# lmb-freiburg/neural-point-cloud-diffusion

Measured on AMD Instinct MI355X. Metric: denoiser train steps/sec (+ rendered rays/sec under 'render'), SRN-Cars 512pt x 128d, higher is better.
Workload: dtype bf16; 1 GPU; BASELINE configs[1]: denoiser fwd/bwd + AdamW + EMA, 512 points x 128-d latents, width 1024 / 24 layers / 16 heads (seq 513), bf16 autocast; global_batch=64, per_gpu_batch=64, parallelism=dp1, rng=weights seed 1234 on every rank; timestep / noise draws seed 42 + rank

## Files before the change

include/npcd_hip.h:

```cpp
#ifndef NPCD_HIP_H
#define NPCD_HIP_H

#include <stdint.h>

#ifdef __cplusplus
extern "C" {
#endif

#define NPCD_OK 0
#define NPCD_ERR_ARG (-1)
#define NPCD_ERR_UNSUPPORTED (-2)
#define NPCD_ERR_HIP (-3)

#define NPCD_BF16 0
#define NPCD_F16 1
#define NPCD_F32 2

int npcd_abi_version(void);
const char* npcd_error_string(int code);
const char* npcd_last_hip_error(void);

int npcd_attn_fwd(const void* q, const void* k, const void* v, void* out, float* lse,
                  int B, int n, int H, int d,
                  int64_t qkv_sb, int64_t qkv_sn, int64_t qkv_sh,
                  int64_t out_sb, int64_t out_sn, int64_t out_sh,
                  float scale, int dtype, void* stream);

int64_t npcd_attn_fwd_workspace_floats(int B, int n, int H);
int npcd_attn_fwd_ws(const void* q, const void* k, const void* v, void* out, float* lse, float* workspace,
                     int B, int n, int H, int d,
                     int64_t qkv_sb, int64_t qkv_sn, int64_t qkv_sh,
                     int64_t out_sb, int64_t out_sn, int64_t out_sh,
                     float scale, int dtype, void* stream);

int64_t npcd_attn_fwd_fp8_workspace_bytes(int B, int n, int H);
int npcd_attn_fwd_fp8(const void* q, const void* k, const void* v, void* out, float* lse, void* workspace,
                      int B, int n, int H, int d,
                      int64_t qkv_sb, int64_t qkv_sn, int64_t qkv_sh,
                      int64_t out_sb, int64_t out_sn, int64_t out_sh,
                      float scale, int dtype, void* stream);

int64_t npcd_attn_bwd_workspace_floats(int B, int n, int H);
int npcd_attn_bwd(const void* q, const void* k, const void* v, const void* out, const void* dout,
                  const float* lse, void* dq, void* dk, void* dv, float* delta,
                  int B, int n, int H, int d,
                  int64_t qkv_sb, int64_t qkv_sn, int64_t qkv_sh,
                  int64_t out_sb, int64_t out_sn, int64_t out_sh,
                  int64_t g_sb, int64_t g_sn, int64_t g_sh,
                  float scale, int dtype, void* stream);

int npcd_attn_bwd_colsum_rows(int B, int n, int H);
int npcd_attn_bwd_colsum(int passes, const void* q, const void* k, const void* v, const void* out, const void* dout,
                         const float* lse, void* dq, void* dk, void* dv, float* delta, float* colsum_part,
                         int B, int n, int H, int d,
                         int64_t qkv_sb, int64_t qkv_sn, int64_t qkv_sh,
                         int64_t out_sb, int64_t out_sn, int64_t out_sh,
                         int64_t g_sb, int64_t g_sn, int64_t g_sh,
                         float scale, int dtype, void* stream);

int npcd_attn_bwd_pass(int pass, const void* q, const void* k, const void* v, const void* out, const void* dout,
                       const float* lse, void* dq, void* dk, void* dv, float* delta,
                       int B, int n, int H, int d,
                       int64_t qkv_sb, int64_t qkv_sn, int64_t qkv_sh,
                       int64_t out_sb, int64_t out_sn, int64_t out_sh,
                       int64_t g_sb, int64_t g_sn, int64_t g_sh,
                       float scale, int dtype, void* stream);

int64_t npcd_attn_bwd_fused_slab_floats(int B, int n, int H);
int npcd_attn_bwd_fused(const void* q, const void* k, const void* v, const void* out, const void* dout,
                        const float* lse, void* dq, void* dk, void* dv, float* delta, float* dq_slab,
                        int B, int n, int H, int d,
                        int64_t qkv_sb, int64_t qkv_sn, int64_t qkv_sh,
                        int64_t out_sb, int64_t out_sn, int64_t out_sh,
                        int64_t g_sb, int64_t g_sn, int64_t g_sh,
                        float scale, int dtype, void* stream);

typedef struct npcd_grid_params {
    float voxel_size[3];
    int32_t voxel_scale[3];
    int32_t kernel_size[3];
    int32_t max_points_per_voxel;
    int32_t max_occ_voxels_per_example;
    float range_min[3];
    float range_max[3];
    int32_t dims[3];
    int32_t cdims[3];
    int32_t grid_level;
} npcd_grid_params;
#define NPCD_GRID_FINE 0
#define NPCD_GRID_SCALED 1

int64_t npcd_grid_workspace_bytes(const npcd_grid_params* g, int B, int N);

int npcd_grid_build(const npcd_grid_params* g, const float* points, const int32_t* counts,
                    int B, int N, void* workspace, void* stream);

int npcd_grid_query(const npcd_grid_params* g, const void* workspace, const float* points,
                    int B, int N, int R, int S, int M, int k, float r, int mode,
                    const float* x, const float* rays_o, const float* rays_d,
                    const float* t0, const float* t1,
                    int32_t* sample_idx, float* sample_loc, int32_t* slot_sample, int32_t* nsel,
                    void* stream);

int npcd_grid_query_compact(const npcd_grid_params* g, const void* workspace, const float* points,
                            int B, int N, int R, int S, int M, int k, float r,
                            const float* rays_o, const float* rays_d, const float* t0, const float* t1,
                            int32_t* counter, int32_t capacity, int32_t* ray_base, int32_t* ray_nsel,
                            uint64_t* ray_bits, int32_t* nb_idx, float* pts, void* stream);

int64_t npcd_grid_query_order_ws_bytes(int B, int R, int M, int k);
int npcd_grid_query_compact_ordered(const npcd_grid_params* g, const void* workspace, const float* points,
                                    int B, int N, int R, int S, int M, int k, float r,
                                    const float* rays_o, const float* rays_d, const float* t0, const float* t1,
                                    int32_t* counter, int32_t capacity, int32_t* ray_base, int32_t* ray_nsel,
                                    uint64_t* ray_bits, int32_t* nb_idx, float* pts, void* order_ws, void* stream);

int64_t npcd_ray_gen_ws_floats(int V, int res, int n_ids);
int npcd_ray_gen(const float* extr, const float* intr, int V, int res, float box,
                 float* rays_o, float* rays_d, float* t0, float* t1, float* limits_ws, void* stream);
int npcd_ray_gen_subset(const float* extr, const float* intr, int V, int res, float box, const int32_t* pixel_ids, int n_ids,
                        float* rays_o, float* rays_d, float* t0, float* t1, float* limits_ws, void* stream);

#define NPCD_SHADE_NONFINITE_PAIRS 1
#define NPCD_SHADE_NONFINITE_HEADS 2
int64_t npcd_shade_wpack_bytes(int feat_dim, int n_freqs, int hidden);
int64_t npcd_shade_workspace_bytes(int max_points, int hidden);
int npcd_shade_pack_weights(const float* const* weights_host, const float* const* biases_host,
                            int feat_dim, int n_freqs, int hidden, void* wpack_host);
int npcd_shade_points(const void* wpack, int feat_dim, int n_freqs, int hidden,
                      const int32_t* nb_idx, const float* pts, const float* kp_pos, const float* kp_feat,
                      const int32_t* n_points_dev, int max_points, int k,
                      float* sigma, float* rgb, void* workspace, int32_t* status, void* stream);

int npcd_shade_points_dir(const void* wpack, int feat_dim, int n_freqs, int hidden,
                          const int32_t* nb_idx, const float* pts, const float* kp_pos, const float* kp_feat,
                          const int32_t* n_points_dev, int max_points, int k,
                          float* sigma, float* rgb, void* workspace, const float* dir_bias, const int32_t* point_ray,
                          int32_t* status, void* stream);

int64_t npcd_pairs_x2_wpack_bytes(int feat_dim);
int npcd_pairs_x2_pack(const float* const* weights_host, const float* const* biases_host, int feat_dim, void* wpack_host);
int npcd_pairs_x2(const void* wpack, int feat_dim, const int32_t* nb_idx, const float* pts, const float* kp_pos, const float* kp_feat,
                  const int32_t* n_points_dev, int max_points, int k, float* G, void* stream);
int64_t npcd_points_x2_wpack_bytes(void);
int npcd_points_x2_pack(const float* const* weights_host, const float* const* biases_host, int c0_in_dim, void* wpack_host);
int npcd_points_x2(const void* wpack, const float* feat, const int32_t* n_points_dev, int max_points, float* sigma, float* rgb,
                   const float* dir_bias, const int32_t* point_ray, void* stream);
int npcd_points_x2_train(const void* wpack, const float* feat, int max_points, float* save, float* pre, void* stream);
int npcd_points_x2_pack_dev(const float* const* weights_dev, const float* const* biases_dev, int c0_in_dim, void* wpack_dev, void* stream);

int64_t npcd_ray_march_ws_floats(int Nr);
int npcd_ray_march(const float* sigma, const float* rgb, const uint8_t* slot_valid, const float* slot_loc,
                   const int32_t* point_base, const float* rays_o, const float* rays_d, const float* t1,
                   int Nr, int M, int white_back, float* mask, float* depth, float* channels,
                   float* depth_ws, void* stream);

int npcd_ray_march_bwd(const float* sigma, const float* rgb, const uint8_t* slot_valid, const float* slot_loc,
                       const int32_t* point_base, const float* rays_o, const float* rays_d, const float* t1,
                       int Nr, int M, int white_back, const float* depth_ws, const float* g_mask, const float* g_depth,
                       const float* g_chan, float* dsigma, float* drgb, void* stream);

int npcd_add_ln_fwd(const float* x_in, const void* delta, const float* gamma, const float* beta,
                    float* x_out, void* y, float* mean, float* rstd, int T, int W, float eps, void* stream);
int npcd_ln_bwd_blocks(int T);
int npcd_ln_bwd(const void* dy, const float* x, const float* mean, const float* rstd, const float* gamma,
                const float* dres, float* dx, void* dxb, float* part_gamma, float* part_beta,
                float* part_col, int T, int W, void* stream);
int npcd_colsum_scratch_rows(void);
int npcd_colsum_finalize(const float* part, int nblk, int N, float* out, int accumulate, void* stream);
#define NPCD_COLSUM_MAX_JOBS 8
typedef struct NpcdColsumJob {
    const float* part;
    float* out;
    int nblk, N, accumulate, reserved;
} NpcdColsumJob;
int npcd_colsum_finalize_batch(const NpcdColsumJob* jobs, int njobs, void* stream);
int npcd_gelu_fwd(const void* h, void* g, int64_t numel, void* stream);
int npcd_colsum_blocks(int T);
int npcd_gelu_bwd(const void* dg, const void* h, void* dh, float* part, int T, int N, void* stream);
int npcd_colsum_bf16(const void* a, float* part, int T, int N, void* stream);
int npcd_small_wgrad_blocks(int T);
int npcd_small_wgrad(const void* dy, const void* x, float* part, int T, int J, int K, void* stream);
int npcd_adamw_ema(float* p, float* g, float* m, float* v, float* ema, void* shadow_bf16, int64_t numel,
                   float lr, float beta1, float beta2, float eps, float weight_decay, int step,
                   float ema_decay, int zero_grad, void* stream);
int npcd_cast_f32_bf16(const float* src, void* dst, int64_t numel, void* stream);
int npcd_add_ln_fwd_dt(const float* x_in, const void* delta, const float* gamma, const float* beta,
                       float* x_out, void* y, float* mean, float* rstd, int T, int W, float eps, int dtype, void* stream);
int npcd_ln_bwd_dt(const void* dy, const float* x, const float* mean, const float* rstd, const float* gamma,
                   const float* dres, float* dx, void* dxb, float* part_gamma, float* part_beta,
                   float* part_col, int T, int W, int dtype, void* stream);
int npcd_gelu_fwd_dt(const void* h, void* g, int64_t numel, int dtype, void* stream);
int npcd_gelu_bwd_dt(const void* dg, const void* h, void* dh, float* part, int T, int N, int dtype, void* stream);
int npcd_colsum_dt(const void* a, float* part, int T, int N, int dtype, void* stream);
int npcd_adamw_ema_dt(float* p, float* g, float* m, float* v, float* ema, void* shadow, int shadow_dtype, int64_t numel,
                      float lr, float beta1, float beta2, float eps, float weight_decay, int step,
                      float ema_decay, int zero_grad, void* stream);
int npcd_cast_f32_dt(const float* src, void* dst, int64_t numel, int dtype, void* stream);

typedef struct NpcdScalerCtl {
    int32_t found_inf, step, growth_tracker, skipped;
    float loss_scale, inv_scale, grad_norm, clip_coef, bc1, bc2_sqrt;
    int32_t reserved[6];
} NpcdScalerCtl;
int npcd_grad_stats_blocks(void);
int npcd_grad_stats(const float* g, int64_t n, double* work, double* out, void* stream);
int npcd_scaler_finalize(const double* stats, int nslots, NpcdScalerCtl* ctl, int scaling, int clip, float max_norm,
                         float beta1, float beta2, float growth_factor, float backoff_factor, int growth_interval, void* stream);
int npcd_adamw_ema_gated(float* p, float* g, float* m, float* v, float* ema, void* shadow, int shadow_dtype, int64_t numel,
                         float lr, float beta1, float beta2, float eps, float weight_decay, double ema_decay, int zero_grad,
                         const NpcdScalerCtl* ctl, void* stream);

int npcd_wgrad_slices(int T, int N, int K);
int npcd_wgrad(const void* dy, const void* x, float* out, float* workspace, int T, int N, int K, int dtype, void* stream);
int npcd_wgrad_group(int count, const void* const* dy, const void* const* x, float* const* out, const int* N, const int* K, int T,
                     int dtype, void* stream);
int npcd_wgrad_group_blocks(int tiles_per_block, int max_products, int products_per_block);

int npcd_linear_fwd(const void* x, const void* w, const void* bias, void* y, int M, int N, int K, int dtype, void* stream);
int npcd_linear_gelu_fwd(const void* x, const void* w, const void* bias, void* h, void* g, int M, int N, int K, int dtype, void* stream);
int npcd_linear_dgelu_rows(int M);
int npcd_linear_dgelu_bwd(const void* dy, const void* wt, const void* h, void* dh, float* part, int M, int N, int K, int dtype, void* stream);
int npcd_linear128_fwd(const void* x, const void* w, const void* bias, void* y, int M, int N, int K, int dtype, void* stream);
int npcd_transpose_16(const void* in, void* out, int R, int C, void* stream);
int npcd_transpose16_group(int count, const void* const* in, void* const* out, const int* R, const int* C, void* stream);

int npcd_sum_slices(const float* part, float* out, int S, int64_t numel, void* stream);

int npcd_ddpm_reverse_step(const float* x_t, const void* eps, int eps_dtype, const float* noise, float* x_prev, float* x0_out,
                           const int64_t* t, int B, int64_t per_sample, const float* tab_recip, const float* tab_recipm1,
                           const float* tab_coef1, const float* tab_coef2, const float* tab_logvar, float clip_lo, float clip_hi,
                           int has_clip, void* stream);

#define NPCD_SAMPLER_REVERSE 0
#define NPCD_SAMPLER_HOLD 1
typedef struct NpcdSamplerTensor {
    const float* x_t;
    const void* eps;
    const float* noise;
    const float* known;
    float* out;
    float* x0_out;
    int64_t per_sample;
    float clip_lo, clip_hi;
    int32_t has_clip, mode, eps_dtype, reserved;
} NpcdSamplerTensor;
int npcd_sampler_step(const NpcdSamplerTensor* coords, const NpcdSamplerTensor* feats, const int64_t* t, const float* table, int T,
                      int B, int deterministic, void* stream);

int npcd_q_sample(const float* x0, const float* noise, const int64_t* t, const float* tab_sqrt_acp, const float* tab_sqrt_1macp,
                  float* x_t, int B, int64_t per_sample, void* stream);
int npcd_eps_mse_blocks(void);
int npcd_eps_mse_fwd(const float* noise, const void* eps, int eps_dtype, int64_t numel, float* pointwise, float* part, float* loss,
                     void* stream);
int npcd_eps_mse_bwd(const float* noise, const void* eps, int eps_dtype, int64_t numel, const float* upstream_dev, void* grad,
                     void* stream);

int npcd_ray_march_compact(const float* sigma, const float* rgb, const uint64_t* ray_bits, const float* pts,
                           const int32_t* ray_base, const float* rays_o, const float* rays_d, const float* t1,
                           int Nr, int M, int capacity, int white_back, float* mask, float* depth, float* channels,
                           float* depth_ws, void* stream);

int64_t npcd_render_lim_words(int B, int R);
int npcd_render_rays_query(const npcd_grid_params* grid, const void* workspace, const float* points, int B, int N, const float* extr,
                           const float* intr, int views, int res, float box, int S, int M, int k, float r, float* rays_o, float* rays_d,
                           float* t0, float* t1, int32_t* counter, int32_t capacity, int32_t* ray_base, int32_t* ray_nsel,
                           uint64_t* ray_bits, int32_t* nb_idx, float* pts, void* order_ws, uint32_t* lim_part, void* stream);
int npcd_ray_march_compact_fused(const float* sigma, const float* rgb, const uint64_t* ray_bits, const float* pts, const int32_t* ray_base,
                                 const float* rays_o, const float* rays_d, const float* t0, const float* t1, const uint32_t* lim_part,
                                 int lim_pairs, int Nr, int M, int capacity, int white_back, float* mask, float* depth,
                                 float* channels, float* depth_ws, void* stream);

int npcd_pair_input_fwd(const int64_t* flat, const int64_t* owner, const float* pts, const float* kp_pos, const float* kp_feat,
                        int feat_dim, int n_freqs, int64_t n_pairs, float* x0, float* w, void* stream);
int npcd_pair_input_bwd(const int64_t* flat, const float* dx0, int feat_dim, int n_cols, int64_t n_pairs, float* dfeat, void* stream);
int npcd_leaky_bwd_blocks(int64_t rows);
int npcd_leaky_bwd_colsum(const void* dz, const void* z, void* dy, float* part, int64_t rows, int N, float slope, int dtype,
                          void* stream);
int npcd_pair_aggregate(int backward, const float* src, const float* w, const int64_t* off, const int64_t* cnt, int channels,
                        int64_t n_points, float* dst, void* stream);

#define NPCD_PAIR_MLP_BF16 0
#define NPCD_PAIR_MLP_X2 1
int64_t npcd_pair_mlp_wpack_bytes(int feat_dim, int precision);
int npcd_pair_mlp_pack(const float* const* weights_dev, const float* const* biases_dev, int feat_dim, int precision, void* wpack_dev,
                       void* stream);
int npcd_pair_mlp_fwd(const void* wpack, int feat_dim, int precision, const int64_t* nb_idx, const float* pts, const float* kp_pos,
                      const float* kp_feat, const int64_t* off, int64_t n_points, int k, int64_t n_pairs, void* x0, void* acts,
                      float* wn, float* G, void* stream);
int npcd_pair_mlp_bwd_slabs(int64_t n_pairs, int precision);
int64_t npcd_pair_mlp_bwd_workspace_floats(int feat_dim, int64_t n_pairs, int precision);
int npcd_pair_mlp_bwd(const void* wpack, int feat_dim, int precision, const float* dG, const int64_t* owner, const float* wn,
                      const void* x0, const void* acts, int64_t n_pairs, void* dact, float* dfeat, float* part, float* const* dW,
                      float* const* db, void* stream);

int npcd_split3_bf16(const float* x, const float* bias, void* out, int64_t rows, int K, int gelu, void* stream);
int npcd_add_ln_split3_bf16(const float* x, const float* o, const float* bias, const float* gamma, const float* beta, float* xnew,
                            void* out, int64_t rows, int W, float eps, void* stream);

#define NPCD_SPLIT_WEIGHTS_MAX 8
typedef struct NpcdSplitWeight {
    const float* w;
    void* fwd;
    void* dgrad;
    int N, K;
} NpcdSplitWeight;
int npcd_add_ln_split3_stats_bf16(const float* x, const float* o, const float* bias, const float* gamma, const float* beta, float* xnew,
                                  void* out, float* mean, float* rstd, int64_t rows, int W, float eps, void* stream);
int npcd_split_weights_bf16(const NpcdSplitWeight* desc, int count, void* stream);
int npcd_ln_bwd_split3_bf16(const float* dy, const float* x, const float* mean, const float* rstd, const float* gamma,
                            const float* dres, float* dx, void* dx3, float* part_gamma, float* part_beta, float* part_col, int T, int W,
                            void* stream);
int npcd_split3_colsum_bf16(const float* a, const float* h, const float* bias, void* out, float* part, int T, int N, int gelu,
                            void* stream);

int64_t npcd_stage1_reg_workspace_floats(int B);
int npcd_stage1_reg_fwd(const float* coords, const int32_t* nb, int64_t nb_ld, const float* feats, int64_t feats_ld, const float* mean,
                        const float* log_var, int64_t kl_ld, int B, int N, int k, int F, float weight_tv, float weight_kl, int dtype,
                        float* tv_pointwise, float* tv_total, float* kl_pointwise, float* kl_total, float* workspace, void* stream);
int npcd_stage1_reg_bwd(const float* coords, const int32_t* nb, int64_t nb_ld, const float* feats, int64_t feats_ld, const float* mean,
                        const float* log_var, int64_t kl_ld, int B, int N, int k, int F, float weight_tv, float weight_kl, int dtype,
                        const float* g_tv_total, const float* g_tv_pointwise, const float* g_kl_total, const float* g_kl_pointwise,
                        float* dfeats, float* dmean, float* dlog_var, void* stream);

int npcd_fps_resident_points(void);
int npcd_fps_max_points(void);
int npcd_fps(const float* points, const int32_t* lengths, const int32_t* ks, const int32_t* start, int64_t* idx_out, float* pts_out,
             int N, int P, int Kmax, void* stream);

int npcd_chamfer_max_points(void);
int npcd_chamfer_directed(const float* x, const int32_t* x_len, const float* y, const int32_t* y_len, float* out, int M, int P, int N,
                          int Q, void* stream);

int npcd_emd_max_points(void);
int npcd_emd_directed(const float* x, const int32_t* x_len, const float* y, const int32_t* y_len, float* out, int M, int P, int N, int Q,
                      void* stream);

int npcd_occupancy_max_resolution(void);
int npcd_occupancy_clouds_per_workgroup(int n, int P, int R);
int npcd_occupancy_grid(const float* points, const int32_t* lengths, const float* lattice, const uint8_t* k_lo, const uint8_t* k_hi,
                        int32_t* counts, int32_t* clouds, int32_t* cells, int n, int P, int R, void* stream);

int npcd_image_metrics_tile(int* rows_host, int* cols_host);
int64_t npcd_image_metrics_workspace_bytes(int V, int C, int H, int W, int w);
int npcd_image_metrics(const float* pred, const float* target, int V, int C, int H, int W, int64_t pred_sv, int64_t pred_sc,
                       int64_t pred_sh, int64_t pred_sw, int64_t target_sv, int64_t target_sc, int64_t target_sh, int64_t target_sw,
                       const double* taps, int w, double n, double data_range, double* workspace, double* mse, double* ssim, double* map,
                       void* stream);

#ifdef __cplusplus
}
#endif
#endif
```

neural-point-cloud-diffusion_amd/csrc/elementwise.hip:

```cpp
#include <math.h>

#include <stdlib.h>

#include "common.h"

namespace npcd {

constexpr int kMaxChunks = 8;

template <class E>
struct V {
    typedef E x4 __attribute__((ext_vector_type(4)));
    typedef E x8 __attribute__((ext_vector_type(8)));
};
template <class X4>
__device__ __forceinline__ f32x4 to_f32(X4 v) { return f32x4{(float)v[0], (float)v[1], (float)v[2], (float)v[3]}; }
template <class E>
__device__ __forceinline__ typename V<E>::x4 from_f32(f32x4 v) { return typename V<E>::x4{(E)v[0], (E)v[1], (E)v[2], (E)v[3]}; }
__device__ __forceinline__ f32x4 bf16x4_to_f32(bf16x4 v) { return to_f32(v); }
__device__ __forceinline__ bf16x4 f32_to_bf16x4(f32x4 v) { return from_f32<__bf16>(v); }

template <class E, int NCH>
__global__ __launch_bounds__(256) void add_ln_fwd_kernel(const float* __restrict__ x_in, const E* __restrict__ delta,
                                                         const float* __restrict__ gamma, const float* __restrict__ beta,
                                                         float* __restrict__ x_out, E* __restrict__ y, float* __restrict__ mean,
                                                         float* __restrict__ rstd, int T, int W, float eps) {
    using e4 = typename V<E>::x4;
    const int lane = threadIdx.x & 63, wave = threadIdx.x >> 6;
    const int NW = gridDim.x * 4;
    int row = blockIdx.x * 4 + wave;
    if (row >= T) return;
    f32x4 gm[NCH], bt[NCH], v[NCH], nx[NCH];
    e4 nd[NCH];
#pragma unroll
    for (int ch = 0; ch < NCH; ++ch) {
        const int c = ch * 256 + lane * 4;
        gm[ch] = bt[ch] = nx[ch] = f32x4{0.f, 0.f, 0.f, 0.f};
        nd[ch] = e4{0, 0, 0, 0};
        if (c < W) {
            gm[ch] = *reinterpret_cast<const f32x4*>(gamma + c);
            bt[ch] = *reinterpret_cast<const f32x4*>(beta + c);
        }
    }
    auto load_row = [&](int r) {
        const int64_t base = (int64_t)r * W;
#pragma unroll
        for (int ch = 0; ch < NCH; ++ch) {
            const int c = ch * 256 + lane * 4;
            if (c < W) {
                nx[ch] = *reinterpret_cast<const f32x4*>(x_in + base + c);
                if (delta) nd[ch] = *reinterpret_cast<const e4*>(delta + base + c);
            }
        }
    };
    load_row(row);
    for (; row < T; row += NW) {
        const int64_t base = (int64_t)row * W;
        float s = 0.f;
#pragma unroll
        for (int ch = 0; ch < NCH; ++ch) {
            v[ch] = nx[ch];
            if (delta) v[ch] += to_f32(nd[ch]);
        }
        if (row + NW < T) load_row(row + NW);
#pragma unroll
        for (int ch = 0; ch < NCH; ++ch) {
            const int c = ch * 256 + lane * 4;
            if (c < W) {
                if (x_out) *reinterpret_cast<f32x4*>(x_out + base + c) = v[ch];
                s += (v[ch][0] + v[ch][1]) + (v[ch][2] + v[ch][3]);
            }
        }
        const float mu = wave_sum64(s) / (float)W;
        float q = 0.f;
#pragma unroll
        for (int ch = 0; ch < NCH; ++ch) {
            const int c = ch * 256 + lane * 4;
            if (c < W) {
                const f32x4 d = v[ch] - mu;
                q += (d[0] * d[0] + d[1] * d[1]) + (d[2] * d[2] + d[3] * d[3]);
            }
        }
        const float rs = rsqrtf(wave_sum64(q) / (float)W + eps);
#pragma unroll
        for (int ch = 0; ch < NCH; ++ch) {
            const int c = ch * 256 + lane * 4;
            if (c < W) *reinterpret_cast<e4*>(y + base + c) = from_f32<E>((v[ch] - mu) * rs * gm[ch] + bt[ch]);
        }
        if (lane == 0) {
            mean[row] = mu;
            rstd[row] = rs;
        }
    }
}

static inline int ln_rows_per_wave(int T) {
    const int one_round = (T + 4 * 512 - 1) / (4 * 512);
    if (one_round <= 32) return one_round < 1 ? 1 : one_round;
    return 16;
}

template <class E, int NCH, class D = E, bool SPLIT = false>
__global__ __launch_bounds__(256, 2) void ln_bwd_kernel(const D* __restrict__ dy, const float* __restrict__ x, const float* __restrict__ mean,
                                                     const float* __restrict__ rstd, const float* __restrict__ gamma,
                                                     const float* __restrict__ dres, float* __restrict__ dx, E* __restrict__ dxb,
                                                     float* __restrict__ part_gamma, float* __restrict__ part_beta,
                                                     float* __restrict__ part_col, int T, int W, int rows_per_wave) {
    using e4 = typename V<D>::x4;
    extern __shared__ __attribute__((aligned(16))) unsigned char dsmem[];
    float* red = reinterpret_cast<float*>(dsmem);
    const int lane = threadIdx.x & 63, wave = threadIdx.x >> 6;
    f32x4 ag[NCH], ab[NCH], ac[NCH];
#pragma unroll
    for (int ch = 0; ch < NCH; ++ch) ag[ch] = ab[ch] = ac[ch] = f32x4{0.f, 0.f, 0.f, 0.f};
    const int row0 = blockIdx.x * 4 + wave, NW = gridDim.x * 4;
    const int nrows = row0 < T ? min(rows_per_wave, (T - row0 + NW - 1) / NW) : 0;
    e4 dyA[NCH], dyB[NCH];
    f32x4 xA[NCH], xB[NCH], rA[NCH], rB[NCH];
    float muA = 0.f, rsA = 0.f, muB = 0.f, rsB = 0.f;
    auto load_row = [&](int row, e4 (&dyr)[NCH], f32x4 (&xr)[NCH], f32x4 (&rr2)[NCH], float& mu, float& rs) {
        const int64_t base = (int64_t)row * W;
        mu = mean[row];
        rs = rstd[row];
#pragma unroll
        for (int ch = 0; ch < NCH; ++ch) {
            const int c = ch * 256 + lane * 4;
            if (c < W) {
                dyr[ch] = *reinterpret_cast<const e4*>(dy + base + c);
                xr[ch] = *reinterpret_cast<const f32x4*>(x + base + c);
                if (dres) rr2[ch] = *reinterpret_cast<const f32x4*>(dres + base + c);
            }
        }
    };
    if (nrows > 0) load_row(row0, dyA, xA, rA, muA, rsA);
    for (int rr = 0; rr < nrows; ++rr) {
        const int row = row0 + rr * NW;
        const int64_t base = (int64_t)row * W;
        if (rr + 1 < nrows) load_row(row + NW, dyB, xB, rB, muB, rsB);
        const float mu = muA, rs = rsA;
        f32x4 gy[NCH], xh[NCH];
        float s1 = 0.f, s2 = 0.f;
#pragma unroll
        for (int ch = 0; ch < NCH; ++ch) {
            const int c = ch * 256 + lane * 4;
            gy[ch] = xh[ch] = f32x4{0.f, 0.f, 0.f, 0.f};
            if (c < W) {
                const f32x4 d = to_f32(dyA[ch]);
                xh[ch] = (xA[ch] - mu) * rs;
                ag[ch] += d * xh[ch];
                ab[ch] += d;
                gy[ch] = d * *reinterpret_cast<const f32x4*>(gamma + c);
                const f32x4 t = gy[ch] * xh[ch];
                s1 += (gy[ch][0] + gy[ch][1]) + (gy[ch][2] + gy[ch][3]);
                s2 += (t[0] + t[1]) + (t[2] + t[3]);
            }
        }
        const float c1 = wave_sum64(s1) / (float)W, c2 = wave_sum64(s2) / (float)W;
#pragma unroll
        for (int ch = 0; ch < NCH; ++ch) {
            const int c = ch * 256 + lane * 4;
            if (c < W) {
                f32x4 o = (gy[ch] - c1 - xh[ch] * c2) * rs;
                if (dres) o += rA[ch];
                *reinterpret_cast<f32x4*>(dx + base + c) = o;
                if (SPLIT && dxb) {
                    bf16x4 hi, lo;
#pragma unroll
                    for (int j = 0; j < 4; ++j) {
                        hi[j] = (__bf16)o[j];
                        lo[j] = (__bf16)(o[j] - (float)hi[j]);
                    }
                    __bf16* o3 = reinterpret_cast<__bf16*>(dxb) + 3 * base + c;
                    *reinterpret_cast<bf16x4*>(o3) = hi;
                    *reinterpret_cast<bf16x4*>(o3 + W) = lo;
                    *reinterpret_cast<bf16x4*>(o3 + 2 * W) = hi;
                } else if (dxb) {
                    *reinterpret_cast<typename V<E>::x4*>(dxb + base + c) = from_f32<E>(o);
                }
                ac[ch] += o;
            }
        }
#pragma unroll
        for (int ch = 0; ch < NCH; ++ch) {
            dyA[ch] = dyB[ch];
            xA[ch] = xB[ch];
            rA[ch] = rB[ch];
        }
        muA = muB;
        rsA = rsB;
    }
#pragma unroll
    for (int ch = 0; ch < NCH; ++ch) {
        const int c = ch * 256 + lane * 4;
        if (c < W) {
            *reinterpret_cast<f32x4*>(red + (0 * 4 + wave) * W + c) = ag[ch];
            *reinterpret_cast<f32x4*>(red + (1 * 4 + wave) * W + c) = ab[ch];
            *reinterpret_cast<f32x4*>(red + (2 * 4 + wave) * W + c) = ac[ch];
        }
    }
    __syncthreads();
    float* outs[3] = {part_gamma, part_beta, part_col};
    for (int q = 0; q < 3; ++q) {
        if (!outs[q]) continue;
        for (int c = threadIdx.x; c < W; c += 256) {
            const float* p = red + q * 4 * W + c;
            outs[q][(int64_t)blockIdx.x * W + c] = (p[0] + p[W]) + (p[2 * W] + p[3 * W]);
        }
    }
}

constexpr int kFinSlices = 16;

struct FinBatch {
    NpcdColsumJob job[NPCD_COLSUM_MAX_JOBS];
    int first1[NPCD_COLSUM_MAX_JOBS + 1];
    int first2[NPCD_COLSUM_MAX_JOBS + 1];
    int njobs;
};
__device__ __forceinline__ int fin_job(const int* first, int njobs, int bx) {
    int j = 0;
    while (j + 1 < njobs && bx >= first[j + 1]) ++j;
    return j;
}
__device__ __forceinline__ bool fin_two_stage(int nblk) { return nblk > 2 * kFinSlices; }

__global__ __launch_bounds__(256) void colsum_stage1_kernel(FinBatch fb) {
    __shared__ float red[4][64];
    const int j = fin_job(fb.first1, fb.njobs, blockIdx.x);
    const float* __restrict__ part = fb.job[j].part;
    const int nblk = fb.job[j].nblk, N = fb.job[j].N;
    if (!fin_two_stage(nblk)) return;
    float* __restrict__ stage = const_cast<float*>(part) + (int64_t)nblk * N;
    const int tx = threadIdx.x & 63, ty = threadIdx.x >> 6;
    const int c = (blockIdx.x - fb.first1[j]) * 64 + tx;
    const int per = (nblk + kFinSlices - 1) / kFinSlices;
    const int b0 = blockIdx.y * per, b1 = min(nblk, b0 + per);
    float s0 = 0.f, s1 = 0.f;
    if (c < N) {
        int b = b0 + ty;
        for (; b + 4 < b1; b += 8) {
            s0 += part[(int64_t)b * N + c];
            s1 += part[(int64_t)(b + 4) * N + c];
        }
        if (b < b1) s0 += part[(int64_t)b * N + c];
    }
    red[ty][tx] = s0 + s1;
    __syncthreads();
    if (ty == 0 && c < N) stage[(int64_t)blockIdx.y * N + c] = (red[0][tx] + red[1][tx]) + (red[2][tx] + red[3][tx]);
}

__global__ __launch_bounds__(256) void colsum_stage2_kernel(FinBatch fb) {
    const int j = fin_job(fb.first2, fb.njobs, blockIdx.x);
    const int nblk = fb.job[j].nblk, N = fb.job[j].N;
    const int c = (blockIdx.x - fb.first2[j]) * 256 + threadIdx.x;
    if (c >= N) return;
    const bool two = fin_two_stage(nblk);
    const float* __restrict__ src = two ? fb.job[j].part + (int64_t)nblk * N : fb.job[j].part;
    const int nrows = two ? kFinSlices : nblk;
    float s = 0.f;
    for (int k = 0; k < nrows; ++k) s += src[(int64_t)k * N + c];
    float* __restrict__ out = fb.job[j].out;
    out[c] = fb.job[j].accumulate ? out[c] + s : s;
}

__device__ __forceinline__ float gelu_f(float x) { return 0.5f * x * (1.f + erff(x * 0.70710678118654752f)); }
__device__ __forceinline__ float gelu_grad_f(float x) {
    return 0.5f * (1.f + erff(x * 0.70710678118654752f)) + x * 0.3989422804014327f * __expf(-0.5f * x * x);
}

__device__ __forceinline__ float gelu_fast(float x) {
    const float u = fabsf(x) * 0.70710678118654752f;
    const float t = __builtin_amdgcn_rcpf(__builtin_fmaf(0.3275911f, u, 1.f));
    const float e = __builtin_amdgcn_exp2f(x * x * -0.72134752044448170f);
    float poly = __builtin_fmaf(t, 1.061405429f, -1.453152027f);
    poly = __builtin_fmaf(poly, t, 1.421413741f);
    poly = __builtin_fmaf(poly, t, -0.284496736f);
    poly = __builtin_fmaf(poly, t, 0.254829592f);
    const float erf_abs = __builtin_fmaf(-poly * t, e, 1.f);
    return x * __builtin_fmaf(0.5f, copysignf(erf_abs, x), 0.5f);
}

template <class E, int VARIANT>
__global__ __launch_bounds__(256) void gelu_fwd_kernel(const typename V<E>::x8* __restrict__ h, typename V<E>::x8* __restrict__ g, int64_t n8) {
    using e8 = typename V<E>::x8;
    for (int64_t i = (int64_t)blockIdx.x * 256 + threadIdx.x; i < n8; i += (int64_t)gridDim.x * 256) {
        const e8 v = h[i];
        e8 o;
#pragma unroll
        for (int j = 0; j < 8; ++j) o[j] = (E)(VARIANT == 0 ? gelu_f((float)v[j]) : gelu_fast((float)v[j]));
        g[i] = o;
    }
}

static inline int col_rows(int T) {
    static const int forced = [] { const char* e = getenv("NPCD_COL_ROWS"); return e ? atoi(e) : 0; }();
    if (forced > 0) return forced;
    int r = T / 512;
    return r < 8 ? 8 : (r > 64 ? 64 : r);
}

__device__ __forceinline__ float gelu_grad_fast(float x) {
    const float u = fabsf(x) * 0.70710678118654752f;
    const float t = __builtin_amdgcn_rcpf(__builtin_fmaf(0.3275911f, u, 1.f));
    const float e = __builtin_amdgcn_exp2f(x * x * -0.72134752044448170f);
    float poly = __builtin_fmaf(t, 1.061405429f, -1.453152027f);
    poly = __builtin_fmaf(poly, t, 1.421413741f);
    poly = __builtin_fmaf(poly, t, -0.284496736f);
    poly = __builtin_fmaf(poly, t, 0.254829592f);
    const float erf_abs = __builtin_fmaf(-poly * t, e, 1.f);
    const float phi_cdf = __builtin_fmaf(0.5f, copysignf(erf_abs, x), 0.5f);
    return __builtin_fmaf(x * 0.3989422804014327f, e, phi_cdf);
}

template <class E, bool GELU, int VARIANT = 1>
__global__ __launch_bounds__(256) void colsum_kernel(const E* __restrict__ a, const E* __restrict__ hpre, E* __restrict__ out,
                                                     float* __restrict__ part, int T, int N, int rows) {
    using e8 = typename V<E>::x8;
    const int col = (blockIdx.x * 256 + threadIdx.x) * 8;
    if (col >= N) return;
    float acc[8];
#pragma unroll
    for (int j = 0; j < 8; ++j) acc[j] = 0.f;
    auto one = [&](const e8 v, const e8 hp, int64_t off) {
        e8 o;
#pragma unroll
        for (int j = 0; j < 8; ++j) {
            const float gp = VARIANT == 0 ? gelu_grad_f((float)hp[j]) : gelu_grad_fast((float)hp[j]);
            o[j] = (E)((float)v[j] * gp);
            acc[j] += (float)o[j];
        }
        *reinterpret_cast<e8*>(out + off) = o;
    };
    if (GELU && VARIANT == 2) {
        int rr = 0;
        for (; rr + 1 < rows; rr += 2) {
            const int r0 = rr * gridDim.y + blockIdx.y, r1 = r0 + gridDim.y;
            if (r1 >= T) break;
            const int64_t o0 = (int64_t)r0 * N + col, o1 = (int64_t)r1 * N + col;
            const e8 v0 = *reinterpret_cast<const e8*>(a + o0), h0 = *reinterpret_cast<const e8*>(hpre + o0);
            const e8 v1 = *reinterpret_cast<const e8*>(a + o1), h1 = *reinterpret_cast<const e8*>(hpre + o1);
            one(v0, h0, o0);
            one(v1, h1, o1);
        }
        for (; rr < rows; ++rr) {
            const int row = rr * gridDim.y + blockIdx.y;
            if (row >= T) break;
            const int64_t off = (int64_t)row * N + col;
            one(*reinterpret_cast<const e8*>(a + off), *reinterpret_cast<const e8*>(hpre + off), off);
        }
    } else {
        for (int rr = 0; rr < rows; ++rr) {
            const int row = rr * gridDim.y + blockIdx.y;
            if (row >= T) break;
            const int64_t off = (int64_t)row * N + col;
            const e8 v = (GELU && VARIANT == 3) ? __builtin_nontemporal_load(reinterpret_cast<const e8*>(a + off))
                                                    : *reinterpret_cast<const e8*>(a + off);
            if (GELU) {
                one(v, VARIANT == 3 ? __builtin_nontemporal_load(reinterpret_cast<const e8*>(hpre + off))
                                    : *reinterpret_cast<const e8*>(hpre + off), off);
            } else {
#pragma unroll
                for (int j = 0; j < 8; ++j) acc[j] += (float)v[j];
            }
        }
    }
    float* p = part + (int64_t)blockIdx.y * N + col;
    *reinterpret_cast<f32x4*>(p) = f32x4{acc[0], acc[1], acc[2], acc[3]};
    *reinterpret_cast<f32x4*>(p + 4) = f32x4{acc[4], acc[5], acc[6], acc[7]};
}

template <int J>
__global__ __launch_bounds__(256) void small_wgrad_kernel(const __bf16* __restrict__ dy, const __bf16* __restrict__ x, float* __restrict__ part,
                                                          int T, int K, int rows_per_block) {
    extern __shared__ float swg_red[];
    const int chunks = K >> 3, lanes = 256 / chunks;
    const int cc = threadIdx.x % chunks, rl = threadIdx.x / chunks;
    const int row0 = blockIdx.x * rows_per_block, row1 = min(T, row0 + rows_per_block);
    float acc[J][8];
#pragma unroll
    for (int j = 0; j < J; ++j)
#pragma unroll
        for (int i = 0; i < 8; ++i) acc[j][i] = 0.f;
    for (int row = row0 + rl; row < row1; row += lanes) {
        const bf16x8 v = *reinterpret_cast<const bf16x8*>(x + (int64_t)row * K + 8 * cc);
        float w[J];
#pragma unroll
        for (int j = 0; j < J; ++j) w[j] = (float)dy[(int64_t)row * J + j];
#pragma unroll
        for (int j = 0; j < J; ++j)
#pragma unroll
            for (int i = 0; i < 8; ++i) acc[j][i] = __builtin_fmaf(w[j], (float)v[i], acc[j][i]);
    }
#pragma unroll
    for (int j = 0; j < J; ++j)
#pragma unroll
        for (int i = 0; i < 8; ++i) swg_red[(rl * J + j) * K + 8 * cc + i] = acc[j][i];
    __syncthreads();
    for (int e = threadIdx.x; e < J * K; e += 256) {
        float sum = 0.f;
        for (int r2 = 0; r2 < lanes; ++r2) sum += swg_red[r2 * J * K + e];
        part[(int64_t)blockIdx.x * J * K + e] = sum;
    }
}

struct AdamArgs {
    float lr, beta1, beta2, eps, wd, bc1, bc2_sqrt, ema_w;
};

__device__ __forceinline__ void adamw_one(f32x4& pp, const f32x4 gg, f32x4& mm, f32x4& vv, const AdamArgs& a) {
    pp *= (1.f - a.lr * a.wd);
    mm = mm * a.beta1 + gg * (1.f - a.beta1);
    vv = vv * a.beta2 + gg * gg * (1.f - a.beta2);
    const float step = a.lr / a.bc1;
#pragma unroll
    for (int j = 0; j < 4; ++j) pp[j] -= step * (mm[j] / (sqrtf(vv[j]) / a.bc2_sqrt + a.eps));
}

template <class E, bool GATED>
__device__ __forceinline__ void adamw_ema_body(f32x4* __restrict__ p, f32x4* __restrict__ g, f32x4* __restrict__ m, f32x4* __restrict__ v,
                                               f32x4* __restrict__ ema, typename V<E>::x4* __restrict__ shadow, int64_t n4, AdamArgs a,
                                               int zero_grad, const NpcdScalerCtl* __restrict__ ctl, float skip_ema_w) {
    const int64_t stride = (int64_t)gridDim.x * 256;
    int64_t i = (int64_t)blockIdx.x * 256 + threadIdx.x;
    float gs = 1.f, gc = 1.f;
    if constexpr (GATED) {
        if (ctl->found_inf) {
            for (; i < n4; i += stride) {
                if (ema) {
                    const f32x4 e = ema[i], pp = p[i];
                    ema[i] = e + (pp - e) * skip_ema_w;
                }
                if (zero_grad) g[i] = f32x4{0.f, 0.f, 0.f, 0.f};
            }
            return;
        }
        gs = ctl->inv_scale;
        gc = ctl->clip_coef;
        a.bc1 = ctl->bc1;
        a.bc2_sqrt = ctl->bc2_sqrt;
    }
    auto grad = [&](f32x4 x) -> f32x4 {
        if constexpr (GATED) {
            x = (x * gs) * gc;
            asm volatile("" : "+v"(x));
        }
        return x;
    };
    for (; i + stride < n4; i += 2 * stride) {
        const int64_t k = i + stride;
        f32x4 p0 = p[i], p1 = p[k];
        const f32x4 g0 = grad(g[i]), g1 = grad(g[k]);
        f32x4 m0 = m[i], m1 = m[k], v0 = v[i], v1 = v[k];
        f32x4 e0 = {0.f, 0.f, 0.f, 0.f}, e1 = e0;
        if (ema) { e0 = ema[i]; e1 = ema[k]; }
        adamw_one(p0, g0, m0, v0, a);
        adamw_one(p1, g1, m1, v1, a);
        p[i] = p0; p[k] = p1;
        m[i] = m0; m[k] = m1;
        v[i] = v0; v[k] = v1;
        if (ema) { ema[i] = e0 + (p0 - e0) * a.ema_w; ema[k] = e1 + (p1 - e1) * a.ema_w; }
        if (shadow) { shadow[i] = from_f32<E>(p0); shadow[k] = from_f32<E>(p1); }
        if (zero_grad) { g[i] = f32x4{0.f, 0.f, 0.f, 0.f}; g[k] = f32x4{0.f, 0.f, 0.f, 0.f}; }
    }
    if (i < n4) {
        f32x4 pp = p[i];
        const f32x4 gg = grad(g[i]);
        f32x4 mm = m[i], vv = v[i];
        adamw_one(pp, gg, mm, vv, a);
        p[i] = pp;
        m[i] = mm;
        v[i] = vv;
        if (ema) {
            const f32x4 e = ema[i];
            ema[i] = e + (pp - e) * a.ema_w;
        }
        if (shadow) shadow[i] = from_f32<E>(pp);
        if (zero_grad) g[i] = f32x4{0.f, 0.f, 0.f, 0.f};
    }
}

template <class E>
__global__ __launch_bounds__(256) void adamw_ema_kernel(f32x4* __restrict__ p, f32x4* __restrict__ g, f32x4* __restrict__ m, f32x4* __restrict__ v,
                                                        f32x4* __restrict__ ema, typename V<E>::x4* __restrict__ shadow, int64_t n4, AdamArgs a, int zero_grad) {
    adamw_ema_body<E, false>(p, g, m, v, ema, shadow, n4, a, zero_grad, nullptr, 0.f);
}
template <class E>
__global__ __launch_bounds__(256) void adamw_ema_gated_kernel(f32x4* __restrict__ p, f32x4* __restrict__ g, f32x4* __restrict__ m,
                                                              f32x4* __restrict__ v, f32x4* __restrict__ ema, typename V<E>::x4* __restrict__ shadow,
                                                              int64_t n4, AdamArgs a, int zero_grad, const NpcdScalerCtl* __restrict__ ctl,
                                                              float skip_ema_w) {
    adamw_ema_body<E, true>(p, g, m, v, ema, shadow, n4, a, zero_grad, ctl, skip_ema_w);
}

constexpr int kStatBlocks = 512;

__device__ __forceinline__ void stat_one(float x, double& s, uint32_t& bad) {
    const bool ok = fabsf(x) <= 3.402823466e38f;
    const double d = ok ? (double)x : 0.0;
    s = fma(d, d, s);
    bad += ok ? 0u : 1u;
}
__device__ __forceinline__ void stat_four(f32x4 x, double& s, uint32_t& bad) {
#pragma unroll
    for (int j = 0; j < 4; ++j) stat_one(x[j], s, bad);
}
__device__ __forceinline__ double wave_sum_f64(double x) {
#pragma unroll
    for (int off = 32; off > 0; off >>= 1) x += __shfl_xor(x, off, 64);
    return x;
}
__device__ __forceinline__ void block_sum2(double& s, double& c) {
    __shared__ double red[2][4];
    s = wave_sum_f64(s);
    c = wave_sum_f64(c);
    if ((threadIdx.x & 63) == 0) { red[0][threadIdx.x >> 6] = s; red[1][threadIdx.x >> 6] = c; }
    __syncthreads();
    s = (red[0][0] + red[0][1]) + (red[0][2] + red[0][3]);
    c = (red[1][0] + red[1][1]) + (red[1][2] + red[1][3]);
}

__global__ __launch_bounds__(256) void grad_stats_kernel(const float* __restrict__ g, int64_t n, double* __restrict__ part) {
    const f32x4* g4 = reinterpret_cast<const f32x4*>(g);
    const int64_t n4 = n / 4, stride = (int64_t)gridDim.x * 256, gid = (int64_t)blockIdx.x * 256 + threadIdx.x;
    double s = 0.0;
    uint32_t bad = 0;
    int64_t i = gid;
    for (; i + stride < n4; i += 2 * stride) {
        const f32x4 x0 = g4[i], x1 = g4[i + stride];
        stat_four(x0, s, bad);
        stat_four(x1, s, bad);
    }
    if (i < n4) stat_four(g4[i], s, bad);
    if (gid < n - 4 * n4) stat_one(g[4 * n4 + gid], s, bad);
    double c = (double)bad;
    block_sum2(s, c);
    if (threadIdx.x == 0) { part[2 * blockIdx.x] = s; part[2 * blockIdx.x + 1] = c; }
}
__global__ __launch_bounds__(256) void grad_stats_sum_kernel(const double* __restrict__ part, int nblk, double* __restrict__ out) {
    double s = 0.0, c = 0.0;
    for (int b = threadIdx.x; b < nblk; b += 256) { s += part[2 * b]; c += part[2 * b + 1]; }
    block_sum2(s, c);
    if (threadIdx.x == 0) { out[0] = s; out[1] = c; }
}

__global__ __launch_bounds__(64) void scaler_finalize_kernel(const double* __restrict__ stats, int nslots, NpcdScalerCtl* __restrict__ ctl,
                                                             int scaling, int clip, float max_norm, float beta1, float beta2, float growth,
                                                             float backoff, int interval) {
    if (threadIdx.x != 0) return;
    double sumsq = 0.0, bad = 0.0;
    for (int k = 0; k < nslots; ++k) { sumsq += stats[2 * k]; bad += stats[2 * k + 1]; }
    NpcdScalerCtl c = *ctl;
    const float inv = scaling ? 1.f / c.loss_scale : 1.f;
    c.inv_scale = inv;
    c.found_inf = (scaling && bad > 0.0) ? 1 : 0;
    const float norm = bad > 0.0 ? INFINITY : (float)(sqrt(sumsq) * (double)inv);
    c.grad_norm = norm;
    c.clip_coef = clip ? fminf((1.f / (norm + 1e-6f)) * max_norm, 1.f) : 1.f;
    if (c.found_inf) {
        c.loss_scale *= backoff;
        c.growth_tracker = 0;
        c.skipped += 1;
    } else {
        c.step += 1;
        c.bc1 = (float)(1.0 - pow((double)beta1, (double)c.step));
        c.bc2_sqrt = (float)sqrt(1.0 - pow((double)beta2, (double)c.step));
        if (scaling && ++c.growth_tracker == interval) {
            c.loss_scale *= growth;
            c.growth_tracker = 0;
        }
    }
    *ctl = c;
}

template <class E>
__global__ __launch_bounds__(256) void cast_kernel(const f32x4* __restrict__ src, typename V<E>::x4* __restrict__ dst, int64_t n4) {
    for (int64_t i = (int64_t)blockIdx.x * 256 + threadIdx.x; i < n4; i += (int64_t)gridDim.x * 256) dst[i] = from_f32<E>(src[i]);
}

template <int S>
__global__ __launch_bounds__(256) void sum_slices_kernel(const f32x4* __restrict__ part, f32x4* __restrict__ out, int64_t n4) {
    for (int64_t i = (int64_t)blockIdx.x * 256 + threadIdx.x; i < n4; i += (int64_t)gridDim.x * 256) {
        f32x4 v[S];
#pragma unroll
        for (int s2 = 0; s2 < S; ++s2) v[s2] = __builtin_nontemporal_load(part + s2 * n4 + i);
        f32x4 acc = v[0];
#pragma unroll
        for (int s2 = 1; s2 < S; ++s2) acc += v[s2];
        out[i] = acc;
    }
}

struct DdpmTables {
    const float *recip, *recipm1, *c1, *c2, *logvar;
};
template <class EPS>
__global__ __launch_bounds__(256) void ddpm_reverse_kernel(const float* __restrict__ x_t, const EPS* __restrict__ eps, const float* __restrict__ noise,
                                                           float* __restrict__ x_prev, float* __restrict__ x0_out, const int64_t* __restrict__ t,
                                                           int64_t per_sample, DdpmTables tab, float lo, float hi, int has_clip) {
    const int b = blockIdx.y;
    const int64_t ts = t[b];
    const float a = tab.recip[ts], bb = tab.recipm1[ts], c1 = tab.c1[ts], c2 = tab.c2[ts];
    const float sd = ts != 0 ? expf(0.5f * tab.logvar[ts]) : 0.f;
    for (int64_t i = (int64_t)blockIdx.x * 256 + threadIdx.x; i < per_sample; i += (int64_t)gridDim.x * 256) {
        const int64_t j = (int64_t)b * per_sample + i;
        const float x = x_t[j];
        float x0 = a * x - bb * (float)eps[j];
        if (has_clip) x0 = fminf(fmaxf(x0, lo), hi);
        if (x0_out) x0_out[j] = x0;
        x_prev[j] = (c1 * x0 + c2 * x) + sd * noise[j];
    }
}

struct SamplerCoef {
    float r, m, c1, c2, s, h1, h2;
};
struct SamplerArgs {
    NpcdSamplerTensor tz[2];
    int vec[2];
};

__device__ __forceinline__ float sampler_x0(const SamplerCoef& k, float x, float e, int has_clip, float lo, float hi) {
    float x0 = __builtin_fmaf(k.r, x, -(k.m * e));
    if (has_clip) x0 = fminf(fmaxf(x0, lo), hi);
    return x0;
}

template <class EPS, bool VEC>
__device__ __forceinline__ void sampler_reverse(const NpcdSamplerTensor& a, const SamplerCoef& k, int64_t base) {
    const float* __restrict__ x_t = a.x_t + base;
    const EPS* __restrict__ eps = static_cast<const EPS*>(a.eps) + base;
    const float* __restrict__ noise = a.noise ? a.noise + base : nullptr;
    float* __restrict__ out = a.out + base;
    float* __restrict__ x0_out = a.x0_out ? a.x0_out + base : nullptr;
    if constexpr (VEC) {
        const int64_t n4 = a.per_sample / 4;
        for (int64_t i = (int64_t)blockIdx.x * 256 + threadIdx.x; i < n4; i += (int64_t)gridDim.x * 256) {
            const f32x4 x = reinterpret_cast<const f32x4*>(x_t)[i];
            const f32x4 e = to_f32(reinterpret_cast<const typename V<EPS>::x4*>(eps)[i]);
            f32x4 z = f32x4{0.f, 0.f, 0.f, 0.f};
            if (noise) z = reinterpret_cast<const f32x4*>(noise)[i];
            f32x4 x0, o;
#pragma unroll
            for (int q = 0; q < 4; ++q) {
                x0[q] = sampler_x0(k, x[q], e[q], a.has_clip, a.clip_lo, a.clip_hi);
                o[q] = __builtin_fmaf(k.c1, x0[q], k.c2 * x[q]);
                if (noise) o[q] = __builtin_fmaf(k.s, z[q], o[q]);
            }
            if (x0_out) reinterpret_cast<f32x4*>(x0_out)[i] = x0;
            reinterpret_cast<f32x4*>(out)[i] = o;
        }
    } else {
        for (int64_t i = (int64_t)blockIdx.x * 256 + threadIdx.x; i < a.per_sample; i += (int64_t)gridDim.x * 256) {
            const float x = x_t[i];
            const float x0 = sampler_x0(k, x, (float)eps[i], a.has_clip, a.clip_lo, a.clip_hi);
            float o = __builtin_fmaf(k.c1, x0, k.c2 * x);
            if (noise) o = __builtin_fmaf(k.s, noise[i], o);
            if (x0_out) x0_out[i] = x0;
            out[i] = o;
        }
    }
}

template <bool VEC>
__device__ __forceinline__ void sampler_hold(const NpcdSamplerTensor& a, const SamplerCoef& k, int64_t base) {
    const float* __restrict__ known = a.known + base;
    const float* __restrict__ noise = a.noise + base;
    float* __restrict__ out = a.out + base;
    if constexpr (VEC) {
        const int64_t n4 = a.per_sample / 4;
        for (int64_t i = (int64_t)blockIdx.x * 256 + threadIdx.x; i < n4; i += (int64_t)gridDim.x * 256) {
            const f32x4 kn = reinterpret_cast<const f32x4*>(known)[i], z = reinterpret_cast<const f32x4*>(noise)[i];
            f32x4 o;
#pragma unroll
            for (int q = 0; q < 4; ++q) o[q] = __builtin_fmaf(k.h1, kn[q], k.h2 * z[q]);
            reinterpret_cast<f32x4*>(out)[i] = o;
        }
    } else {
        for (int64_t i = (int64_t)blockIdx.x * 256 + threadIdx.x; i < a.per_sample; i += (int64_t)gridDim.x * 256)
            out[i] = __builtin_fmaf(k.h1, known[i], k.h2 * noise[i]);
    }
}

__global__ __launch_bounds__(256) void sampler_step_kernel(SamplerArgs args, const int64_t* __restrict__ t, const float* __restrict__ table, int T) {
    const int z = blockIdx.z, b = blockIdx.y;
    const NpcdSamplerTensor& a = args.tz[z];
    const int vec = args.vec[z];
    const int64_t ts = t[b];
    const float nan = __builtin_nanf("");
    SamplerCoef k{nan, nan, nan, nan, nan, nan, nan};
    if (ts >= 0 && ts < T) {
        const f32x4 lo = reinterpret_cast<const f32x4*>(table)[2 * ts], hi = reinterpret_cast<const f32x4*>(table)[2 * ts + 1];
        k = SamplerCoef{lo[0], lo[1], lo[2], lo[3], hi[0], hi[1], hi[2]};
    }
    const int64_t base = (int64_t)b * a.per_sample;
    if (a.mode == NPCD_SAMPLER_HOLD) {
        if (vec) sampler_hold<true>(a, k, base);
        else sampler_hold<false>(a, k, base);
    } else if (a.eps_dtype == NPCD_F32) {
        if (vec) sampler_reverse<float, true>(a, k, base);
        else sampler_reverse<float, false>(a, k, base);
    } else {
        if (vec) sampler_reverse<__bf16, true>(a, k, base);
        else sampler_reverse<__bf16, false>(a, k, base);
    }
}

static bool al16(const void* p) { return (reinterpret_cast<uintptr_t>(p) & 15) == 0; }

}

using namespace npcd;

static inline int ln_fwd_blocks(int T) { const int b = (T + 3) / 4; return b < 2048 ? b : 2048; }

static inline bool dt16(int dtype) { return dtype == NPCD_BF16 || dtype == NPCD_F16; }

extern "C" int npcd_add_ln_fwd_dt(const float* x_in, const void* delta, const float* gamma, const float* beta, float* x_out, void* y,
                                  float* mean, float* rstd, int T, int W, float eps, int dtype, void* stream) {
    if (!x_in || !gamma || !beta || !y || !mean || !rstd || T <= 0 || W <= 0) return NPCD_ERR_ARG;
    if (W % 4 != 0 || W > 256 * kMaxChunks || !dt16(dtype)) return NPCD_ERR_UNSUPPORTED;
    if (!al16(x_in) || !al16(gamma) || !al16(beta) || (x_out && !al16(x_out)) || (reinterpret_cast<uintptr_t>(y) & 7) ||
        (delta && (reinterpret_cast<uintptr_t>(delta) & 7)))
        return NPCD_ERR_ARG;
#define NPCD_LAUNCH_LN_FWD(E, NCH)                                                                                            \
    hipLaunchKernelGGL((add_ln_fwd_kernel<E, NCH>), dim3(ln_fwd_blocks(T)), dim3(256), 0, static_cast<hipStream_t>(stream), x_in, \
                       static_cast<const E*>(delta), gamma, beta, x_out, static_cast<E*>(y), mean, rstd, T, W, eps)
#define NPCD_LN_FWD_W(E)                     \
    do {                                     \
        if (W <= 256) NPCD_LAUNCH_LN_FWD(E, 1);      \
        else if (W <= 512) NPCD_LAUNCH_LN_FWD(E, 2); \
        else if (W <= 1024) NPCD_LAUNCH_LN_FWD(E, 4);\
        else NPCD_LAUNCH_LN_FWD(E, 8);               \
    } while (0)
    if (dtype == NPCD_BF16) NPCD_LN_FWD_W(__bf16);
    else NPCD_LN_FWD_W(_Float16);
#undef NPCD_LN_FWD_W
#undef NPCD_LAUNCH_LN_FWD
    NPCD_HIP_CHECK(hipGetLastError());
    return NPCD_OK;
}
extern "C" int npcd_add_ln_fwd(const float* x_in, const void* delta, const float* gamma, const float* beta, float* x_out, void* y,
                               float* mean, float* rstd, int T, int W, float eps, void* stream) {
    return npcd_add_ln_fwd_dt(x_in, delta, gamma, beta, x_out, y, mean, rstd, T, W, eps, NPCD_BF16, stream);
}

extern "C" int npcd_ln_bwd_blocks(int T) { const int r = ln_rows_per_wave(T); return (T + 4 * r - 1) / (4 * r); }

extern "C" int npcd_ln_bwd_dt(const void* dy, const float* x, const float* mean, const float* rstd, const float* gamma, const float* dres,
                              float* dx, void* dxb, float* part_gamma, float* part_beta, float* part_col, int T, int W, int dtype, void* stream) {
    if (!dy || !x || !mean || !rstd || !gamma || !dx || T <= 0 || W <= 0) return NPCD_ERR_ARG;
    if (W % 4 != 0 || W > 256 * kMaxChunks || !dt16(dtype)) return NPCD_ERR_UNSUPPORTED;
    if (!al16(x) || !al16(gamma) || !al16(dx) || (dres && !al16(dres))) return NPCD_ERR_ARG;
    const int nblk = npcd_ln_bwd_blocks(T);
    const size_t lds = (size_t)3 * 4 * W * sizeof(float);
    hipStream_t st = static_cast<hipStream_t>(stream);
    static DynLds lds_attr_b, lds_attr_h;
    if (dtype == NPCD_BF16) NPCD_HIP_CHECK(lds_attr_b.ensure(reinterpret_cast<const void*>(ln_bwd_kernel<__bf16, 8>), 3 * 4 * 2048 * 4));
    else NPCD_HIP_CHECK(lds_attr_h.ensure(reinterpret_cast<const void*>(ln_bwd_kernel<_Float16, 8>), 3 * 4 * 2048 * 4));
#define NPCD_LAUNCH_LN_BWD(E, NCH)                                                                                             \
    hipLaunchKernelGGL((ln_bwd_kernel<E, NCH>), dim3(nblk), dim3(256), lds, st, static_cast<const E*>(dy), x, mean, rstd, gamma, \
                       dres, dx, static_cast<E*>(dxb), part_gamma, part_beta, part_col, T, W, ln_rows_per_wave(T))
#define NPCD_LN_BWD_W(E)                     \
    do {                                     \
        if (W <= 256) NPCD_LAUNCH_LN_BWD(E, 1);      \
        else if (W <= 512) NPCD_LAUNCH_LN_BWD(E, 2); \
        else if (W <= 1024) NPCD_LAUNCH_LN_BWD(E, 4);\
        else NPCD_LAUNCH_LN_BWD(E, 8);               \
    } while (0)
    if (dtype == NPCD_BF16) NPCD_LN_BWD_W(__bf16);
    else NPCD_LN_BWD_W(_Float16);
#undef NPCD_LN_BWD_W
#undef NPCD_LAUNCH_LN_BWD
    NPCD_HIP_CHECK(hipGetLastError());
    return NPCD_OK;
}
extern "C" int npcd_ln_bwd_split3_bf16(const float* dy, const float* x, const float* mean, const float* rstd, const float* gamma,
                                       const float* dres, float* dx, void* dx3, float* part_gamma, float* part_beta, float* part_col, int T,
                                       int W, void* stream) {
    if (!dy || !x || !mean || !rstd || !gamma || !dx || T <= 0 || W <= 0) return NPCD_ERR_ARG;
    if (W % 4 != 0 || W > 256 * kMaxChunks) return NPCD_ERR_UNSUPPORTED;
    if (!al16(dy) || !al16(x) || !al16(gamma) || !al16(dx) || (dres && !al16(dres)) || (dx3 && !al16(dx3))) return NPCD_ERR_ARG;
    const int nblk = npcd_ln_bwd_blocks(T);
    const size_t lds = (size_t)3 * 4 * W * sizeof(float);
    hipStream_t st = static_cast<hipStream_t>(stream);
    static DynLds lds_attr;
    NPCD_HIP_CHECK(lds_attr.ensure(reinterpret_cast<const void*>(ln_bwd_kernel<__bf16, 8, float, true>), 3 * 4 * 2048 * 4));
#define NPCD_LAUNCH_LN_BWD3(NCH)                                                                                                        \
    hipLaunchKernelGGL((ln_bwd_kernel<__bf16, NCH, float, true>), dim3(nblk), dim3(256), lds, st, dy, x, mean, rstd, gamma, dres, dx, \
                       static_cast<__bf16*>(dx3), part_gamma, part_beta, part_col, T, W, ln_rows_per_wave(T))
    if (W <= 256) NPCD_LAUNCH_LN_BWD3(1);
    else if (W <= 512) NPCD_LAUNCH_LN_BWD3(2);
    else if (W <= 1024) NPCD_LAUNCH_LN_BWD3(4);
    else NPCD_LAUNCH_LN_BWD3(8);
#undef NPCD_LAUNCH_LN_BWD3
    NPCD_HIP_CHECK(hipGetLastError());
    return NPCD_OK;
}

extern "C" int npcd_ln_bwd(const void* dy, const float* x, const float* mean, const float* rstd, const float* gamma, const float* dres,
                           float* dx, void* dxb, float* part_gamma, float* part_beta, float* part_col, int T, int W, void* stream) {
    return npcd_ln_bwd_dt(dy, x, mean, rstd, gamma, dres, dx, dxb, part_gamma, part_beta, part_col, T, W, NPCD_BF16, stream);
}

__global__ __launch_bounds__(1024) void colsum_onepass_kernel(FinBatch fb) {
    __shared__ float red[16][64];
    const int j = fin_job(fb.first1, fb.njobs, blockIdx.x);
    const float* __restrict__ part = fb.job[j].part;
    const int nblk = fb.job[j].nblk, N = fb.job[j].N;
    const int tx = threadIdx.x & 63, ty = threadIdx.x >> 6;
    const int c = (blockIdx.x - fb.first1[j]) * 64 + tx;
    float s0 = 0.f, s1 = 0.f;
    if (c < N) {
        int b = ty;
        for (; b + 16 < nblk; b += 32) {
            s0 += part[(int64_t)b * N + c];
            s1 += part[(int64_t)(b + 16) * N + c];
        }
        if (b < nblk) s0 += part[(int64_t)b * N + c];
    }
    red[ty][tx] = s0 + s1;
    __syncthreads();
    if (ty == 0 && c < N) {
        float q[4];
#pragma unroll
        for (int g = 0; g < 4; ++g) q[g] = (red[4 * g][tx] + red[4 * g + 1][tx]) + (red[4 * g + 2][tx] + red[4 * g + 3][tx]);
        const float s = (q[0] + q[1]) + (q[2] + q[3]);
        float* __restrict__ out = fb.job[j].out;
        out[c] = fb.job[j].accumulate ? out[c] + s : s;
    }
}

extern "C" int npcd_colsum_scratch_rows(void) { return kFinSlices; }

extern "C" int npcd_colsum_finalize_batch(const NpcdColsumJob* jobs, int njobs, void* stream) {
    if (!jobs || njobs <= 0 || njobs > NPCD_COLSUM_MAX_JOBS) return NPCD_ERR_ARG;
    FinBatch fb;
    fb.njobs = njobs;
    bool any_two_stage = false;
    int n1 = 0, n2 = 0;
    for (int j = 0; j < njobs; ++j) {
        if (!jobs[j].part || !jobs[j].out || jobs[j].nblk <= 0 || jobs[j].N <= 0) return NPCD_ERR_ARG;
        fb.job[j] = jobs[j];
        fb.first1[j] = n1;
        fb.first2[j] = n2;
        n1 += (jobs[j].N + 63) / 64;
        n2 += (jobs[j].N + 255) / 256;
        any_two_stage |= jobs[j].nblk > 2 * kFinSlices;
    }
    for (int j = njobs; j <= NPCD_COLSUM_MAX_JOBS; ++j) { fb.first1[j] = n1; fb.first2[j] = n2; }
    hipStream_t st = static_cast<hipStream_t>(stream);
    static const bool onepass = [] { const char* e = getenv("NPCD_COLSUM_ONEPASS"); return e && atoi(e) > 0; }();
    if (onepass) {
        hipLaunchKernelGGL(colsum_onepass_kernel, dim3(n1), dim3(1024), 0, st, fb);
        NPCD_HIP_CHECK(hipGetLastError());
        return NPCD_OK;
    }
    if (any_two_stage) hipLaunchKernelGGL(colsum_stage1_kernel, dim3(n1, kFinSlices), dim3(256), 0, st, fb);
    hipLaunchKernelGGL(colsum_stage2_kernel, dim3(n2), dim3(256), 0, st, fb);
    NPCD_HIP_CHECK(hipGetLastError());
    return NPCD_OK;
}

extern "C" int npcd_colsum_finalize(const float* part, int nblk, int N, float* out, int accumulate, void* stream) {
    NpcdColsumJob job;
    job.part = part; job.out = out; job.nblk = nblk; job.N = N; job.accumulate = accumulate; job.reserved = 0;
    return npcd_colsum_finalize_batch(&job, 1, stream);
}

extern "C" int npcd_gelu_fwd_dt(const void* h, void* g, int64_t numel, int dtype, void* stream) {
    if (!h || !g || numel <= 0) return NPCD_ERR_ARG;
    if (numel % 8 != 0 || !al16(h) || !al16(g) || !dt16(dtype)) return NPCD_ERR_UNSUPPORTED;
    const int64_t n8 = numel / 8;
    const int grid = (int)((n8 + 255) / 256 < 16384 ? (n8 + 255) / 256 : 16384);
    static const int variant = [] { const char* e = getenv("NPCD_GELU_FWD_VARIANT"); return e ? atoi(e) : 1; }();
    hipStream_t st = static_cast<hipStream_t>(stream);
#define NPCD_LAUNCH_GELU_FWD(E, VV)                                                                                                 \
    hipLaunchKernelGGL((gelu_fwd_kernel<E, VV>), dim3(grid), dim3(256), 0, st, static_cast<const typename V<E>::x8*>(h), \
                       static_cast<typename V<E>::x8*>(g), n8)
    if (dtype == NPCD_BF16) {
        if (variant == 0) NPCD_LAUNCH_GELU_FWD(__bf16, 0);
        else NPCD_LAUNCH_GELU_FWD(__bf16, 1);
    } else {
        NPCD_LAUNCH_GELU_FWD(_Float16, 1);
    }
#undef NPCD_LAUNCH_GELU_FWD
    NPCD_HIP_CHECK(hipGetLastError());
    return NPCD_OK;
}
extern "C" int npcd_gelu_fwd(const void* h, void* g, int64_t numel, void* stream) { return npcd_gelu_fwd_dt(h, g, numel, NPCD_BF16, stream); }

extern "C" int npcd_colsum_blocks(int T) { const int r = col_rows(T); return (T + r - 1) / r; }

extern "C" int npcd_gelu_bwd_dt(const void* dg, const void* h, void* dh, float* part, int T, int N, int dtype, void* stream) {
    if (!dg || !h || !dh || !part || T <= 0 || N <= 0) return NPCD_ERR_ARG;
    if (N % 8 != 0 || !al16(dg) || !al16(h) || !al16(dh) || !al16(part) || !dt16(dtype)) return NPCD_ERR_UNSUPPORTED;
    dim3 grid((N / 8 + 255) / 256, npcd_colsum_blocks(T));
    static const int variant = [] { const char* e = getenv("NPCD_GELU_BWD_VARIANT"); return e ? atoi(e) : 1; }();
#define NPCD_LAUNCH_GELU_BWD(E, VV)                                                                                                    \
    hipLaunchKernelGGL((colsum_kernel<E, true, VV>), grid, dim3(256), 0, static_cast<hipStream_t>(stream), static_cast<const E*>(dg), \
                       static_cast<const E*>(h), static_cast<E*>(dh), part, T, N, col_rows(T))
    if (dtype == NPCD_F16) NPCD_LAUNCH_GELU_BWD(_Float16, 1);
    else if (variant == 0) NPCD_LAUNCH_GELU_BWD(__bf16, 0);
    else if (variant == 2) NPCD_LAUNCH_GELU_BWD(__bf16, 2);
    else if (variant == 3) NPCD_LAUNCH_GELU_BWD(__bf16, 3);
    else NPCD_LAUNCH_GELU_BWD(__bf16, 1);
#undef NPCD_LAUNCH_GELU_BWD
    NPCD_HIP_CHECK(hipGetLastError());
    return NPCD_OK;
}
extern "C" int npcd_gelu_bwd(const void* dg, const void* h, void* dh, float* part, int T, int N, void* stream) {
    return npcd_gelu_bwd_dt(dg, h, dh, part, T, N, NPCD_BF16, stream);
}

extern "C" int npcd_colsum_dt(const void* a, float* part, int T, int N, int dtype, void* stream) {
    if (!a || !part || T <= 0 || N <= 0) return NPCD_ERR_ARG;
    if (N % 8 != 0 || !al16(a) || !al16(part) || !dt16(dtype)) return NPCD_ERR_UNSUPPORTED;
    dim3 grid((N / 8 + 255) / 256, npcd_colsum_blocks(T));
    if (dtype == NPCD_BF16)
        hipLaunchKernelGGL((colsum_kernel<__bf16, false>), grid, dim3(256), 0, static_cast<hipStream_t>(stream), static_cast<const __bf16*>(a),
                           static_cast<const __bf16*>(nullptr), static_cast<__bf16*>(nullptr), part, T, N, col_rows(T));
    else
        hipLaunchKernelGGL((colsum_kernel<_Float16, false>), grid, dim3(256), 0, static_cast<hipStream_t>(stream), static_cast<const _Float16*>(a),
                           static_cast<const _Float16*>(nullptr), static_cast<_Float16*>(nullptr), part, T, N, col_rows(T));
    NPCD_HIP_CHECK(hipGetLastError());
    return NPCD_OK;
}
extern "C" int npcd_colsum_bf16(const void* a, float* part, int T, int N, void* stream) { return npcd_colsum_dt(a, part, T, N, NPCD_BF16, stream); }

extern "C" int npcd_small_wgrad_blocks(int T) { return T <= 0 ? -1 : (T + 255) / 256 < 1024 ? (T + 255) / 256 : 1024; }

extern "C" int npcd_small_wgrad(const void* dy, const void* x, float* part, int T, int J, int K, void* stream) {
    if (!dy || !x || !part || T <= 0) return NPCD_ERR_ARG;
    if (J < 1 || J > 4 || K < 64 || K > 2048 || (K & (K - 1)) || !al16(x) || !al16(part)) return NPCD_ERR_UNSUPPORTED;
    const int nblk = npcd_small_wgrad_blocks(T), rpb = (T + nblk - 1) / nblk;
    const size_t lds = (size_t)(256 / (K / 8)) * J * K * sizeof(float);
    hipStream_t st = static_cast<hipStream_t>(stream);
    const __bf16* d = static_cast<const __bf16*>(dy);
    const __bf16* xx = static_cast<const __bf16*>(x);
    switch (J) {
        case 1: hipLaunchKernelGGL(small_wgrad_kernel<1>, dim3(nblk), dim3(256), lds, st, d, xx, part, T, K, rpb); break;
        case 2: hipLaunchKernelGGL(small_wgrad_kernel<2>, dim3(nblk), dim3(256), lds, st, d, xx, part, T, K, rpb); break;
        case 3: hipLaunchKernelGGL(small_wgrad_kernel<3>, dim3(nblk), dim3(256), lds, st, d, xx, part, T, K, rpb); break;
        default: hipLaunchKernelGGL(small_wgrad_kernel<4>, dim3(nblk), dim3(256), lds, st, d, xx, part, T, K, rpb); break;
    }
    NPCD_HIP_CHECK(hipGetLastError());
    return NPCD_OK;
}

extern "C" int npcd_adamw_ema_dt(float* p, float* g, float* m, float* v, float* ema, void* shadow, int shadow_dtype, int64_t numel, float lr,
                                 float beta1, float beta2, float eps, float weight_decay, int step, float ema_decay, int zero_grad, void* stream) {
    if (!p || !g || !m || !v || numel <= 0 || step <= 0) return NPCD_ERR_ARG;
    if (numel % 4 != 0 || !al16(p) || !al16(g) || !al16(m) || !al16(v) || (ema && !al16(ema)) ||
        (shadow && ((reinterpret_cast<uintptr_t>(shadow) & 7) || !dt16(shadow_dtype))))
        return NPCD_ERR_UNSUPPORTED;
    AdamArgs a;
    a.lr = lr; a.beta1 = beta1; a.beta2 = beta2; a.eps = eps; a.wd = weight_decay;
    a.bc1 = (float)(1.0 - pow((double)beta1, (double)step));
    a.bc2_sqrt = (float)sqrt(1.0 - pow((double)beta2, (double)step));
    a.ema_w = 1.f - ema_decay;
    const int64_t n4 = numel / 4;
    const int grid = (int)((n4 + 255) / 256 < 8192 ? (n4 + 255) / 256 : 8192);
    hipStream_t st = static_cast<hipStream_t>(stream);
    if (shadow && shadow_dtype == NPCD_F16)
        hipLaunchKernelGGL(adamw_ema_kernel<_Float16>, dim3(grid), dim3(256), 0, st, reinterpret_cast<f32x4*>(p), reinterpret_cast<f32x4*>(g),
                           reinterpret_cast<f32x4*>(m), reinterpret_cast<f32x4*>(v), reinterpret_cast<f32x4*>(ema),
                           static_cast<V<_Float16>::x4*>(shadow), n4, a, zero_grad);
    else
        hipLaunchKernelGGL(adamw_ema_kernel<__bf16>, dim3(grid), dim3(256), 0, st, reinterpret_cast<f32x4*>(p), reinterpret_cast<f32x4*>(g),
                           reinterpret_cast<f32x4*>(m), reinterpret_cast<f32x4*>(v), reinterpret_cast<f32x4*>(ema),
                           static_cast<V<__bf16>::x4*>(shadow), n4, a, zero_grad);
    NPCD_HIP_CHECK(hipGetLastError());
    return NPCD_OK;
}
extern "C" int npcd_adamw_ema(float* p, float* g, float* m, float* v, float* ema, void* shadow_bf16, int64_t numel, float lr, float beta1,
                              float beta2, float eps, float weight_decay, int step, float ema_decay, int zero_grad, void* stream) {
    return npcd_adamw_ema_dt(p, g, m, v, ema, shadow_bf16, NPCD_BF16, numel, lr, beta1, beta2, eps, weight_decay, step, ema_decay, zero_grad, stream);
}

extern "C" int npcd_adamw_ema_gated(float* p, float* g, float* m, float* v, float* ema, void* shadow, int shadow_dtype, int64_t numel, float lr,
                                    float beta1, float beta2, float eps, float weight_decay, double ema_decay, int zero_grad,
                                    const NpcdScalerCtl* ctl, void* stream) {
    if (!p || !g || !m || !v || !ctl || numel <= 0) return NPCD_ERR_ARG;
    if (numel % 4 != 0 || !al16(p) || !al16(g) || !al16(m) || !al16(v) || (ema && !al16(ema)) || (reinterpret_cast<uintptr_t>(ctl) & 15) ||
        (shadow && ((reinterpret_cast<uintptr_t>(shadow) & 7) || !dt16(shadow_dtype))))
        return NPCD_ERR_UNSUPPORTED;
    AdamArgs a;
    a.lr = lr; a.beta1 = beta1; a.beta2 = beta2; a.eps = eps; a.wd = weight_decay;
    a.bc1 = 1.f; a.bc2_sqrt = 1.f;
    a.ema_w = 1.f - (float)ema_decay;
    const float skip_w = (float)(1.0 - ema_decay);
    const int64_t n4 = numel / 4;
    const int grid = (int)((n4 + 255) / 256 < 8192 ? (n4 + 255) / 256 : 8192);
    hipStream_t st = static_cast<hipStream_t>(stream);
    if (shadow && shadow_dtype == NPCD_F16)
        hipLaunchKernelGGL(adamw_ema_gated_kernel<_Float16>, dim3(grid), dim3(256), 0, st, reinterpret_cast<f32x4*>(p), reinterpret_cast<f32x4*>(g),
                           reinterpret_cast<f32x4*>(m), reinterpret_cast<f32x4*>(v), reinterpret_cast<f32x4*>(ema),
                           static_cast<V<_Float16>::x4*>(shadow), n4, a, zero_grad, ctl, skip_w);
    else
        hipLaunchKernelGGL(adamw_ema_gated_kernel<__bf16>, dim3(grid), dim3(256), 0, st, reinterpret_cast<f32x4*>(p), reinterpret_cast<f32x4*>(g),
                           reinterpret_cast<f32x4*>(m), reinterpret_cast<f32x4*>(v), reinterpret_cast<f32x4*>(ema),
                           static_cast<V<__bf16>::x4*>(shadow), n4, a, zero_grad, ctl, skip_w);
    NPCD_HIP_CHECK(hipGetLastError());
    return NPCD_OK;
}

extern "C" int npcd_grad_stats_blocks(void) { return kStatBlocks; }

extern "C" int npcd_grad_stats(const float* g, int64_t n, double* work, double* out, void* stream) {
    if (!g || !work || !out || n <= 0) return NPCD_ERR_ARG;
    if (!al16(g) || (reinterpret_cast<uintptr_t>(work) & 7) || (reinterpret_cast<uintptr_t>(out) & 7)) return NPCD_ERR_UNSUPPORTED;
    const int64_t n4 = n / 4, want = (n4 + 511) / 512;
    const int grid = (int)(want < 1 ? 1 : want < kStatBlocks ? want : kStatBlocks);
    hipStream_t st = static_cast<hipStream_t>(stream);
    hipLaunchKernelGGL(grad_stats_kernel, dim3(grid), dim3(256), 0, st, g, n, work);
    hipLaunchKernelGGL(grad_stats_sum_kernel, dim3(1), dim3(256), 0, st, work, grid, out);
    NPCD_HIP_CHECK(hipGetLastError());
    return NPCD_OK;
}

extern "C" int npcd_scaler_finalize(const double* stats, int nslots, NpcdScalerCtl* ctl, int scaling, int clip, float max_norm, float beta1,
                                    float beta2, float growth_factor, float backoff_factor, int growth_interval, void* stream) {
    if (!stats || !ctl || nslots <= 0 || growth_interval <= 0) return NPCD_ERR_ARG;
    if ((reinterpret_cast<uintptr_t>(stats) & 7) || (reinterpret_cast<uintptr_t>(ctl) & 15)) return NPCD_ERR_UNSUPPORTED;
    hipLaunchKernelGGL(scaler_finalize_kernel, dim3(1), dim3(64), 0, static_cast<hipStream_t>(stream), stats, nslots, ctl, scaling, clip, max_norm,
                       beta1, beta2, growth_factor, backoff_factor, growth_interval);
    NPCD_HIP_CHECK(hipGetLastError());
    return NPCD_OK;
}

extern "C" int npcd_ddpm_reverse_step(const float* x_t, const void* eps, int eps_dtype, const float* noise, float* x_prev, float* x0_out,
                                      const int64_t* t, int B, int64_t per_sample, const float* tab_recip, const float* tab_recipm1,
                                      const float* tab_coef1, const float* tab_coef2, const float* tab_logvar, float clip_lo, float clip_hi,
                                      int has_clip, void* stream) {
    if (!x_t || !eps || !noise || !x_prev || !t || B <= 0 || per_sample <= 0) return NPCD_ERR_ARG;
    if (!tab_recip || !tab_recipm1 || !tab_coef1 || !tab_coef2 || !tab_logvar) return NPCD_ERR_ARG;
    if (eps_dtype != NPCD_F32 && eps_dtype != NPCD_BF16) return NPCD_ERR_UNSUPPORTED;
    const DdpmTables tab{tab_recip, tab_recipm1, tab_coef1, tab_coef2, tab_logvar};
    const int gx = (int)((per_sample + 255) / 256 < 1024 ? (per_sample + 255) / 256 : 1024);
    hipStream_t st = static_cast<hipStream_t>(stream);
    if (eps_dtype == NPCD_F32)
        hipLaunchKernelGGL(ddpm_reverse_kernel<float>, dim3(gx, B), dim3(256), 0, st, x_t, static_cast<const float*>(eps), noise, x_prev, x0_out, t,
                           per_sample, tab, clip_lo, clip_hi, has_clip);
    else
        hipLaunchKernelGGL(ddpm_reverse_kernel<__bf16>, dim3(gx, B), dim3(256), 0, st, x_t, static_cast<const __bf16*>(eps), noise, x_prev, x0_out, t,
                           per_sample, tab, clip_lo, clip_hi, has_clip);
    NPCD_HIP_CHECK(hipGetLastError());
    return NPCD_OK;
}

extern "C" int npcd_sampler_step(const NpcdSamplerTensor* coords, const NpcdSamplerTensor* feats, const int64_t* t, const float* table, int T,
                                 int B, int deterministic, void* stream) {
    if (!coords || !feats || !t || !table || T <= 0 || B <= 0) return NPCD_ERR_ARG;
    if (B > 65535 || !al16(table)) return NPCD_ERR_UNSUPPORTED;
    SamplerArgs args;
    int gx = 1;
    for (int z = 0; z < 2; ++z) {
        const NpcdSamplerTensor& a = z ? *feats : *coords;
        if (!a.out || a.per_sample <= 0) return NPCD_ERR_ARG;
        bool vec = a.per_sample % 4 == 0 && al16(a.out);
        if (a.mode == NPCD_SAMPLER_HOLD) {
            if (!a.known || !a.noise) return NPCD_ERR_ARG;
            vec = vec && al16(a.known) && al16(a.noise);
        } else if (a.mode == NPCD_SAMPLER_REVERSE) {
            if (!a.x_t || !a.eps || (!a.noise && !deterministic)) return NPCD_ERR_ARG;
            if (a.eps_dtype != NPCD_F32 && a.eps_dtype != NPCD_BF16) return NPCD_ERR_UNSUPPORTED;
            vec = vec && al16(a.x_t) && (!a.noise || al16(a.noise)) && (!a.x0_out || al16(a.x0_out)) &&
                  (reinterpret_cast<uintptr_t>(a.eps) & (a.eps_dtype == NPCD_F32 ? 15 : 7)) == 0;
        } else {
            return NPCD_ERR_ARG;
        }
        args.tz[z] = a;
        args.vec[z] = vec ? 1 : 0;
        const int64_t items = vec ? a.per_sample / 4 : a.per_sample;
        const int g = (int)((items + 255) / 256 < 1024 ? (items + 255) / 256 : 1024);
        gx = g > gx ? g : gx;
    }
    hipLaunchKernelGGL(sampler_step_kernel, dim3(gx, B, 2), dim3(256), 0, static_cast<hipStream_t>(stream), args, t, table, T);
    NPCD_HIP_CHECK(hipGetLastError());
    return NPCD_OK;
}

namespace npcd {
__global__ __launch_bounds__(256) void q_sample_kernel(const float* __restrict__ x0, const float* __restrict__ noise, const int64_t* __restrict__ t,
                                                       const float* __restrict__ tab_a, const float* __restrict__ tab_s, float* __restrict__ xt,
                                                       int64_t per_sample) {
#pragma clang fp contract(off)
    const int b = blockIdx.y;
    const float ca = tab_a[t[b]], cs = tab_s[t[b]];
    const int64_t base = (int64_t)b * per_sample;
    for (int64_t i = (int64_t)blockIdx.x * 256 + threadIdx.x; i < per_sample; i += (int64_t)gridDim.x * 256) {
        const float p0 = ca * x0[base + i], p1 = cs * noise[base + i];
        xt[base + i] = p0 + p1;
    }
}

constexpr int kMseBlocks = 256;
template <class T>
__global__ __launch_bounds__(256) void eps_mse_fwd_kernel(const float* __restrict__ noise, const T* __restrict__ eps, float* __restrict__ pointwise,
                                                          float* __restrict__ part, int64_t numel) {
    __shared__ float red[4];
    float s = 0.f;
    for (int64_t i = (int64_t)blockIdx.x * 256 + threadIdx.x; i < numel; i += (int64_t)gridDim.x * 256) {
        const float d = noise[i] - (float)eps[i];
        const float pw = d * d * 0.5f;
        if (pointwise) pointwise[i] = pw;
        s += pw;
    }
#pragma unroll
    for (int off = 32; off > 0; off >>= 1) s += __shfl_xor(s, off, 64);
    if ((threadIdx.x & 63) == 0) red[threadIdx.x >> 6] = s;
    __syncthreads();
    if (threadIdx.x == 0) part[blockIdx.x] = (red[0] + red[1]) + (red[2] + red[3]);
}
__global__ __launch_bounds__(64) void eps_mse_finalize_kernel(const float* __restrict__ part, int nblocks, float inv_numel, float* __restrict__ out) {
    float s = 0.f;
    for (int i = threadIdx.x; i < nblocks; i += 64) s += part[i];
#pragma unroll
    for (int off = 32; off > 0; off >>= 1) s += __shfl_xor(s, off, 64);
    if (threadIdx.x == 0) out[0] = s * inv_numel;
}
template <class T>
__global__ __launch_bounds__(256) void eps_mse_bwd_kernel(const float* __restrict__ noise, const T* __restrict__ eps, const float* __restrict__ upstream,
                                                          float inv_numel, T* __restrict__ grad, int64_t numel) {
    const float g = upstream[0] * inv_numel;
    for (int64_t i = (int64_t)blockIdx.x * 256 + threadIdx.x; i < numel; i += (int64_t)gridDim.x * 256)
        grad[i] = (T)(-(noise[i] - (float)eps[i]) * g);
}
}

extern "C" int npcd_q_sample(const float* x0, const float* noise, const int64_t* t, const float* tab_sqrt_acp, const float* tab_sqrt_1macp,
                             float* x_t, int B, int64_t per_sample, void* stream) {
    if (!x0 || !noise || !t || !tab_sqrt_acp || !tab_sqrt_1macp || !x_t || B <= 0 || per_sample <= 0) return NPCD_ERR_ARG;
    const int gx = (int)((per_sample + 255) / 256 < 256 ? (per_sample + 255) / 256 : 256);
    hipLaunchKernelGGL(q_sample_kernel, dim3(gx, B), dim3(256), 0, static_cast<hipStream_t>(stream), x0, noise, t, tab_sqrt_acp, tab_sqrt_1macp, x_t,
                       per_sample);
    NPCD_HIP_CHECK(hipGetLastError());
    return NPCD_OK;
}

extern "C" int npcd_eps_mse_blocks(void) { return kMseBlocks; }

extern "C" int npcd_eps_mse_fwd(const float* noise, const void* eps, int eps_dtype, int64_t numel, float* pointwise, float* part, float* loss,
                                void* stream) {
    if (!noise || !eps || !part || !loss || numel <= 0) return NPCD_ERR_ARG;
    if (eps_dtype != NPCD_F32 && eps_dtype != NPCD_BF16) return NPCD_ERR_UNSUPPORTED;
    hipStream_t st = static_cast<hipStream_t>(stream);
    if (eps_dtype == NPCD_F32)
        hipLaunchKernelGGL(eps_mse_fwd_kernel<float>, dim3(kMseBlocks), dim3(256), 0, st, noise, static_cast<const float*>(eps), pointwise, part, numel);
    else
        hipLaunchKernelGGL(eps_mse_fwd_kernel<__bf16>, dim3(kMseBlocks), dim3(256), 0, st, noise, static_cast<const __bf16*>(eps), pointwise, part, numel);
    hipLaunchKernelGGL(eps_mse_finalize_kernel, dim3(1), dim3(64), 0, st, part, kMseBlocks, 1.f / (float)numel, loss);
    NPCD_HIP_CHECK(hipGetLastError());
    return NPCD_OK;
}

extern "C" int npcd_eps_mse_bwd(const float* noise, const void* eps, int eps_dtype, int64_t numel, const float* upstream_dev, void* grad,
                                void* stream) {
    if (!noise || !eps || !upstream_dev || !grad || numel <= 0) return NPCD_ERR_ARG;
    if (eps_dtype != NPCD_F32 && eps_dtype != NPCD_BF16) return NPCD_ERR_UNSUPPORTED;
    hipStream_t st = static_cast<hipStream_t>(stream);
    const int grid = (int)((numel + 255) / 256 < 2048 ? (numel + 255) / 256 : 2048);
    if (eps_dtype == NPCD_F32)
        hipLaunchKernelGGL(eps_mse_bwd_kernel<float>, dim3(grid), dim3(256), 0, st, noise, static_cast<const float*>(eps), upstream_dev,
                           1.f / (float)numel, static_cast<float*>(grad), numel);
    else
        hipLaunchKernelGGL(eps_mse_bwd_kernel<__bf16>, dim3(grid), dim3(256), 0, st, noise, static_cast<const __bf16*>(eps), upstream_dev,
                           1.f / (float)numel, static_cast<__bf16*>(grad), numel);
    NPCD_HIP_CHECK(hipGetLastError());
    return NPCD_OK;
}

extern "C" int npcd_sum_slices(const float* part, float* out, int S, int64_t numel, void* stream) {
    if (!part || !out || numel <= 0) return NPCD_ERR_ARG;
    if ((S != 2 && S != 4 && S != 8) || numel % 4 != 0 || !al16(part) || !al16(out)) return NPCD_ERR_UNSUPPORTED;
    const int64_t n4 = numel / 4;
    const int grid = (int)((n4 + 255) / 256 < 4096 ? (n4 + 255) / 256 : 4096);
    hipStream_t st = static_cast<hipStream_t>(stream);
    const f32x4* p4 = reinterpret_cast<const f32x4*>(part);
    f32x4* o4 = reinterpret_cast<f32x4*>(out);
    if (S == 2) hipLaunchKernelGGL(sum_slices_kernel<2>, dim3(grid), dim3(256), 0, st, p4, o4, n4);
    else if (S == 4) hipLaunchKernelGGL(sum_slices_kernel<4>, dim3(grid), dim3(256), 0, st, p4, o4, n4);
    else hipLaunchKernelGGL(sum_slices_kernel<8>, dim3(grid), dim3(256), 0, st, p4, o4, n4);
    NPCD_HIP_CHECK(hipGetLastError());
    return NPCD_OK;
}

extern "C" int npcd_cast_f32_dt(const float* src, void* dst, int64_t numel, int dtype, void* stream) {
    if (!src || !dst || numel <= 0) return NPCD_ERR_ARG;
    if (numel % 4 != 0 || !al16(src) || (reinterpret_cast<uintptr_t>(dst) & 7) || !dt16(dtype)) return NPCD_ERR_UNSUPPORTED;
    const int64_t n4 = numel / 4;
    const int grid = (int)((n4 + 255) / 256 < 8192 ? (n4 + 255) / 256 : 8192);
    hipStream_t st = static_cast<hipStream_t>(stream);
    if (dtype == NPCD_BF16)
        hipLaunchKernelGGL(cast_kernel<__bf16>, dim3(grid), dim3(256), 0, st, reinterpret_cast<const f32x4*>(src), static_cast<V<__bf16>::x4*>(dst), n4);
    else
        hipLaunchKernelGGL(cast_kernel<_Float16>, dim3(grid), dim3(256), 0, st, reinterpret_cast<const f32x4*>(src), static_cast<V<_Float16>::x4*>(dst), n4);
    NPCD_HIP_CHECK(hipGetLastError());
    return NPCD_OK;
}
extern "C" int npcd_cast_f32_bf16(const float* src, void* dst, int64_t numel, void* stream) { return npcd_cast_f32_dt(src, dst, numel, NPCD_BF16, stream); }
```

neural-point-cloud-diffusion_amd/npcd/hip/__init__.py:

```python
import ctypes
import os
from ctypes import POINTER, c_char_p, c_double, c_float, c_int, c_int32, c_int64, c_void_p

import torch

_PKG_ROOT = os.path.dirname(os.path.dirname(os.path.dirname(os.path.abspath(__file__))))
LIB_PATH = os.environ.get("NPCD_HIP_LIB") or os.path.join(_PKG_ROOT, "lib", "libnpcd_hip.so")

NPCD_BF16, NPCD_F16, NPCD_F32 = 0, 1, 2
NPCD_GRID_FINE, NPCD_GRID_SCALED = 0, 1
_DTYPE_CODE = {torch.bfloat16: NPCD_BF16, torch.float16: NPCD_F16, torch.float32: NPCD_F32}


class GridParams(ctypes.Structure):
    _fields_ = [("voxel_size", c_float * 3), ("voxel_scale", c_int32 * 3), ("kernel_size", c_int32 * 3),
                ("max_points_per_voxel", c_int32), ("max_occ_voxels_per_example", c_int32),
                ("range_min", c_float * 3), ("range_max", c_float * 3), ("dims", c_int32 * 3), ("cdims", c_int32 * 3),
                ("grid_level", c_int32)]


_P = c_void_p
SIGNATURES = {
    "npcd_abi_version": (c_int, []),
    "npcd_error_string": (c_char_p, [c_int]),
    "npcd_last_hip_error": (c_char_p, []),
    "npcd_attn_fwd": (c_int, [_P, _P, _P, _P, _P, c_int, c_int, c_int, c_int] + [c_int64] * 6 + [c_float, c_int, _P]),
    "npcd_attn_fwd_workspace_floats": (c_int64, [c_int, c_int, c_int]),
    "npcd_attn_fwd_ws": (c_int, [_P, _P, _P, _P, _P, _P, c_int, c_int, c_int, c_int] + [c_int64] * 6 + [c_float, c_int, _P]),
    "npcd_ray_march_bwd": (c_int, [_P] * 8 + [c_int, c_int, c_int] + [_P] * 6 + [_P]),
    "npcd_leaky_bwd_blocks": (c_int, [c_int64]),
    "npcd_leaky_bwd_colsum": (c_int, [_P, _P, _P, _P, c_int64, c_int, c_float, c_int, _P]),
    "npcd_pair_input_fwd": (c_int, [_P] * 5 + [c_int, c_int, c_int64, _P, _P, _P]),
    "npcd_pair_input_bwd": (c_int, [_P, _P, c_int, c_int, c_int64, _P, _P]),
    "npcd_pair_aggregate": (c_int, [c_int, _P, _P, _P, _P, c_int, c_int64, _P, _P]),
    "npcd_attn_bwd": (c_int, [_P] * 10 + [c_int] * 4 + [c_int64] * 9 + [c_float, c_int, _P]),
    "npcd_attn_bwd_workspace_floats": (c_int64, [c_int, c_int, c_int]),
    "npcd_attn_bwd_colsum_rows": (c_int, [c_int, c_int, c_int]),
    "npcd_attn_bwd_colsum": (c_int, [c_int] + [_P] * 11 + [c_int] * 4 + [c_int64] * 9 + [c_float, c_int, _P]),
    "npcd_attn_fwd_fp8_workspace_bytes": (c_int64, [c_int, c_int, c_int]),
    "npcd_attn_fwd_fp8": (c_int, [_P] * 6 + [c_int] * 4 + [c_int64] * 6 + [c_float, c_int, _P]),
    "npcd_attn_bwd_fused_slab_floats": (c_int64, [c_int, c_int, c_int]),
    "npcd_attn_bwd_fused": (c_int, [_P] * 11 + [c_int] * 4 + [c_int64] * 9 + [c_float, c_int, _P]),
    "npcd_attn_bwd_pass": (c_int, [c_int] + [_P] * 10 + [c_int] * 4 + [c_int64] * 9 + [c_float, c_int, _P]),
    "npcd_grid_workspace_bytes": (c_int64, [POINTER(GridParams), c_int, c_int]),
    "npcd_grid_build": (c_int, [POINTER(GridParams), _P, _P, c_int, c_int, _P, _P]),
    "npcd_grid_query": (c_int, [POINTER(GridParams), _P, _P] + [c_int] * 6 + [c_float, c_int] + [_P] * 9 + [_P]),
    "npcd_grid_query_compact": (c_int, [POINTER(GridParams), _P, _P] + [c_int] * 6 + [c_float] + [_P] * 5 + [c_int32] + [_P] * 5 + [_P]),
    "npcd_grid_query_compact_ordered": (c_int, [POINTER(GridParams), _P, _P] + [c_int] * 6 + [c_float] + [_P] * 5 + [c_int32] + [_P] * 5
                                        + [_P, _P]),
    "npcd_grid_query_order_ws_bytes": (c_int64, [c_int] * 4),
    "npcd_ray_march_compact": (c_int, [_P] * 8 + [c_int, c_int, c_int, c_int] + [_P] * 4 + [_P]),
    "npcd_render_lim_words": (c_int64, [c_int, c_int]),
    "npcd_render_rays_query": (c_int, [POINTER(GridParams), _P, _P, c_int, c_int, _P, _P, c_int, c_int, c_float, c_int, c_int, c_int, c_float]
                               + [_P] * 5 + [c_int32] + [_P] * 7 + [_P]),
    "npcd_ray_march_compact_fused": (c_int, [_P] * 10 + [c_int, c_int, c_int, c_int, c_int] + [_P] * 4 + [_P]),
    "npcd_ray_gen": (c_int, [_P, _P, c_int, c_int, c_float] + [_P] * 5 + [_P]),
    "npcd_ray_gen_subset": (c_int, [_P, _P, c_int, c_int, c_float, _P, c_int] + [_P] * 5 + [_P]),
    "npcd_shade_wpack_bytes": (c_int64, [c_int, c_int, c_int]),
    "npcd_shade_workspace_bytes": (c_int64, [c_int, c_int]),
    "npcd_shade_pack_weights": (c_int, [POINTER(_P), POINTER(_P), c_int, c_int, c_int, _P]),
    "npcd_pairs_x2_wpack_bytes": (c_int64, [c_int]),
    "npcd_pairs_x2_pack": (c_int, [POINTER(_P), POINTER(_P), c_int, _P]),
    "npcd_pairs_x2": (c_int, [_P, c_int, _P, _P, _P, _P, _P, c_int, c_int, _P, _P]),
    "npcd_points_x2_wpack_bytes": (c_int64, []),
    "npcd_points_x2_pack": (c_int, [POINTER(_P), POINTER(_P), c_int, _P]),
    "npcd_points_x2": (c_int, [_P, _P, _P, c_int, _P, _P, _P, _P, _P]),
    "npcd_points_x2_train": (c_int, [_P, _P, c_int, _P, _P, _P]),
    "npcd_points_x2_pack_dev": (c_int, [POINTER(_P), POINTER(_P), c_int, _P, _P]),
    "npcd_shade_points": (c_int, [_P, c_int, c_int, c_int] + [_P] * 5 + [c_int, c_int] + [_P] * 3 + [_P] + [_P]),
    "npcd_shade_points_dir": (c_int, [_P, c_int, c_int, c_int] + [_P] * 5 + [c_int, c_int] + [_P] * 3 + [_P, _P] + [_P] + [_P]),
    "npcd_ray_march_ws_floats": (c_int64, [c_int]),
    "npcd_ray_gen_ws_floats": (c_int64, [c_int, c_int, c_int]),
    "npcd_ray_march": (c_int, [_P] * 8 + [c_int, c_int, c_int] + [_P] * 4 + [_P]),
    "npcd_add_ln_fwd": (c_int, [_P] * 8 + [c_int, c_int, c_float, _P]),
    "npcd_ln_bwd_blocks": (c_int, [c_int]),
    "npcd_ln_bwd": (c_int, [_P] * 11 + [c_int, c_int, _P]),
    "npcd_colsum_scratch_rows": (c_int, []),
    "npcd_colsum_finalize": (c_int, [_P, c_int, c_int, _P, c_int, _P]),
    "npcd_colsum_finalize_batch": (c_int, [_P, c_int, _P]),
    "npcd_ddpm_reverse_step": (c_int, [_P, _P, c_int, _P, _P, _P, _P, c_int, c_int64, _P, _P, _P, _P, _P, c_float, c_float, c_int, _P]),
    "npcd_sampler_step": (c_int, [_P, _P, _P, _P, c_int, c_int, c_int, _P]),
    "npcd_gelu_fwd": (c_int, [_P, _P, c_int64, _P]),
    "npcd_colsum_blocks": (c_int, [c_int]),
    "npcd_gelu_bwd": (c_int, [_P, _P, _P, _P, c_int, c_int, _P]),
    "npcd_colsum_bf16": (c_int, [_P, _P, c_int, c_int, _P]),
    "npcd_adamw_ema": (c_int, [_P] * 6 + [c_int64] + [c_float] * 5 + [c_int, c_float, c_int, _P]),
    "npcd_cast_f32_bf16": (c_int, [_P, _P, c_int64, _P]),
    "npcd_add_ln_fwd_dt": (c_int, [_P] * 8 + [c_int, c_int, c_float, c_int, _P]),
    "npcd_ln_bwd_dt": (c_int, [_P] * 11 + [c_int, c_int, c_int, _P]),
    "npcd_gelu_fwd_dt": (c_int, [_P, _P, c_int64, c_int, _P]),
    "npcd_gelu_bwd_dt": (c_int, [_P, _P, _P, _P, c_int, c_int, c_int, _P]),
    "npcd_colsum_dt": (c_int, [_P, _P, c_int, c_int, c_int, _P]),
    "npcd_adamw_ema_dt": (c_int, [_P] * 6 + [c_int, c_int64] + [c_float] * 5 + [c_int, c_float, c_int, _P]),
    "npcd_cast_f32_dt": (c_int, [_P, _P, c_int64, c_int, _P]),
    "npcd_grad_stats_blocks": (c_int, []),
    "npcd_grad_stats": (c_int, [_P, c_int64, _P, _P, _P]),
    "npcd_scaler_finalize": (c_int, [_P, c_int, _P, c_int, c_int] + [c_float] * 5 + [c_int, _P]),
    "npcd_adamw_ema_gated": (c_int, [_P] * 6 + [c_int, c_int64] + [c_float] * 5 + [c_double, c_int, _P, _P]),
    "npcd_wgrad_slices": (c_int, [c_int, c_int, c_int]),
    "npcd_wgrad": (c_int, [_P, _P, _P, _P, c_int, c_int, c_int, c_int, _P]),
    "npcd_wgrad_group": (c_int, [c_int, POINTER(_P), POINTER(_P), POINTER(_P), POINTER(c_int), POINTER(c_int), c_int, c_int, _P]),
    "npcd_wgrad_group_blocks": (c_int, [c_int, c_int, c_int]),
    "npcd_sum_slices": (c_int, [_P, _P, c_int, c_int64, _P]),
    "npcd_linear_fwd": (c_int, [_P, _P, _P, _P, c_int, c_int, c_int, c_int, _P]),
    "npcd_linear128_fwd": (c_int, [_P, _P, _P, _P, c_int, c_int, c_int, c_int, _P]),
    "npcd_linear_gelu_fwd": (c_int, [_P, _P, _P, _P, _P, c_int, c_int, c_int, c_int, _P]),
    "npcd_linear_dgelu_rows": (c_int, [c_int]),
    "npcd_linear_dgelu_bwd": (c_int, [_P, _P, _P, _P, _P, c_int, c_int, c_int, c_int, _P]),
    "npcd_transpose_16": (c_int, [_P, _P, c_int, c_int, _P]),
    "npcd_transpose16_group": (c_int, [c_int, POINTER(_P), POINTER(_P), POINTER(c_int), POINTER(c_int), _P]),
    "npcd_small_wgrad_blocks": (c_int, [c_int]),
    "npcd_small_wgrad": (c_int, [_P, _P, _P, c_int, c_int, c_int, _P]),
    "npcd_q_sample": (c_int, [_P] * 6 + [c_int, c_int64, _P]),
    "npcd_eps_mse_blocks": (c_int, []),
    "npcd_eps_mse_fwd": (c_int, [_P, _P, c_int, c_int64, _P, _P, _P, _P]),
    "npcd_eps_mse_bwd": (c_int, [_P, _P, c_int, c_int64, _P, _P, _P]),
    "npcd_split3_bf16": (c_int, [_P, _P, _P, c_int64, c_int, c_int, _P]),
    "npcd_add_ln_split3_bf16": (c_int, [_P] * 7 + [c_int64, c_int, c_float, _P]),
    "npcd_add_ln_split3_stats_bf16": (c_int, [_P] * 9 + [c_int64, c_int, c_float, _P]),
    "npcd_split_weights_bf16": (c_int, [_P, c_int, _P]),
    "npcd_ln_bwd_split3_bf16": (c_int, [_P] * 11 + [c_int, c_int, _P]),
    "npcd_split3_colsum_bf16": (c_int, [_P] * 5 + [c_int, c_int, c_int, _P]),
    "npcd_pair_mlp_wpack_bytes": (c_int64, [c_int, c_int]),
    "npcd_pair_mlp_pack": (c_int, [POINTER(_P), POINTER(_P), c_int, c_int, _P, _P]),
    "npcd_pair_mlp_fwd": (c_int, [_P, c_int, c_int] + [_P] * 5 + [c_int64, c_int, c_int64] + [_P] * 4 + [_P]),
    "npcd_pair_mlp_bwd_slabs": (c_int, [c_int64, c_int]),
    "npcd_pair_mlp_bwd_workspace_floats": (c_int64, [c_int, c_int64, c_int]),
    "npcd_pair_mlp_bwd": (c_int, [_P, c_int, c_int] + [_P] * 5 + [c_int64] + [_P] * 3 + [POINTER(_P), POINTER(_P), _P]),
    "npcd_stage1_reg_workspace_floats": (c_int64, [c_int]),
    "npcd_stage1_reg_fwd": (c_int, [_P, _P, c_int64, _P, c_int64, _P, _P, c_int64] + [c_int] * 4 + [c_float, c_float, c_int] + [_P] * 5 + [_P]),
    "npcd_stage1_reg_bwd": (c_int, [_P, _P, c_int64, _P, c_int64, _P, _P, c_int64] + [c_int] * 4 + [c_float, c_float, c_int] + [_P] * 7 + [_P]),
    "npcd_fps_resident_points": (c_int, []),
    "npcd_fps_max_points": (c_int, []),
    "npcd_fps": (c_int, [_P] * 6 + [c_int, c_int, c_int, _P]),
    "npcd_chamfer_max_points": (c_int, []),
    "npcd_chamfer_directed": (c_int, [_P] * 5 + [c_int] * 4 + [_P]),
    "npcd_emd_max_points": (c_int, []),
    "npcd_emd_directed": (c_int, [_P] * 5 + [c_int] * 4 + [_P]),
    "npcd_occupancy_max_resolution": (c_int, []),
    "npcd_occupancy_clouds_per_workgroup": (c_int, [c_int, c_int, c_int]),
    "npcd_occupancy_grid": (c_int, [_P] * 8 + [c_int] * 3 + [_P]),
    "npcd_image_metrics_tile": (c_int, [POINTER(c_int), POINTER(c_int)]),
    "npcd_image_metrics_workspace_bytes": (c_int64, [c_int] * 5),
    "npcd_image_metrics": (c_int, [_P, _P] + [c_int] * 4 + [c_int64] * 8 + [_P, c_int, c_double, c_double] + [_P] * 4 + [_P]),
}

_lib = None


def lib() -> ctypes.CDLL:
    global _lib
    if _lib is None:
        if not os.path.exists(LIB_PATH):
            raise RuntimeError(
                f"libnpcd_hip.so not found at {LIB_PATH}: build it with "
                f"`python neural-point-cloud-diffusion_amd/csrc/build.py` (or __graft_entry__.build()). "
                f"There is no CPU / PyTorch fallback for the NPCD hot path.")
        handle = ctypes.CDLL(LIB_PATH)
        missing = []
        for name, (res, args) in SIGNATURES.items():
            try:
                fn = getattr(handle, name)
            except AttributeError:
                missing.append(name)
                continue
            fn.restype, fn.argtypes = res, args
        handle.npcd_missing = tuple(missing)
        _lib = handle
    return _lib


def check(rc: int, what: str):
    if rc != 0:
        L = lib()
        msg = L.npcd_error_string(rc).decode()
        if rc == -3:
            msg += ": " + L.npcd_last_hip_error().decode()
        raise RuntimeError(f"{what} failed: {msg} (code {rc})")


def require_gpu(*tensors: torch.Tensor):
    for t in tensors:
        if t is not None and not t.is_cuda:
            raise RuntimeError("npcd.hip operators need GPU tensors (MI355X); got a tensor on "
                               f"{t.device}. There is no CPU fallback in the product path.")


def dtype_code(t: torch.Tensor) -> int:
    try:
        return _DTYPE_CODE[t.dtype]
    except KeyError:
        raise RuntimeError(f"unsupported dtype {t.dtype}") from None


def ptr(t):
    return c_void_p(0 if t is None else t.data_ptr())


_raw_stream = getattr(torch._C, "_cuda_getCurrentRawStream", None)


def stream_ptr():
    if _raw_stream is not None:
        return c_void_p(_raw_stream(torch.cuda.current_device()))
    return c_void_p(torch.cuda.current_stream().cuda_stream)
```

neural-point-cloud-diffusion_amd/npcd/hip/elementwise.py:

```python
import ctypes

import torch

from . import arena, check, dtype_code, lib, ptr, require_gpu, stream_ptr

_f32, _bf16, _f16 = torch.float32, torch.bfloat16, torch.float16
MAX_JOBS = 8

KERNEL_EVENTS = None


def _timed(tag, fn):
    if KERNEL_EVENTS is None or tag not in KERNEL_EVENTS:
        return fn()
    e0, e1 = torch.cuda.Event(enable_timing=True), torch.cuda.Event(enable_timing=True)
    e0.record()
    rc = fn()
    e1.record()
    KERNEL_EVENTS[tag].append((e0, e1))
    return rc


class ColsumJob(ctypes.Structure):
    _fields_ = [("part", ctypes.c_void_p), ("out", ctypes.c_void_p), ("nblk", ctypes.c_int), ("N", ctypes.c_int),
                ("accumulate", ctypes.c_int), ("reserved", ctypes.c_int)]


class ColsumBatch:

    def __init__(self):
        self.jobs = []

    def add(self, part, nblk, N, out, accumulate=False):
        self.jobs.append((part, nblk, N, out, accumulate))

    def flush(self):
        L, s = lib(), stream_ptr()
        for i in range(0, len(self.jobs), MAX_JOBS):
            chunk = self.jobs[i:i + MAX_JOBS]
            arr = (ColsumJob * len(chunk))()
            for a, (part, nblk, N, out, acc) in zip(arr, chunk):
                a.part, a.out, a.nblk, a.N, a.accumulate, a.reserved = part.data_ptr(), out.data_ptr(), nblk, N, int(acc), 0
            check(L.npcd_colsum_finalize_batch(ctypes.cast(arr, ctypes.c_void_p), len(chunk), s), "npcd_colsum_finalize_batch")
        self.jobs = []


def _finish(batch, part, nblk, N, out):
    if batch is not None:
        batch.add(part, nblk, N, out)
    else:
        check(lib().npcd_colsum_finalize(ptr(part), nblk, N, ptr(out), 0, stream_ptr()), "npcd_colsum_finalize")


def add_ln_fwd(x_in, delta, gamma, beta, eps=1e-5, want_sum=True, dtype=_bf16):
    require_gpu(x_in)
    T, W = x_in.shape
    dev = x_in.device
    if delta is not None:
        dtype = delta.dtype
    x_out = arena.empty_like(x_in) if (delta is not None and want_sum) else None
    y = arena.empty((T, W), dtype, dev)
    mean = arena.empty(T, _f32, dev)
    rstd = arena.empty(T, _f32, dev)
    check(_timed("add_ln_fwd" if delta is not None and want_sum else "ln_fwd",
                 lambda: lib().npcd_add_ln_fwd_dt(ptr(x_in), ptr(delta), ptr(gamma), ptr(beta), ptr(x_out), ptr(y), ptr(mean), ptr(rstd), T, W,
                                                  float(eps), dtype_code(y), stream_ptr())), "npcd_add_ln_fwd")
    return x_out, y, mean, rstd


def ln_bwd(dy, x, mean, rstd, gamma, dres, dgamma_out, dbeta_out, dcol_out=None, want_bf16=True, batch=None):
    T, W = x.shape
    dev = x.device
    L = lib()
    nblk = L.npcd_ln_bwd_blocks(T)
    dx = arena.empty((T, W), _f32, dev)
    dxb = arena.empty((T, W), dy.dtype, dev) if want_bf16 else None
    parts = arena.empty((3, nblk + L.npcd_colsum_scratch_rows(), W), _f32, dev)
    full = dres is not None and want_bf16
    check(_timed("ln_bwd" if full else "ln_bwd_partial",
                 lambda: L.npcd_ln_bwd_dt(ptr(dy), ptr(x), ptr(mean), ptr(rstd), ptr(gamma), ptr(dres), ptr(dx), ptr(dxb), ptr(parts[0]),
                                          ptr(parts[1]), ptr(parts[2]) if dcol_out is not None else ptr(None), T, W, dtype_code(dy), stream_ptr())),
          "npcd_ln_bwd")
    _finish(batch, parts[0], nblk, W, dgamma_out)
    _finish(batch, parts[1], nblk, W, dbeta_out)
    if dcol_out is not None:
        _finish(batch, parts[2], nblk, W, dcol_out)
    return dx, dxb


def gelu_fwd(h):
    g = arena.empty_like(h)
    check(_timed("gelu_fwd", lambda: lib().npcd_gelu_fwd_dt(ptr(h), ptr(g), h.numel(), dtype_code(h), stream_ptr())), "npcd_gelu_fwd")
    return g


def gelu_bwd(dg, h, dbias_out, batch=None, out=None, part_rows=None):
    T, N = h.shape
    L = lib()
    nblk = L.npcd_colsum_blocks(T)
    dh = arena.empty_like(h) if out is None else out
    if part_rows is not None:
        check(_timed("gelu_bwd", lambda: L.npcd_gelu_bwd_dt(ptr(dg), ptr(h), ptr(dh), ptr(part_rows), T, N, dtype_code(h), stream_ptr())), "npcd_gelu_bwd")
        return dh, nblk
    part = arena.empty((nblk + L.npcd_colsum_scratch_rows(), N), _f32, h.device)
    check(_timed("gelu_bwd", lambda: L.npcd_gelu_bwd_dt(ptr(dg), ptr(h), ptr(dh), ptr(part), T, N, dtype_code(h), stream_ptr())), "npcd_gelu_bwd")
    _finish(batch, part, nblk, N, dbias_out)
    return dh


def colsum_bf16(a, out, batch=None):
    T, N = a.shape
    L = lib()
    nblk = L.npcd_colsum_blocks(T)
    part = arena.empty((nblk + L.npcd_colsum_scratch_rows(), N), _f32, a.device)
    check(L.npcd_colsum_dt(ptr(a), ptr(part), T, N, dtype_code(a), stream_ptr()), "npcd_colsum")
    _finish(batch, part, nblk, N, out)
    return out


def adamw_ema(p, g, m, v, ema, shadow, lr, beta1, beta2, eps, weight_decay, step, ema_decay, zero_grad=True):
    require_gpu(p)
    check(lib().npcd_adamw_ema_dt(ptr(p), ptr(g), ptr(m), ptr(v), ptr(ema), ptr(shadow), dtype_code(shadow) if shadow is not None else 0,
                                  p.numel(), float(lr), float(beta1), float(beta2), float(eps), float(weight_decay), int(step),
                                  float(ema_decay if ema_decay is not None else 0.0), int(bool(zero_grad)), stream_ptr()), "npcd_adamw_ema")



CTL_FOUND_INF, CTL_STEP, CTL_GROWTH_TRACKER, CTL_SKIPPED = 0, 1, 2, 3
CTL_LOSS_SCALE, CTL_INV_SCALE, CTL_GRAD_NORM, CTL_CLIP_COEF, CTL_BC1, CTL_BC2_SQRT = 4, 5, 6, 7, 8, 9
CTL_WORDS = 16


def scaler_record(device, loss_scale=1.0, step=0):
    ctl = torch.zeros(CTL_WORDS, dtype=torch.int32, device=device)
    ctl[CTL_STEP] = int(step)
    ctl.view(_f32)[CTL_LOSS_SCALE] = float(loss_scale)
    return ctl


def grad_stats_work(device):
    return torch.empty(2 * lib().npcd_grad_stats_blocks(), dtype=torch.float64, device=device)


def grad_stats(g, out, work):
    require_gpu(g)
    check(lib().npcd_grad_stats(ptr(g), g.numel(), ptr(work), ptr(out), stream_ptr()), "npcd_grad_stats")


def scaler_finalize(stats, nslots, ctl, scaling, max_norm, beta1, beta2, growth_factor=2.0, backoff_factor=0.5, growth_interval=2000):
    check(lib().npcd_scaler_finalize(ptr(stats), int(nslots), ptr(ctl), int(bool(scaling)), int(max_norm is not None),
                                     float(max_norm if max_norm is not None else 0.0), float(beta1), float(beta2), float(growth_factor),
                                     float(backoff_factor), int(growth_interval), stream_ptr()), "npcd_scaler_finalize")


def adamw_ema_gated(p, g, m, v, ema, shadow, lr, beta1, beta2, eps, weight_decay, ema_decay, ctl, zero_grad=True):
    require_gpu(p)
    check(lib().npcd_adamw_ema_gated(ptr(p), ptr(g), ptr(m), ptr(v), ptr(ema), ptr(shadow), dtype_code(shadow) if shadow is not None else 0,
                                     p.numel(), float(lr), float(beta1), float(beta2), float(eps), float(weight_decay),
                                     float(ema_decay if ema_decay is not None else 0.0), int(bool(zero_grad)), ptr(ctl), stream_ptr()),
          "npcd_adamw_ema_gated")

def small_wgrad(dy, x):
    T, J = dy.shape
    K = x.shape[1]
    if not (1 <= J <= 4 and 64 <= K <= 2048 and K & (K - 1) == 0 and dy.dtype == _bf16 and x.dtype == _bf16 and dy.is_contiguous()
            and x.is_contiguous() and T > 0):
        return None
    L = lib()
    nblk = L.npcd_small_wgrad_blocks(T)
    part = arena.empty((nblk + L.npcd_colsum_scratch_rows(), J * K), _f32, x.device)
    out = arena.empty((J, K), _f32, x.device)
    check(L.npcd_small_wgrad(ptr(dy), ptr(x), ptr(part), T, J, K, stream_ptr()), "npcd_small_wgrad")
    check(L.npcd_colsum_finalize(ptr(part), nblk, J * K, ptr(out), 0, stream_ptr()), "npcd_colsum_finalize")
    return out


def wgrad(dy, x, out):
    T, N = dy.shape
    K = x.shape[1]
    if (N % 256 or K % 256 or dy.dtype != x.dtype or dy.dtype not in (_bf16, _f16) or not dy.is_contiguous() or not x.is_contiguous()
            or not out.is_contiguous() or out.dtype != _f32):
        return False
    L = lib()
    S = L.npcd_wgrad_slices(T, N, K)
    ws = arena.empty((S, N, K), _f32, dy.device) if S > 1 else None
    check(L.npcd_wgrad(ptr(dy), ptr(x), ptr(out), ptr(ws), T, N, K, dtype_code(dy), stream_ptr()), "npcd_wgrad")
    return True


WGRAD_GROUP_MAX = 16


def wgrad_group(triples):
    import ctypes
    n = len(triples)
    if not 1 <= n <= WGRAD_GROUP_MAX:
        return False
    T, dt = triples[0][0].shape[0], triples[0][0].dtype
    for dy, x, out in triples:
        if (dy.shape[0] != T or x.shape[0] != T or dy.dtype != dt or x.dtype != dt or dt not in (_bf16, _f16) or dy.shape[1] % 256 or x.shape[1] % 256
                or not dy.is_contiguous() or not x.is_contiguous() or not out.is_contiguous() or out.dtype != _f32
                or tuple(out.shape) != (dy.shape[1], x.shape[1])):
            return False
    if len({t[2].data_ptr() for t in triples}) != n:
        return False
    P = ctypes.c_void_p * n
    I = ctypes.c_int * n
    check(lib().npcd_wgrad_group(n, P(*[ptr(t[0]) for t in triples]), P(*[ptr(t[1]) for t in triples]), P(*[ptr(t[2]) for t in triples]),
                                 I(*[t[0].shape[1] for t in triples]), I(*[t[1].shape[1] for t in triples]), T, dtype_code(triples[0][0]), stream_ptr()),
          "npcd_wgrad_group")
    return True


def wgrad_group_blocks_rule(tiles_per_block, max_products, products_per_block, cus):
    if tiles_per_block <= 0 or products_per_block <= 0 or cus <= 0:
        return 0
    G = 1
    while G * products_per_block <= max_products:
        tiles = G * tiles_per_block
        rounds = -(-tiles // cus)
        if tiles * 100 >= rounds * cus * 95:
            return G
        G += 1
    return 0


def wgrad_group_blocks(shapes):
    if not shapes or any(N % 256 or K % 256 for N, K in shapes):
        return 0
    return int(lib().npcd_wgrad_group_blocks(sum((N // 256) * (K // 256) for N, K in shapes), WGRAD_GROUP_MAX, len(shapes)))


def sum_slices(part, out):
    S, n = part.shape[0], out.numel()
    if S not in (2, 4, 8) or n % 4 or not part.is_contiguous() or not out.is_contiguous() or part.dtype != _f32 or out.dtype != _f32:
        return False
    check(lib().npcd_sum_slices(ptr(part), ptr(out), S, n, stream_ptr()), "npcd_sum_slices")
    return True


def cast_f32_bf16(src, dst):
    check(lib().npcd_cast_f32_dt(ptr(src), ptr(dst), src.numel(), dtype_code(dst), stream_ptr()), "npcd_cast_f32")
    return dst


def split3(x, bias=None, gelu=False):
    require_gpu(x)
    x = x.contiguous()
    T, K = x.shape
    out = arena.empty((T, 3 * K), torch.bfloat16, x.device)
    b = None if bias is None else bias.to(torch.float32).contiguous()
    check(lib().npcd_split3_bf16(ptr(x), ptr(b), ptr(out), T, K, 1 if gelu else 0, stream_ptr()), "npcd_split3_bf16")
    return out


def add_ln_split3(x, gamma, beta, o=None, bias=None, eps=1e-5):
    require_gpu(x)
    T, W = x.shape
    if W % 256 or W // 256 not in (1, 2, 3, 4, 8, 16):
        return None
    x = x.contiguous()
    out = arena.empty((T, 3 * W), torch.bfloat16, x.device)
    xnew = None
    if o is not None:
        o = o.contiguous()
        bias = bias.to(torch.float32).contiguous()
        xnew = arena.empty_like(x)
    check(lib().npcd_add_ln_split3_bf16(ptr(x), ptr(o), ptr(bias), ptr(gamma.contiguous()), ptr(beta.contiguous()), ptr(xnew), ptr(out), T, W,
                                        float(eps), stream_ptr()), "npcd_add_ln_split3_bf16")
    return (x if xnew is None else xnew), out


class SplitWeight(ctypes.Structure):
    _fields_ = [("w", ctypes.c_void_p), ("fwd", ctypes.c_void_p), ("dgrad", ctypes.c_void_p), ("N", ctypes.c_int), ("K", ctypes.c_int)]


def split_weights(ws):
    require_gpu(*ws)
    if not all(w.is_contiguous() and w.dtype == _f32 for w in ws):
        raise RuntimeError("split_weights takes contiguous fp32 weights (the views of a trainer's flat parameter buffer)")
    out = []
    arr = (SplitWeight * len(ws))()
    for a, w in zip(arr, ws):
        N, K = w.shape
        f, d = arena.empty((N, 3 * K), _bf16, w.device), arena.empty((3 * N, K), _bf16, w.device)
        a.w, a.fwd, a.dgrad, a.N, a.K = w.data_ptr(), f.data_ptr(), d.data_ptr(), N, K
        out.append((f, d))
    check(lib().npcd_split_weights_bf16(ctypes.cast(arr, ctypes.c_void_p), len(ws), stream_ptr()), "npcd_split_weights_bf16")
    return out


def add_ln_split3_stats(x, gamma, beta, o=None, bias=None, eps=1e-5):
    require_gpu(x)
    T, W = x.shape
    if W % 256 or W // 256 not in (1, 2, 3, 4, 8, 16):
        raise RuntimeError(f"npcd_add_ln_split3_stats_bf16 takes widths 256, 512, 768, 1024, 2048 and 4096 (got {W})")
    x = x.contiguous()
    out = arena.empty((T, 3 * W), _bf16, x.device)
    mean, rstd = arena.empty(T, _f32, x.device), arena.empty(T, _f32, x.device)
    xnew = None
    if o is not None:
        o, bias = o.contiguous(), bias.to(_f32).contiguous()
        xnew = arena.empty_like(x)
    check(lib().npcd_add_ln_split3_stats_bf16(ptr(x), ptr(o), ptr(bias), ptr(gamma.contiguous()), ptr(beta.contiguous()), ptr(xnew), ptr(out),
                                              ptr(mean), ptr(rstd), T, W, float(eps), stream_ptr()), "npcd_add_ln_split3_stats_bf16")
    return (x if xnew is None else xnew), out, mean, rstd


def ln_bwd_split3(dy, x, mean, rstd, gamma, dres, dgamma_out, dbeta_out, dcol_out=None, want_split=True, batch=None):
    T, W = x.shape
    dev = x.device
    L = lib()
    nblk = L.npcd_ln_bwd_blocks(T)
    dx = arena.empty((T, W), _f32, dev)
    dx3 = arena.empty((T, 3 * W), _bf16, dev) if want_split else None
    parts = arena.empty((3, nblk + L.npcd_colsum_scratch_rows(), W), _f32, dev)
    check(L.npcd_ln_bwd_split3_bf16(ptr(dy), ptr(x), ptr(mean), ptr(rstd), ptr(gamma), ptr(dres), ptr(dx), ptr(dx3), ptr(parts[0]), ptr(parts[1]),
                                    ptr(parts[2]) if dcol_out is not None else ptr(None), T, W, stream_ptr()), "npcd_ln_bwd_split3_bf16")
    _finish(batch, parts[0], nblk, W, dgamma_out)
    _finish(batch, parts[1], nblk, W, dbeta_out)
    if dcol_out is not None:
        _finish(batch, parts[2], nblk, W, dcol_out)
    return dx, dx3


def split3_colsum(a, colsum_out, h=None, bias=None, batch=None):
    require_gpu(a)
    T, N = a.shape
    L = lib()
    nblk = L.npcd_colsum_blocks(T)
    out = arena.empty((T, 3 * N), _bf16, a.device)
    part = arena.empty((nblk + L.npcd_colsum_scratch_rows(), N), _f32, a.device)
    b = None if bias is None else bias.to(_f32).contiguous()
    check(L.npcd_split3_colsum_bf16(ptr(a), ptr(h), ptr(b), ptr(out), ptr(part), T, N, int(h is not None), stream_ptr()), "npcd_split3_colsum_bf16")
    _finish(batch, part, nblk, N, colsum_out)
    return out


def ddpm_reverse_step(x_t, eps, noise, t, tables, clip=None, want_x0=False):
    require_gpu(x_t)
    x_t, noise, eps = x_t.contiguous(), noise.contiguous(), eps.contiguous()
    B = x_t.shape[0]
    out = arena.empty_like(x_t)
    x0 = arena.empty_like(x_t) if want_x0 else None
    code = {torch.float32: 2, torch.bfloat16: 0}[eps.dtype]
    lo, hi = (float(clip[0]), float(clip[1])) if clip is not None else (0.0, 0.0)
    check(lib().npcd_ddpm_reverse_step(ptr(x_t), ptr(eps), code, ptr(noise), ptr(out), ptr(x0), ptr(t), B, x_t.numel() // B,
                                       *[ptr(tb) for tb in tables], lo, hi, int(clip is not None), stream_ptr()), "npcd_ddpm_reverse_step")
    return out, x0


class SamplerTensor(ctypes.Structure):
    _fields_ = [("x_t", ctypes.c_void_p), ("eps", ctypes.c_void_p), ("noise", ctypes.c_void_p), ("known", ctypes.c_void_p),
                ("out", ctypes.c_void_p), ("x0_out", ctypes.c_void_p), ("per_sample", ctypes.c_int64), ("clip_lo", ctypes.c_float),
                ("clip_hi", ctypes.c_float), ("has_clip", ctypes.c_int32), ("mode", ctypes.c_int32), ("eps_dtype", ctypes.c_int32),
                ("reserved", ctypes.c_int32)]


SAMPLER_REVERSE, SAMPLER_HOLD = 0, 1


def _sampler_tensor(spec, B):
    hold = spec.get("mode", "reverse") == "hold"
    if spec.get("mode", "reverse") not in ("reverse", "hold"):
        raise ValueError("sampler_step: mode is 'reverse' or 'hold'")
    keep = [None if spec.get(k) is None else spec[k].contiguous() for k in ("x_t", "eps", "noise", "known")]
    x_t, eps, noise, known = keep
    like = known if hold else x_t
    if like is None:
        like = next((v for v in keep if v is not None), None)
    if like is None or like.shape[0] != B:
        raise RuntimeError("sampler_step: every tensor is [B, ...] with the B of t")
    for v in (x_t, noise, known):
        if v is not None and (v.dtype != _f32 or v.shape != like.shape):
            raise RuntimeError("sampler_step: x_t, noise and known are fp32 tensors of one shape")
    if eps is not None and eps.shape != like.shape:
        raise RuntimeError("sampler_step: eps has the shape of x_t")
    require_gpu(*[v for v in keep if v is not None])
    out = spec.get("out")
    out = arena.empty(like.shape, _f32, like.device) if out is None else out
    x0 = spec.get("x0_out")
    if x0 is None and spec.get("want_x0") and not hold:
        x0 = arena.empty(like.shape, _f32, like.device)
    clip = None if hold else spec.get("clip")
    rec = SamplerTensor()
    rec.x_t, rec.eps, rec.noise, rec.known = (0 if v is None else v.data_ptr() for v in keep)
    rec.out, rec.x0_out = out.data_ptr(), (0 if x0 is None else x0.data_ptr())
    rec.per_sample = like.numel() // B
    rec.clip_lo, rec.clip_hi = (float(clip[0]), float(clip[1])) if clip is not None else (0.0, 0.0)
    rec.has_clip, rec.mode = int(clip is not None), SAMPLER_HOLD if hold else SAMPLER_REVERSE
    rec.eps_dtype = dtype_code(eps) if eps is not None else 2
    return rec, out, x0, keep


def sampler_step(coords, feats, t, table, deterministic):
    require_gpu(t, table)
    if t.dtype != torch.int64 or table.dtype != _f32 or table.dim() != 2 or table.shape[1] != 8 or not table.is_contiguous():
        raise RuntimeError("sampler_step: t is int64 [B], table a contiguous fp32 [T, 8]")
    t = t.contiguous()
    B = t.shape[0]
    rc, oc, x0c, keep_c = _sampler_tensor(coords, B)
    rf, of, x0f, keep_f = _sampler_tensor(feats, B)
    check(lib().npcd_sampler_step(ctypes.byref(rc), ctypes.byref(rf), ptr(t), ptr(table), table.shape[0], B, int(bool(deterministic)),
                                  stream_ptr()), "npcd_sampler_step")
    del keep_c, keep_f
    return (oc, x0c), (of, x0f)


def q_sample(x0, noise, t, tab_sqrt_acp, tab_sqrt_1macp):
    require_gpu(x0, noise, t)
    x0, noise = x0.contiguous(), noise.contiguous()
    out = arena.empty_like(x0)
    B = x0.shape[0]
    check(lib().npcd_q_sample(ptr(x0), ptr(noise), ptr(t.contiguous()), ptr(tab_sqrt_acp), ptr(tab_sqrt_1macp), ptr(out), B, x0.numel() // B,
                              stream_ptr()), "npcd_q_sample")
    return out


class _EpsMSE(torch.autograd.Function):

    @staticmethod
    def forward(ctx, eps, noise, want_pointwise):
        from . import dtype_code
        L = lib()
        eps_c, noise_c = eps.contiguous(), noise.contiguous()
        n = eps_c.numel()
        pw = arena.empty(eps_c.shape, _f32, eps.device) if want_pointwise else None
        part = arena.empty(L.npcd_eps_mse_blocks(), _f32, eps.device)
        loss = arena.empty(1, _f32, eps.device)
        check(L.npcd_eps_mse_fwd(ptr(noise_c), ptr(eps_c), dtype_code(eps_c), n, ptr(pw), ptr(part), ptr(loss), stream_ptr()), "npcd_eps_mse_fwd")
        ctx.save_for_backward(eps_c, noise_c)
        if pw is None:
            pw = loss.new_empty(0)
        ctx.mark_non_differentiable(pw)
        return loss[0], pw

    @staticmethod
    def backward(ctx, g, _gpw):
        from . import dtype_code
        eps, noise = ctx.saved_tensors
        grad = arena.empty_like(eps)
        up = g.reshape(1).to(_f32).contiguous()
        check(lib().npcd_eps_mse_bwd(ptr(noise), ptr(eps), dtype_code(eps), eps.numel(), ptr(up), ptr(grad), stream_ptr()), "npcd_eps_mse_bwd")
        return grad, None, None


def eps_mse(eps, noise, want_pointwise=True):
    loss, pw = _EpsMSE.apply(eps, noise, want_pointwise)
    return loss, (pw if want_pointwise else None)
```

neural-point-cloud-diffusion_amd/npcd/models/diffusion/fused.py:

```python
import math

import torch

from ...hip import arena as harena
from ...hip import attention as hattn
from ...hip import elementwise as ew
from ...hip import linear as hlin

_bf16, _f32 = torch.bfloat16, torch.float32
_BLOCK_PARAMS = ("ln_1.weight", "ln_1.bias", "attn.c_qkv.weight", "attn.c_qkv.bias", "attn.c_proj.weight", "attn.c_proj.bias",
                 "ln_2.weight", "ln_2.bias", "mlp.c_fc.weight", "mlp.c_fc.bias", "mlp.c_proj.weight", "mlp.c_proj.bias")
_LINEARS = ("attn_c_qkv", "attn_c_proj", "mlp_c_fc", "mlp_c_proj")


import os


def _env_on(name):
    return os.environ.get(name, "") not in ("", "0")


_SPLIT = 0 if os.environ.get("NPCD_NO_GEMM_SPLIT") else 256
_SPLIT_MIN = int(os.environ.get("NPCD_GEMM_SPLIT_MIN", "16000"))
_SPLIT_BIG_FIRST = not os.environ.get("NPCD_GEMM_SPLIT_SMALL_FIRST")
_ATTN_COLSUM = not os.environ.get("NPCD_NO_ATTN_COLSUM")
_SUM_KERNEL = not os.environ.get("NPCD_NO_SUM_KERNEL")
_OWN_WGRAD = _env_on("NPCD_OWN_WGRAD")
_OWN_DGELU = _env_on("NPCD_OWN_DGELU")
_DGRAD_NN = _env_on("NPCD_DGRAD_NN")
_DGRAD_T_MIN_T = int(os.environ.get("NPCD_DGRAD_T_MIN_T", "16000"))


_SPLIT_WIDE_N = int(os.environ.get("NPCD_GEMM_SPLIT_WIDE_N", "4096"))


def _split_gemm(fn, T, N=0):
    wide = _SPLIT_WIDE_N > 0 and N >= _SPLIT_WIDE_N and T > _SPLIT
    Tm = T - T % _SPLIT if (_SPLIT and (T >= _SPLIT_MIN or wide)) else T
    if Tm == 0 or Tm == T:
        fn(slice(0, T))
        return
    if _SPLIT_BIG_FIRST:
        fn(slice(0, Tm))
        fn(slice(Tm, T))
        return
    fn(slice(Tm, T))
    fn(slice(0, Tm))


_LIN128 = not os.environ.get("NPCD_NO_LIN128")
_LIN128_MAX_T = int(os.environ.get("NPCD_LIN128_MAX_T", "4200"))


def _linear(bias, x, w16):
    T = x.shape[0]
    out = harena.empty((T, w16.shape[0]), x.dtype, x.device)
    N, K = w16.shape
    if (_LIN128 and N == 1024 and K == 1024 and T <= _LIN128_MAX_T and x.is_cuda and x.is_contiguous() and w16.is_contiguous()
            and bias.is_contiguous() and x.dtype == w16.dtype == bias.dtype and hlin.supported128(T, N, K)):
        return hlin.linear128_fwd(x, w16, bias, out)
    wt = w16.t()
    _split_gemm(lambda r: torch.addmm(bias, x[r], wt, out=out[r]), T, N)
    return out


def _dgrad(dy, w16, wT=None):
    T = dy.shape[0]
    out = harena.empty((T, w16.shape[1]), dy.dtype, dy.device)
    b = w16 if wT is None else wT.t()
    _split_gemm(lambda r: torch.mm(dy[r], b, out=out[r]), T, w16.shape[1])
    return out


def _wgrad(dy, x, out):
    if _OWN_WGRAD and ew.wgrad(dy, x, out):
        return
    T = dy.shape[0]
    small = out.numel() <= (1 << 20)
    S = 8 if small else 4
    S = min(S, max(1, T // (2048 if small else 4096)))
    while S > 1 and T % S:
        S //= 2
    if S == 1:
        torch.mm(dy.t(), x, out_dtype=_f32, out=out)
        return
    part = torch.bmm(dy.view(S, T // S, -1).transpose(1, 2), x.view(S, T // S, -1), out_dtype=_f32)
    if not (_SUM_KERNEL and ew.sum_slices(part, out)):
        torch.sum(part, dim=0, out=out)


def _parse_wgrad_stream(value):
    if value is None or value == "":
        return True, 20000
    if value == "0":
        return False, 0
    if value == "1":
        return True, 1 << 62
    try:
        return True, int(value)
    except ValueError:
        raise ValueError(f"NPCD_WGRAD_STREAM={value!r}: expected unset, 0 (off), 1 (on at every size) or a token-row limit") from None


_WGRAD_STREAM, _WGRAD_STREAM_MAX_T = _parse_wgrad_stream(os.environ.get("NPCD_WGRAD_STREAM"))
_side = {}


def _side_stream(device):
    s = _side.get(device)
    if s is None:
        s = _side[device] = torch.cuda.Stream(device=device, priority=int(os.environ.get("NPCD_WGRAD_STREAM_PRIO", "0")))
    return s


def _wgrad_side_ok(T):
    return _WGRAD_STREAM and T <= _WGRAD_STREAM_MAX_T


_WGRAD_GROUP = os.environ.get("NPCD_WGRAD_GROUP", "1") != "0"
_WGRAD_GROUP_MAX_T = int(os.environ.get("NPCD_WGRAD_GROUP_MAX_T", "17000"))
_JOIN_PER_BLOCK = _env_on("NPCD_WGRAD_JOIN_PER_BLOCK")
_STEP_ARENA = os.environ.get("NPCD_STEP_ARENA", "1") != "0"
_STEP_ARENA_MAX_T = int(os.environ.get("NPCD_STEP_ARENA_MAX_T", "20000"))


def _parse_wgrad_multiblock(value):
    modes = {None: "on", "": "on", "1": "on", "0": "off", "force": "force"}
    if value not in modes:
        raise ValueError(f"NPCD_WGRAD_MULTIBLOCK={value!r}: expected unset, 0 (off), 1 (on) or force (skip the fill rule)")
    return modes[value]


_WGRAD_MULTIBLOCK = _parse_wgrad_multiblock(os.environ.get("NPCD_WGRAD_MULTIBLOCK"))
_WGRAD_MULTIBLOCK_MIN_T = int(os.environ.get("NPCD_WGRAD_MULTIBLOCK_MIN_T", "20000"))
_multiblock_blocks = {}


def _wgrad_multiblock_blocks(T, W, dtype, device):
    if (_WGRAD_MULTIBLOCK == "off" or T < _WGRAD_MULTIBLOCK_MIN_T or _wgrad_side_ok(T) or device.type != "cuda"
            or dtype not in (torch.bfloat16, torch.float16)):
        return 0
    if _WGRAD_MULTIBLOCK == "force":
        return ew.WGRAD_GROUP_MAX // len(_LINEARS)
    key = (W, device.index)
    if key not in _multiblock_blocks:
        with torch.cuda.device(device):
            _multiblock_blocks[key] = ew.wgrad_group_blocks([(3 * W, W), (W, W), (4 * W, W), (W, 4 * W)])
    return _multiblock_blocks[key]


def _wgrad_fork(pending, device, before=None):
    side = _side_stream(device)
    with torch.cuda.stream(side):
        if before is not None:
            before()
    side.wait_stream(torch.cuda.current_stream())
    with torch.cuda.stream(side):
        for dy, x, out in pending:
            dy.record_stream(side)
            x.record_stream(side)
        if not (_WGRAD_GROUP and pending and pending[0][0].shape[0] <= _WGRAD_GROUP_MAX_T and ew.wgrad_group(pending)):
            for dy, x, out in pending:
                _wgrad(dy, x, out)
    pending.clear()


def _wgrad_join(device):
    torch.cuda.current_stream().wait_stream(_side_stream(device))


def _no_engine():
    return None


import contextlib

_NULL = contextlib.nullcontext()


class _BlockViews:
    fp32_class = False

    def __deepcopy__(self, memo):
        return None

    def __reduce__(self):
        return (_no_engine, ())

    def __init__(self, backbone, flat, reducer=None):
        self.heads = backbone.resblocks[0].attn.heads
        self.width = backbone.width
        self.reducer = reducer
        self._offset = {id(p): off for p, off in zip(flat.params, flat.offsets)}
        self.blocks = []
        for blk in backbone.resblocks:
            named = dict(blk.named_parameters())
            entry = {"params": [named[n] for n in _BLOCK_PARAMS]}
            for n in _BLOCK_PARAMS:
                p = named[n]
                off = self._offset[id(p)]
                key = n.replace(".", "_")
                entry[key] = p.data
                entry[key + "_g"] = flat.grad[off:off + p.numel()].view_as(p)
            self.blocks.append(entry)
        self.block_ranges, self.wait_range = None, None

    def shadow_written(self):
        pass


class FusedBackboneEngine(_BlockViews):

    def __init__(self, backbone, flat, shadow, reducer=None):
        super().__init__(backbone, flat, reducer)
        for blk, entry in zip(backbone.resblocks, self.blocks):
            named = dict(blk.named_parameters())
            for n in _BLOCK_PARAMS:
                p = named[n]
                off = self._offset[id(p)]
                entry[n.replace(".", "_") + "_16"] = shadow[off:off + p.numel()].view_as(p)

        self._flat, self._shadow = flat, shadow
        self.dtype = shadow.dtype
        self._stamped = [p for e in self.blocks for p in e["params"]]
        self._stamp = self._versions()
        self.shadow_epoch = 0
        self._shadowT, self._wT = None, None
        self._wT_stamp = [None] * len(self.blocks)
        self.transposed_refreshes = 0
        self.arena = harena.StepArena() if _STEP_ARENA else None

    def shadow_written(self):
        self.shadow_epoch += 1

    def wants_transposed(self, T):
        return _OWN_DGELU or (not _DGRAD_NN and T >= _DGRAD_T_MIN_T)

    def refresh_transposed(self, bi):
        if self._wT_stamp[bi] == self.shadow_epoch:
            return
        if self._shadowT is None:
            sizes = [entry[k + "_weight_16"].numel() for entry in self.blocks for k in _LINEARS]
            self._shadowT = torch.empty(sum(sizes), dtype=self._shadow.dtype, device=self._shadow.device)
            self._wT, off = [], 0
            for entry in self.blocks:
                views = []
                for k in _LINEARS:
                    N, K = entry[k + "_weight_16"].shape
                    views.append(self._shadowT[off:off + N * K].view(K, N))
                    off += N * K
                self._wT.append(views)
        e = self.blocks[bi]
        hlin.transpose16_group([(e[k + "_weight_16"], v) for k, v in zip(_LINEARS, self._wT[bi])])
        for k, v in zip(_LINEARS, self._wT[bi]):
            e[k + "_weight_16T"] = v
        self._wT_stamp[bi] = self.shadow_epoch
        self.transposed_refreshes += 1

    def _versions(self):
        return [p._version for p in self._stamped]

    def sync_shadow(self, force=False):
        v = self._versions()
        if force or v != self._stamp:
            if self.wait_range is not None:
                self.wait_range()
            for p, off in zip(self._flat.params, self._flat.offsets):
                if p.data_ptr() != self._flat.flat.data_ptr() + off * self._flat.flat.element_size():
                    raise RuntimeError("a parameter of the fused backbone was re-homed outside the trainer's flat buffer "
                                       "(p.data replaced): build a new DiffusionTrainer for this model")
            ew.cast_f32_bf16(self._flat.flat, self._shadow)
            self.shadow_written()
            self._stamp = v

    def __call__(self, x):
        self.sync_shadow()
        return _BackboneFn.apply(x, self)


class InferenceWeights:

    def __init__(self, backbone):
        self.heads = backbone.resblocks[0].attn.heads
        self.params = [[dict(blk.named_parameters())[n] for n in _BLOCK_PARAMS] for blk in backbone.resblocks]
        self.stamp, self.blocks = None, None

    def current(self):
        stamp = [(p._version, p.data_ptr()) for ps in self.params for p in ps]
        if stamp != self.stamp:
            self.blocks = []
            for ps in self.params:
                e = {}
                for n, p in zip(_BLOCK_PARAMS, ps):
                    key = n.replace(".", "_")
                    e[key] = p.data
                    if not n.startswith("ln_"):
                        e[key + "_16"] = p.data.to(_bf16)
                self.blocks.append(e)
            self.stamp = stamp
        return self.blocks


class InferenceWeightsX2:

    def __init__(self, backbone):
        self.heads = backbone.resblocks[0].attn.heads
        self.params = [[dict(blk.named_parameters())[n] for n in _BLOCK_PARAMS] for blk in backbone.resblocks]
        self.stamp, self.blocks = None, None

    def current(self):
        stamp = [(p._version, p.data_ptr()) for ps in self.params for p in ps]
        if stamp != self.stamp:
            self.blocks = []
            for ps in self.params:
                e = {}
                for n, p in zip(_BLOCK_PARAMS, ps):
                    key = n.replace(".", "_")
                    w = p.data.to(_f32)
                    if n.endswith("weight") and not n.startswith("ln_"):
                        hi = w.to(_bf16)
                        lo = (w - hi.float()).to(_bf16)
                        e[key + "_x3"] = torch.cat((hi, hi, lo), dim=1).contiguous()
                    else:
                        e[key] = w.contiguous()
                self.blocks.append(e)
            self.stamp = stamp
        return self.blocks


def backbone_forward_x2(x, blocks, heads):
    import torch.nn.functional as F
    B, n, W = x.shape
    T, d = B * n, W // heads
    scale = 1.0 / math.sqrt(d)
    f32 = _f32

    def lin(a3, e, name):
        return torch.mm(a3, e[name + "_weight_x3"].t(), out_dtype=f32)
    def ln_split(xs, e, ln, o=None, bias=None):
        r = ew.add_ln_split3(xs, e[ln + "_weight"], e[ln + "_bias"], o, bias)
        if r is not None:
            return r
        if o is not None:
            xs = xs + o + bias
        return xs, ew.split3(F.layer_norm(xs, (W,), e[ln + "_weight"], e[ln + "_bias"]))
    with torch.autocast("cuda", enabled=False):
        xs = x.reshape(T, W).contiguous()
        o, ob = None, None
        for e in blocks:
            xs, y1 = ln_split(xs, e, "ln_1", o, ob)
            qkv = lin(y1, e, "attn_c_qkv").add_(e["attn_c_qkv_bias"]).view(B, n, heads, 3 * d)
            a, _ = hattn._fwd(qkv[..., :d], qkv[..., d:2 * d], qkv[..., 2 * d:], scale)
            xs, y2 = ln_split(xs, e, "ln_2", lin(ew.split3(a.reshape(T, W)), e, "attn_c_proj"), e["attn_c_proj_bias"])
            h = lin(y2, e, "mlp_c_fc")
            o, ob = lin(ew.split3(h, bias=e["mlp_c_fc_bias"], gelu=True), e, "mlp_c_proj"), e["mlp_c_proj_bias"]
        xs = xs + o + ob
    return xs.view(B, n, W)


def backbone_forward(x, blocks, heads, dtype=_bf16):
    B, n, W = x.shape
    T, d = B * n, W // heads
    scale = 1.0 / math.sqrt(d)
    with torch.autocast("cuda", enabled=False):
        xs = x.reshape(T, W).contiguous()
        delta = None
        for e in blocks:
            x1, y1, _, _ = ew.add_ln_fwd(xs, delta, e["ln_1_weight"], e["ln_1_bias"], dtype=dtype)
            x_cur = xs if x1 is None else x1
            q4 = _linear(e["attn_c_qkv_bias_16"], y1, e["attn_c_qkv_weight_16"]).view(B, n, heads, 3 * d)
            a, _ = hattn._fwd(q4[..., :d], q4[..., d:2 * d], q4[..., 2 * d:], scale)
            o = _linear(e["attn_c_proj_bias_16"], a.view(T, W), e["attn_c_proj_weight_16"])
            xs, y2, _, _ = ew.add_ln_fwd(x_cur, o, e["ln_2_weight"], e["ln_2_bias"])
            g = ew.gelu_fwd(_linear(e["mlp_c_fc_bias_16"], y2, e["mlp_c_fc_weight_16"]))
            delta = _linear(e["mlp_c_proj_bias_16"], g, e["mlp_c_proj_weight_16"])
        out = xs + delta
    return out.view(B, n, W)


class _BackboneFn(torch.autograd.Function):
    @staticmethod
    def forward(ctx, x, eng):
        B, n, W = x.shape
        T = B * n
        arena = eng.arena if (eng.arena is not None and x.is_cuda and T <= _STEP_ARENA_MAX_T) else None
        token = arena.begin() if arena is not None else 0
        if not token:
            arena = None
        ctx.arena, ctx.arena_token = arena, token
        if arena is None:
            return _BackboneFn._forward(ctx, x, eng)
        ctx.arena_guard = harena.StepGuard(arena, token)
        try:
            with arena.active():
                return _BackboneFn._forward(ctx, x, eng)
        except BaseException:
            arena.end(token)
            raise

    @staticmethod
    def _forward(ctx, x, eng):
        B, n, W = x.shape
        T, H = B * n, eng.heads
        d = W // H
        scale = 1.0 / math.sqrt(d)
        saved = []
        with torch.autocast("cuda", enabled=False):
            xs = x.reshape(T, W).contiguous()
            delta = None
            ctx.transposed = transposed = x.is_cuda and eng.wants_transposed(T)
            for bi, e in enumerate(eng.blocks):
                if eng.wait_range is not None:
                    eng.wait_range(*eng.block_ranges[bi])
                if transposed:
                    eng.refresh_transposed(bi)
                x1, y1, mean1, rstd1 = ew.add_ln_fwd(xs, delta, e["ln_1_weight"], e["ln_1_bias"], dtype=eng.dtype)
                x_cur = xs if x1 is None else x1
                qkv = _linear(e["attn_c_qkv_bias_16"], y1, e["attn_c_qkv_weight_16"])
                q4 = qkv.view(B, n, H, 3 * d)
                a, lse = hattn._fwd(q4[..., :d], q4[..., d:2 * d], q4[..., 2 * d:], scale)
                a = a.view(T, W)
                o = _linear(e["attn_c_proj_bias_16"], a, e["attn_c_proj_weight_16"])
                x2, y2, mean2, rstd2 = ew.add_ln_fwd(x_cur, o, e["ln_2_weight"], e["ln_2_bias"])
                h = _linear(e["mlp_c_fc_bias_16"], y2, e["mlp_c_fc_weight_16"])
                g = ew.gelu_fwd(h)
                delta = _linear(e["mlp_c_proj_bias_16"], g, e["mlp_c_proj_weight_16"])
                saved.append((x_cur, mean1, rstd1, y1, qkv, a, lse, x2, mean2, rstd2, y2, h, g))
                xs = x2
            out = xs + delta
        ctx.eng, ctx.saved, ctx.dims, ctx.scale = eng, saved, (B, n, W, H, d), scale
        return out.view(B, n, W)

    @staticmethod
    def backward(ctx, dout):
        if any(s is None for s in ctx.saved):
            raise RuntimeError("the fused backbone engine does not support retain_graph / double backward: run a new forward "
                               "for every backward")
        arena = ctx.arena
        if arena is None:
            return _BackboneFn._backward(ctx, dout)
        try:
            with arena.active():
                return _BackboneFn._backward(ctx, dout)
        finally:
            arena.end(ctx.arena_token)

    @staticmethod
    def _backward(ctx, dout):
        eng, (B, n, W, H, d), scale = ctx.eng, ctx.dims, ctx.scale
        T = B * n
        with torch.autocast("cuda", enabled=False):
            dx = dout.reshape(T, W).contiguous().float()
            dxb = dx.to(eng.dtype)
            last = eng.blocks[-1]
            last["mlp_c_proj_bias_g"].copy_(dx.sum(dim=0))
            side, pending = _wgrad_side_ok(T), []
            dgrad_t = ctx.transposed and not _DGRAD_NN and T >= _DGRAD_T_MIN_T

            reducing = eng.reducer is not None and eng.reducer.active

            def ready(entry):
                if reducing:
                    for p in entry["params"]:
                        eng.reducer.mark_ready(p)
            group = 0 if side else _wgrad_multiblock_blocks(T, W, eng.dtype, dx.device)
            tail = len(eng.blocks) % group if group else len(eng.blocks)
            queued, queued_blocks = [], []
            for bi in range(len(eng.blocks) - 1, -1, -1):
                e = eng.blocks[bi]
                x_cur, mean1, rstd1, y1, qkv, a, lse, x2, mean2, rstd2, y2, h, g = ctx.saved[bi]
                ctx.saved[bi] = None
                sums = ew.ColsumBatch()
                wg = pending.append if side else queued.append if bi >= tail else (lambda t: _wgrad(*t))
                Tm = T - T % 256
                w2 = e["mlp_c_proj_weight_16"]
                if (_OWN_DGELU and ctx.transposed and Tm > 0 and hlin.supported(Tm, 4 * W, W) and dxb.is_contiguous() and h.is_contiguous()
                        and w2.is_contiguous() and dxb.dtype == w2.dtype == h.dtype and dxb.dtype in (torch.bfloat16, torch.float16)):
                    wT = e["mlp_c_proj_weight_16T"]
                    dh = harena.empty_like(h)
                    extra = ew.lib().npcd_colsum_blocks(T - Tm) if Tm < T else 0
                    _, part, rows = hlin.linear_dgelu_bwd(dxb[:Tm], wT, h[:Tm], out=dh[:Tm], extra_part_rows=extra)
                    if Tm < T:
                        dg = torch.mm(dxb[Tm:], wT.t() if dgrad_t else w2)
                        ew.gelu_bwd(dg, h[Tm:], None, out=dh[Tm:], part_rows=part[rows:])
                        del dg
                    sums.add(part, rows + extra, 4 * W, e["mlp_c_fc_bias_g"])
                    wg((dxb, g, e["mlp_c_proj_weight_g"]))
                    del g, h
                else:
                    dg = _dgrad(dxb, w2, e["mlp_c_proj_weight_16T"] if dgrad_t else None)
                    wg((dxb, g, e["mlp_c_proj_weight_g"]))
                    dh = ew.gelu_bwd(dg, h, e["mlp_c_fc_bias_g"], batch=sums)
                    del dg, g, h
                dy2 = _dgrad(dh, e["mlp_c_fc_weight_16"], e["mlp_c_fc_weight_16T"] if dgrad_t else None)
                wg((dh, y2, e["mlp_c_fc_weight_g"]))
                del dh, y2
                dx2, dx2b = ew.ln_bwd(dy2, x2, mean2, rstd2, e["ln_2_weight"], dx, e["ln_2_weight_g"], e["ln_2_bias_g"],
                                      e["attn_c_proj_bias_g"], batch=sums)
                del dy2, x2, dx, dxb
                da = _dgrad(dx2b, e["attn_c_proj_weight_16"], e["attn_c_proj_weight_16T"] if dgrad_t else None)
                wg((dx2b, a, e["attn_c_proj_weight_g"]))
                dqkv = harena.empty_like(qkv)
                q4, g4 = qkv.view(B, n, H, 3 * d), dqkv.view(B, n, H, 3 * d)
                cpart = hattn.colsum_part_for(g4[..., :d]) if _ATTN_COLSUM else None
                hattn._bwd(q4[..., :d], q4[..., d:2 * d], q4[..., 2 * d:], a.view(B, n, H, d), da.view(B, n, H, d), lse,
                           g4[..., :d], g4[..., d:2 * d], g4[..., 2 * d:], scale, colsum_part=cpart[0] if cpart else None)
                del da, a, qkv, dx2b
                if cpart:
                    sums.add(cpart[0], cpart[1], 3 * W, e["attn_c_qkv_bias_g"])
                else:
                    ew.colsum_bf16(dqkv, e["attn_c_qkv_bias_g"], batch=sums)
                dy1 = _dgrad(dqkv, e["attn_c_qkv_weight_16"], e["attn_c_qkv_weight_16T"] if dgrad_t else None)
                wg((dqkv, y1, e["attn_c_qkv_weight_g"]))
                del dqkv, y1
                prev_bias_g = eng.blocks[bi - 1]["mlp_c_proj_bias_g"] if bi > 0 else None
                with (harena.paused() if bi == 0 else _NULL):
                    dx, dxb = ew.ln_bwd(dy1, x_cur, mean1, rstd1, e["ln_1_weight"], dx2, e["ln_1_weight_g"], e["ln_1_bias_g"],
                                        prev_bias_g, want_bf16=bi > 0, batch=sums)
                del dy1, dx2
                sums.flush()
                if side and _JOIN_PER_BLOCK:
                    if bi + 1 < len(eng.blocks):
                        _wgrad_join(dx.device)
                        ready(eng.blocks[bi + 1])
                    _wgrad_fork(pending, dx.device)
                elif side:
                    above = eng.blocks[bi + 1] if (reducing and bi + 1 < len(eng.blocks)) else None
                    _wgrad_fork(pending, dx.device, before=None if above is None else (lambda: ready(above)))
                elif bi >= tail:
                    queued_blocks.append(e)
                    if (len(eng.blocks) - bi) % group == 0:
                        if not ew.wgrad_group(queued):
                            for t in queued:
                                _wgrad(*t)
                        queued.clear()
                        for qe in queued_blocks:
                            ready(qe)
                        queued_blocks.clear()
                else:
                    ready(e)
            if side:
                _wgrad_join(dx.device)
                ready(eng.blocks[0])
        return dx.view(B, n, W), None


SPLIT_WIDTHS = (256, 512, 768, 1024, 2048)
_X2_LINEARS = ("attn_c_qkv", "attn_c_proj", "mlp_c_fc", "mlp_c_proj")


def x2_supported(width, heads):
    if heads <= 0 or width % heads or width // heads != 64:
        return (f"head dim {width // heads if heads > 0 and width % heads == 0 else width / max(heads, 1)}: the fp32 attention backward "
                f"is built for head dim 64 only")
    if width not in SPLIT_WIDTHS:
        return f"width {width}: the split-operand kernels take widths {', '.join(map(str, SPLIT_WIDTHS))}"
    return None


def _mm_x2(a3, w3):
    return torch.mm(a3, w3, out_dtype=_f32)


def _wgrad_x2(dy3, x3, out):
    T, N = dy3.shape[0], out.shape[0]
    K = out.shape[1]
    d, x = dy3.view(T, 3, N), x3.view(T, 3, K)
    part = harena.empty((3, N, K), _f32, out.device)
    torch.bmm(d[:, 0:2].permute(1, 2, 0), x[:, 1:3].permute(1, 0, 2), out_dtype=_f32, out=part[0:2])
    torch.mm(d[:, 0].t(), x[:, 0], out_dtype=_f32, out=part[2])
    torch.sum(part, dim=0, out=out)


_X2_WGRAD = os.environ.get("NPCD_X2_WGRAD", "library")
if _X2_WGRAD not in ("library", "own"):
    raise ValueError(f"NPCD_X2_WGRAD={_X2_WGRAD!r}: expected library or own")


def _stack_x2(a3, lo_first):
    T, N = a3.shape[0], a3.shape[1] // 3
    v = a3.view(T, 3, N)
    out = harena.empty((3, T, N), _bf16, a3.device)
    if lo_first:
        out[0].copy_(v[:, 1])
        out[1:].copy_(v[:, 0::2].transpose(0, 1))
    else:
        out.copy_(v.transpose(0, 1))
    return out.view(3 * T, N)


def _wgrad_own(pending):
    triples = [(_stack_x2(dy3, False), _stack_x2(x3, True), out) for dy3, x3, out in pending]
    pending.clear()
    if triples[0][0].shape[0] <= _WGRAD_GROUP_MAX_T:
        ok = ew.wgrad_group(triples)
    else:
        ok = all(ew.wgrad(dy, x, out) for dy, x, out in triples)
    if not ok:
        raise RuntimeError("fp32-class weight gradients: the own kernels do not take these shapes (NPCD_X2_WGRAD=library does)")


class FusedBackboneEngineX2(_BlockViews):
    fp32_class = True

    def __init__(self, backbone, flat, reducer=None):
        why = x2_supported(backbone.width, backbone.resblocks[0].attn.heads)
        if why is not None:
            raise ValueError(f"fp32_class training: {why}")
        super().__init__(backbone, flat, reducer)

    def __call__(self, x):
        return _BackboneX2Fn.apply(x, self)


class _BackboneX2Fn(torch.autograd.Function):
    @staticmethod
    def forward(ctx, x, eng):
        B, n, W = x.shape
        T, H = B * n, eng.heads
        d = W // H
        scale = 1.0 / math.sqrt(d)
        saved = []
        with torch.autocast("cuda", enabled=False):
            xs = x.reshape(T, W).contiguous().float()
            o, ob = None, None
            for bi, e in enumerate(eng.blocks):
                if eng.wait_range is not None:
                    eng.wait_range(*eng.block_ranges[bi])
                split = dict(zip(_X2_LINEARS, ew.split_weights([e[k + "_weight"] for k in _X2_LINEARS])))
                x_cur, y1, mean1, rstd1 = ew.add_ln_split3_stats(xs, e["ln_1_weight"], e["ln_1_bias"], o, ob)
                qkv = _mm_x2(y1, split["attn_c_qkv"][0].t()).add_(e["attn_c_qkv_bias"])
                q4 = qkv.view(B, n, H, 3 * d)
                a, lse = hattn._fwd_f32(q4[..., :d], q4[..., d:2 * d], q4[..., 2 * d:], scale, want_lse=True)
                a = a.view(T, W)
                o = _mm_x2(ew.split3(a), split["attn_c_proj"][0].t())
                x2, y2, mean2, rstd2 = ew.add_ln_split3_stats(x_cur, e["ln_2_weight"], e["ln_2_bias"], o, e["attn_c_proj_bias"])
                h = _mm_x2(y2, split["mlp_c_fc"][0].t())
                o, ob = _mm_x2(ew.split3(h, bias=e["mlp_c_fc_bias"], gelu=True), split["mlp_c_proj"][0].t()), e["mlp_c_proj_bias"]
                saved.append((x_cur, mean1, rstd1, y1, qkv, a, lse, x2, mean2, rstd2, y2, h, {k: v[1] for k, v in split.items()}))
                del split
                xs = x2
            out = xs + o + ob
        ctx.eng, ctx.saved, ctx.dims, ctx.scale = eng, saved, (B, n, W, H, d), scale
        return out.view(B, n, W)

    @staticmethod
    def backward(ctx, dout):
        if any(s is None for s in ctx.saved):
            raise RuntimeError("the fused backbone engine does not support retain_graph / double backward: run a new forward "
                               "for every backward")
        eng, (B, n, W, H, d), scale = ctx.eng, ctx.dims, ctx.scale
        T = B * n
        with torch.autocast("cuda", enabled=False):
            dx = dout.reshape(T, W).contiguous().float()
            eng.blocks[-1]["mlp_c_proj_bias_g"].copy_(dx.sum(dim=0))
            dx3 = ew.split3(dx)
            reducing = eng.reducer is not None and eng.reducer.active
            for bi in range(len(eng.blocks) - 1, -1, -1):
                e = eng.blocks[bi]
                x_cur, mean1, rstd1, y1, qkv, a, lse, x2, mean2, rstd2, y2, h, wd = ctx.saved[bi]
                ctx.saved[bi] = None
                sums = ew.ColsumBatch()
                pending = []
                wg = (lambda *t: pending.append(t)) if _X2_WGRAD == "own" else _wgrad_x2
                dg = _mm_x2(dx3, wd["mlp_c_proj"])
                wg(dx3, ew.split3(h, bias=e["mlp_c_fc_bias"], gelu=True), e["mlp_c_proj_weight_g"])
                dh3 = ew.split3_colsum(dg, e["mlp_c_fc_bias_g"], h=h, bias=e["mlp_c_fc_bias"], batch=sums)
                del dg, h
                dy2 = _mm_x2(dh3, wd["mlp_c_fc"])
                wg(dh3, y2, e["mlp_c_fc_weight_g"])
                del dh3, y2
                dx2, dx2_3 = ew.ln_bwd_split3(dy2, x2, mean2, rstd2, e["ln_2_weight"], dx, e["ln_2_weight_g"], e["ln_2_bias_g"],
                                              e["attn_c_proj_bias_g"], batch=sums)
                del dy2, x2, dx, dx3
                da = _mm_x2(dx2_3, wd["attn_c_proj"])
                wg(dx2_3, ew.split3(a), e["attn_c_proj_weight_g"])
                del dx2_3
                dqkv = torch.empty_like(qkv)
                q4, g4, a4 = qkv.view(B, n, H, 3 * d), dqkv.view(B, n, H, 3 * d), a.view(B, n, H, d)
                hattn._bwd_f32(q4[..., :d], q4[..., d:2 * d], q4[..., 2 * d:], a4, da.view(B, n, H, d), lse,
                               g4[..., :d], g4[..., d:2 * d], g4[..., 2 * d:], scale)
                del da, a, qkv, lse
                dqkv3 = ew.split3_colsum(dqkv, e["attn_c_qkv_bias_g"], batch=sums)
                del dqkv
                dy1 = _mm_x2(dqkv3, wd["attn_c_qkv"])
                wg(dqkv3, y1, e["attn_c_qkv_weight_g"])
                del dqkv3, y1
                prev_bias_g = eng.blocks[bi - 1]["mlp_c_proj_bias_g"] if bi > 0 else None
                dx, dx3 = ew.ln_bwd_split3(dy1, x_cur, mean1, rstd1, e["ln_1_weight"], dx2, e["ln_1_weight_g"], e["ln_1_bias_g"],
                                           prev_bias_g, want_split=bi > 0, batch=sums)
                del dy1, dx2
                if pending:
                    _wgrad_own(pending)
                sums.flush()
                if reducing:
                    for p in e["params"]:
                        eng.reducer.mark_ready(p)
        return dx.view(B, n, W), None
```

neural-point-cloud-diffusion_amd/npcd/models/diffusion/transformer.py:

```python
import math
import os
from typing import Tuple

import torch
import torch.nn as nn
import torch.nn.functional as F

from ...hip.attention import attention_qkvpacked

_NO_FAST_GLUE = bool(os.environ.get("NPCD_NO_FAST_GLUE"))


def timestep_embedding(t: torch.Tensor, dim: int, max_period: float = 10000.0) -> torch.Tensor:
    half = dim // 2
    j = torch.arange(half, dtype=torch.float32, device=t.device)
    freqs = torch.exp(j * (-math.log(max_period)) / half)
    ang = t.reshape(-1, 1) * freqs.reshape(1, -1)
    emb = torch.cat((torch.cos(ang), torch.sin(ang)), dim=1)
    if dim & 1:
        emb = F.pad(emb, (0, 1))
    return emb


def _normal_init(linear: nn.Linear, std: float):
    nn.init.normal_(linear.weight, std=std)
    nn.init.zeros_(linear.bias)


class QKVMultiheadAttention(nn.Module):

    def __init__(self, *, heads: int, dropout: float = 0.0, use_flash_attn: bool = True):
        super().__init__()
        if dropout:
            raise NotImplementedError("attention dropout is 0 everywhere in the reference")
        self.heads = heads
        self.use_flash_attn = use_flash_attn

    def forward(self, qkv: torch.Tensor) -> torch.Tensor:
        return attention_qkvpacked(qkv, self.heads)


class MultiheadAttention(nn.Module):
    def __init__(self, *, width: int, heads: int, init_scale: float = 1.0, use_flash_attn: bool = True):
        super().__init__()
        self.width, self.heads = width, heads
        self.c_qkv = nn.Linear(width, 3 * width)
        self.c_proj = nn.Linear(width, width)
        self.attention = QKVMultiheadAttention(heads=heads, use_flash_attn=use_flash_attn)
        _normal_init(self.c_qkv, init_scale)
        _normal_init(self.c_proj, init_scale)

    def forward(self, x):
        return self.c_proj(self.attention(self.c_qkv(x)))


class MLP(nn.Module):
    def __init__(self, *, width: int, init_scale: float = 1.0):
        super().__init__()
        self.width = width
        self.c_fc = nn.Linear(width, 4 * width)
        self.c_proj = nn.Linear(4 * width, width)
        _normal_init(self.c_fc, init_scale)
        _normal_init(self.c_proj, init_scale)

    def forward(self, x):
        return self.c_proj(F.gelu(self.c_fc(x)))


class ResidualAttentionBlock(nn.Module):

    def __init__(self, *, width: int, heads: int, init_scale: float = 1.0, use_flash_attn: bool = True):
        super().__init__()
        self.attn = MultiheadAttention(width=width, heads=heads, init_scale=init_scale, use_flash_attn=use_flash_attn)
        self.ln_1 = nn.LayerNorm(width)
        self.ln_2 = nn.LayerNorm(width)
        self.mlp = MLP(width=width, init_scale=init_scale)

    def forward(self, x):
        x = x + self.attn(self.ln_1(x))
        return x + self.mlp(self.ln_2(x))


class Transformer(nn.Module):
    def __init__(self, *, width: int, layers: int, heads: int, init_scale: float = 0.25, use_flash_attn: bool = True):
        super().__init__()
        self.width, self.layers = width, layers
        std = init_scale * math.sqrt(1.0 / width)
        self.resblocks = nn.ModuleList(
            ResidualAttentionBlock(width=width, heads=heads, init_scale=std, use_flash_attn=use_flash_attn)
            for _ in range(layers))
        self.fused_engine = None
        self._infer_weights = None
        self._infer_weights_x2 = None
        self.fp32_class = False

    def forward(self, x):
        eng = self.fused_engine
        if eng is not None and eng.fp32_class:
            if x.is_cuda and x.dtype == torch.float32 and torch.is_grad_enabled() and not torch.is_autocast_enabled():
                return eng(x)
            if eng.wait_range is not None:
                eng.wait_range()
            eng = None
        if x.is_cuda and x.dtype == torch.float32 and torch.is_autocast_enabled():
            act = torch.get_autocast_dtype("cuda")
            if torch.is_grad_enabled():
                if eng is not None and eng.dtype == act:
                    return eng(x)
            elif eng is not None and eng.dtype == act:
                from . import fused
                if eng.wait_range is not None:
                    eng.wait_range()
                eng.sync_shadow()
                return fused.backbone_forward(x, eng.blocks, eng.heads, eng.dtype)
            elif eng is None and act == torch.bfloat16:
                from . import fused
                if self._infer_weights is None:
                    self._infer_weights = fused.InferenceWeights(self)
                return fused.backbone_forward(x, self._infer_weights.current(), self._infer_weights.heads)
        if eng is not None and eng.wait_range is not None:
            eng.wait_range()
        if (self.fp32_class and x.is_cuda and x.dtype == torch.float32 and not torch.is_autocast_enabled() and not torch.is_grad_enabled()
                and self.width // self.resblocks[0].attn.heads == 64 and self.width % 8 == 0):
            from . import fused
            if self._infer_weights_x2 is None:
                self._infer_weights_x2 = fused.InferenceWeightsX2(self)
            return fused.backbone_forward_x2(x, self._infer_weights_x2.current(), self._infer_weights_x2.heads)
        for blk in self.resblocks:
            x = blk(x)
        return x


class _TimeTokenCat(torch.autograd.Function):

    @staticmethod
    def forward(ctx, temb, tokens, bias):
        B, N, W = tokens.shape
        h = torch.empty((B, N + 1, W), dtype=tokens.dtype, device=tokens.device)
        h[:, 0] = temb
        h[:, 1:] = tokens
        ctx.bias_dtype = bias.dtype
        return h

    @staticmethod
    def backward(ctx, dh):
        from ...hip import elementwise as ew
        dh = dh.contiguous()
        B, n, W = dh.shape
        db = None
        if ctx.needs_input_grad[2]:
            db = torch.empty(W, dtype=torch.float32, device=dh.device)
            ew.colsum_bf16(dh.view(B * n, W), db)
            db -= dh[:, 0].float().sum(dim=0)
            db = db.to(ctx.bias_dtype)
        return dh[:, 0], dh[:, 1:], db


class _LayerNormToBF16(torch.autograd.Function):

    @staticmethod
    def forward(ctx, x, gamma, beta, eps):
        from ...hip import elementwise as ew
        B, n, W = x.shape
        x2 = x.reshape(B * n, W).contiguous()
        _, y, mean, rstd = ew.add_ln_fwd(x2, None, gamma, beta, eps=eps, dtype=torch.get_autocast_dtype("cuda"))
        ctx.save_for_backward(x2, mean, rstd, gamma)
        return y.view(B, n, W)

    @staticmethod
    def backward(ctx, dy):
        from ...hip import elementwise as ew
        x2, mean, rstd, gamma = ctx.saved_tensors
        B, n, W = dy.shape
        dgamma, dbeta = torch.empty(W, dtype=torch.float32, device=dy.device), torch.empty(W, dtype=torch.float32, device=dy.device)
        dx, _ = ew.ln_bwd(dy.reshape(B * n, W).contiguous(), x2, mean, rstd, gamma, None, dgamma, dbeta, want_bf16=False)
        return dx.view(B, n, W), dgamma.to(gamma.dtype), dbeta.to(gamma.dtype), None


class NPCDTransformer(nn.Module):

    def __init__(self, *, coords_dim: int, feats_dim: int, width: int = 512, layers: int = 12, heads: int = 8,
                 init_scale: float = 0.25, use_flash_attn: bool = True):
        super().__init__()
        self.coords_dim, self.feats_dim = coords_dim, feats_dim
        self.input_channels = self.output_channels = coords_dim + feats_dim
        self.time_embed = MLP(width=width, init_scale=init_scale * math.sqrt(1.0 / width))
        self.ln_pre = nn.LayerNorm(width)
        self.backbone = Transformer(width=width, layers=layers, heads=heads, init_scale=init_scale,
                                    use_flash_attn=use_flash_attn)
        self.ln_post = nn.LayerNorm(width)
        self.input_proj = nn.Linear(self.input_channels, width)
        self.output_proj = nn.Linear(width, self.output_channels)
        nn.init.zeros_(self.output_proj.weight)
        nn.init.zeros_(self.output_proj.bias)

    def forward(self, coords: torch.Tensor, feats: torch.Tensor, t: torch.Tensor) -> Tuple[torch.Tensor, torch.Tensor]:
        x = torch.cat((coords, feats), dim=1).transpose(1, 2)
        temb = self.time_embed(timestep_embedding(t, self.backbone.width))
        if (x.is_cuda and torch.is_grad_enabled() and torch.is_autocast_enabled()
                and torch.get_autocast_dtype("cuda") in (torch.bfloat16, torch.float16) and self.backbone.width % 8 == 0 and not _NO_FAST_GLUE):
            tokens = F.linear(x, self.input_proj.weight, self.input_proj.bias.detach())
            h = _TimeTokenCat.apply(temb.to(tokens.dtype), tokens, self.input_proj.bias)
        else:
            tokens = self.input_proj(x)
            h = torch.cat((temb.unsqueeze(1).to(tokens.dtype), tokens), dim=1)
        h = self.backbone(self.ln_pre(h))
        W = h.shape[-1]
        if (h.is_cuda and h.dtype == torch.float32 and torch.is_grad_enabled() and torch.is_autocast_enabled() and W % 4 == 0 and W <= 2048
                and torch.get_autocast_dtype("cuda") in (torch.bfloat16, torch.float16) and self.ln_post.weight.dtype == torch.float32
                and not _NO_FAST_GLUE):
            h = _LayerNormToBF16.apply(h, self.ln_post.weight, self.ln_post.bias, self.ln_post.eps)
        else:
            h = self.ln_post(h)
        eps = self.output_proj(h[:, 1:]).transpose(1, 2)
        return eps[:, :self.coords_dim], eps[:, self.coords_dim:]
```

Before: 12.81 steps/s.

## Fuse time-token concat into ln_pre and final residual add into ln_post readout

Adds HIP LayerNorm kernel modes. The embed mode reads the time embedding and the input tokens directly, without first building a concatenated tensor, and writes the fp32 ln_pre output. The readout mode folds the last block's residual add into ln_post and writes only the non-time token rows. The matching backward kernels scatter gradients back to the token and time-embedding buffers and drop the time row's gradient. This removes the separate concat, residual add and slice kernels and their memory traffic, at the cost of more code paths and a lower occupancy bound in the new backward kernels.

```diff
diff --git a/include/npcd_hip.h b/include/npcd_hip.h
--- a/include/npcd_hip.h
+++ b/include/npcd_hip.h
@@ -197,6 +197,16 @@
                       float lr, float beta1, float beta2, float eps, float weight_decay, int step,
                       float ema_decay, int zero_grad, void* stream);
 int npcd_cast_f32_dt(const float* src, void* dst, int64_t numel, int dtype, void* stream);
+int npcd_embed_ln_fwd(const void* tokens, const void* temb, const float* gamma, const float* beta, float* x0, float* mean,
+                      float* rstd, int B, int N, int W, float eps, int dtype, void* stream);
+int npcd_embed_ln_bwd(const float* dy, const void* tokens, const void* temb, const float* mean, const float* rstd,
+                      const float* gamma, void* dtok, void* dtemb, float* part_gamma, float* part_beta, float* part_col,
+                      int B, int N, int W, int dtype, void* stream);
+int npcd_readout_ln_fwd(const float* x_in, const void* delta, const float* gamma, const float* beta, float* x_out, void* y_tok,
+                        float* mean, float* rstd, int B, int N, int W, float eps, int dtype, void* stream);
+int npcd_readout_ln_bwd(const void* dy_tok, const float* x, const float* mean, const float* rstd, const float* gamma, float* dx,
+                        void* dxb, float* part_gamma, float* part_beta, float* part_col, int B, int N, int W, int dtype,
+                        void* stream);
 
 typedef struct NpcdScalerCtl {
     int32_t found_inf, step, growth_tracker, skipped;
diff --git a/neural-point-cloud-diffusion_amd/csrc/elementwise.hip b/neural-point-cloud-diffusion_amd/csrc/elementwise.hip
--- a/neural-point-cloud-diffusion_amd/csrc/elementwise.hip
+++ b/neural-point-cloud-diffusion_amd/csrc/elementwise.hip
@@ -1,6 +1,8 @@
 #include <math.h>
 
 #include <stdlib.h>
+
+#include <type_traits>
 
 #include "common.h"
 
@@ -20,11 +22,19 @@
 __device__ __forceinline__ f32x4 bf16x4_to_f32(bf16x4 v) { return to_f32(v); }
 __device__ __forceinline__ bf16x4 f32_to_bf16x4(f32x4 v) { return from_f32<__bf16>(v); }
 
-template <class E, int NCH>
+enum { LN_PLAIN = 0, LN_EMBED = 1, LN_READOUT = 2 };
+
+__device__ __forceinline__ int64_t token_row(int r, int n1) {
+    const int b = r / n1;
+    return r - b * n1 == 0 ? (int64_t)(-1 - b) : (int64_t)r - b - 1;
+}
+
+template <class E, int NCH, int MODE = LN_PLAIN>
 __global__ __launch_bounds__(256) void add_ln_fwd_kernel(const float* __restrict__ x_in, const E* __restrict__ delta,
                                                          const float* __restrict__ gamma, const float* __restrict__ beta,
                                                          float* __restrict__ x_out, E* __restrict__ y, float* __restrict__ mean,
-                                                         float* __restrict__ rstd, int T, int W, float eps) {
+                                                         float* __restrict__ rstd, int T, int W, float eps,
+                                                         const E* __restrict__ temb, float* __restrict__ y32, int n1) {
     using e4 = typename V<E>::x4;
     const int lane = threadIdx.x & 63, wave = threadIdx.x >> 6;
     const int NW = gridDim.x * 4;
@@ -44,23 +54,37 @@
     }
     auto load_row = [&](int r) {
         const int64_t base = (int64_t)r * W;
+        const E* src16 = nullptr;
+        if constexpr (MODE == LN_EMBED) {
+            const int64_t tr = token_row(r, n1);
+            src16 = tr < 0 ? temb + (-1 - tr) * W : delta + tr * W;
+        }
 #pragma unroll
         for (int ch = 0; ch < NCH; ++ch) {
             const int c = ch * 256 + lane * 4;
             if (c < W) {
-                nx[ch] = *reinterpret_cast<const f32x4*>(x_in + base + c);
-                if (delta) nd[ch] = *reinterpret_cast<const e4*>(delta + base + c);
+                if constexpr (MODE == LN_EMBED) {
+                    nd[ch] = *reinterpret_cast<const e4*>(src16 + c);
+                } else {
+                    nx[ch] = *reinterpret_cast<const f32x4*>(x_in + base + c);
+                    if (delta) nd[ch] = *reinterpret_cast<const e4*>(delta + base + c);
+                }
             }
         }
     };
     load_row(row);
     for (; row < T; row += NW) {
         const int64_t base = (int64_t)row * W;
+        [[maybe_unused]] const int64_t tr = MODE == LN_READOUT ? token_row(row, n1) : 0;
         float s = 0.f;
 #pragma unroll
         for (int ch = 0; ch < NCH; ++ch) {
-            v[ch] = nx[ch];
-            if (delta) v[ch] += to_f32(nd[ch]);
+            if constexpr (MODE == LN_EMBED) {
+                v[ch] = to_f32(nd[ch]);
+            } else {
+                v[ch] = nx[ch];
+                if (delta) v[ch] += to_f32(nd[ch]);
+            }
         }
         if (row + NW < T) load_row(row + NW);
 #pragma unroll
@@ -85,7 +109,13 @@
 #pragma unroll
         for (int ch = 0; ch < NCH; ++ch) {
             const int c = ch * 256 + lane * 4;
-            if (c < W) *reinterpret_cast<e4*>(y + base + c) = from_f32<E>((v[ch] - mu) * rs * gm[ch] + bt[ch]);
+            if constexpr (MODE == LN_EMBED) {
+                if (c < W) *reinterpret_cast<f32x4*>(y32 + base + c) = (v[ch] - mu) * rs * gm[ch] + bt[ch];
+            } else if constexpr (MODE == LN_READOUT) {
+                if (c < W && tr >= 0) *reinterpret_cast<e4*>(y + tr * W + c) = from_f32<E>((v[ch] - mu) * rs * gm[ch] + bt[ch]);
+            } else {
+                if (c < W) *reinterpret_cast<e4*>(y + base + c) = from_f32<E>((v[ch] - mu) * rs * gm[ch] + bt[ch]);
+            }
         }
         if (lane == 0) {
             mean[row] = mu;
@@ -100,13 +130,16 @@
     return 16;
 }
 
-template <class E, int NCH, class D = E, bool SPLIT = false>
-__global__ __launch_bounds__(256, 2) void ln_bwd_kernel(const D* __restrict__ dy, const float* __restrict__ x, const float* __restrict__ mean,
+template <class E, int NCH, class D = E, bool SPLIT = false, int MODE = LN_PLAIN>
+__global__ __launch_bounds__(256, (MODE != LN_PLAIN && NCH == 8) ? 1 : 2) void ln_bwd_kernel(
+                                                     const D* __restrict__ dy, const float* __restrict__ x, const float* __restrict__ mean,
                                                      const float* __restrict__ rstd, const float* __restrict__ gamma,
                                                      const float* __restrict__ dres, float* __restrict__ dx, E* __restrict__ dxb,
                                                      float* __restrict__ part_gamma, float* __restrict__ part_beta,
-                                                     float* __restrict__ part_col, int T, int W, int rows_per_wave) {
+                                                     float* __restrict__ part_col, int T, int W, int rows_per_wave,
+                                                     const E* __restrict__ x16, const E* __restrict__ t16, E* __restrict__ dt16, int n1) {
     using e4 = typename V<D>::x4;
+    using x4 = typename std::conditional<MODE == LN_EMBED, typename V<E>::x4, f32x4>::type;
     extern __shared__ __attribute__((aligned(16))) unsigned char dsmem[];
     float* red = reinterpret_cast<float*>(dsmem);
     const int lane = threadIdx.x & 63, wave = threadIdx.x >> 6;
@@ -116,18 +149,28 @@
     const int row0 = blockIdx.x * 4 + wave, NW = gridDim.x * 4;
     const int nrows = row0 < T ? min(rows_per_wave, (T - row0 + NW - 1) / NW) : 0;
     e4 dyA[NCH], dyB[NCH];
-    f32x4 xA[NCH], xB[NCH], rA[NCH], rB[NCH];
+    x4 xA[NCH], xB[NCH];
+    f32x4 rA[NCH], rB[NCH];
     float muA = 0.f, rsA = 0.f, muB = 0.f, rsB = 0.f;
-    auto load_row = [&](int row, e4 (&dyr)[NCH], f32x4 (&xr)[NCH], f32x4 (&rr2)[NCH], float& mu, float& rs) {
+    auto load_row = [&](int row, e4 (&dyr)[NCH], x4 (&xr)[NCH], f32x4 (&rr2)[NCH], float& mu, float& rs) {
         const int64_t base = (int64_t)row * W;
+        [[maybe_unused]] const int64_t tr = MODE != LN_PLAIN ? token_row(row, n1) : 0;
+        [[maybe_unused]] const E* xrow = nullptr;
+        if constexpr (MODE == LN_EMBED) xrow = tr < 0 ? t16 + (-1 - tr) * W : x16 + tr * W;
         mu = mean[row];
         rs = rstd[row];
 #pragma unroll
         for (int ch = 0; ch < NCH; ++ch) {
             const int c = ch * 256 + lane * 4;
             if (c < W) {
-                dyr[ch] = *reinterpret_cast<const e4*>(dy + base + c);
-                xr[ch] = *reinterpret_cast<const f32x4*>(x + base + c);
+                if constexpr (MODE == LN_READOUT) {
+                    dyr[ch] = e4{0, 0, 0, 0};
+                    if (tr >= 0) dyr[ch] = *reinterpret_cast<const e4*>(dy + tr * W + c);
+                } else {
+                    dyr[ch] = *reinterpret_cast<const e4*>(dy + base + c);
+                }
+                if constexpr (MODE == LN_EMBED) xr[ch] = *reinterpret_cast<const x4*>(xrow + c);
+                else xr[ch] = *reinterpret_cast<const x4*>(x + base + c);
                 if (dres) rr2[ch] = *reinterpret_cast<const f32x4*>(dres + base + c);
             }
         }
@@ -136,6 +179,7 @@
     for (int rr = 0; rr < nrows; ++rr) {
         const int row = row0 + rr * NW;
         const int64_t base = (int64_t)row * W;
+        [[maybe_unused]] const int64_t tr = MODE == LN_EMBED ? token_row(row, n1) : 0;
         if (rr + 1 < nrows) load_row(row + NW, dyB, xB, rB, muB, rsB);
         const float mu = muA, rs = rsA;
         f32x4 gy[NCH], xh[NCH];
@@ -146,7 +190,7 @@
             gy[ch] = xh[ch] = f32x4{0.f, 0.f, 0.f, 0.f};
             if (c < W) {
                 const f32x4 d = to_f32(dyA[ch]);
-                xh[ch] = (xA[ch] - mu) * rs;
+                xh[ch] = (to_f32(xA[ch]) - mu) * rs;
                 ag[ch] += d * xh[ch];
                 ab[ch] += d;
                 gy[ch] = d * *reinterpret_cast<const f32x4*>(gamma + c);
@@ -162,6 +206,16 @@
             if (c < W) {
                 f32x4 o = (gy[ch] - c1 - xh[ch] * c2) * rs;
                 if (dres) o += rA[ch];
+                if constexpr (MODE == LN_EMBED) {
+                    const typename V<E>::x4 ob = from_f32<E>(o);
+                    if (tr >= 0) {
+                        *reinterpret_cast<typename V<E>::x4*>(dxb + tr * W + c) = ob;
+                        ac[ch] += to_f32(ob);
+                    } else {
+                        *reinterpret_cast<typename V<E>::x4*>(dt16 + (-1 - tr) * W + c) = ob;
+                    }
+                    continue;
+                }
                 *reinterpret_cast<f32x4*>(dx + base + c) = o;
                 if (SPLIT && dxb) {
                     bf16x4 hi, lo;
@@ -724,7 +778,8 @@
         return NPCD_ERR_ARG;
 #define NPCD_LAUNCH_LN_FWD(E, NCH)                                                                                            \
     hipLaunchKernelGGL((add_ln_fwd_kernel<E, NCH>), dim3(ln_fwd_blocks(T)), dim3(256), 0, static_cast<hipStream_t>(stream), x_in, \
-                       static_cast<const E*>(delta), gamma, beta, x_out, static_cast<E*>(y), mean, rstd, T, W, eps)
+                       static_cast<const E*>(delta), gamma, beta, x_out, static_cast<E*>(y), mean, rstd, T, W, eps,         \
+                       static_cast<const E*>(nullptr), static_cast<float*>(nullptr), 0)
 #define NPCD_LN_FWD_W(E)                     \
     do {                                     \
         if (W <= 256) NPCD_LAUNCH_LN_FWD(E, 1);      \
@@ -759,7 +814,8 @@
     else NPCD_HIP_CHECK(lds_attr_h.ensure(reinterpret_cast<const void*>(ln_bwd_kernel<_Float16, 8>), 3 * 4 * 2048 * 4));
 #define NPCD_LAUNCH_LN_BWD(E, NCH)                                                                                             \
     hipLaunchKernelGGL((ln_bwd_kernel<E, NCH>), dim3(nblk), dim3(256), lds, st, static_cast<const E*>(dy), x, mean, rstd, gamma, \
-                       dres, dx, static_cast<E*>(dxb), part_gamma, part_beta, part_col, T, W, ln_rows_per_wave(T))
+                       dres, dx, static_cast<E*>(dxb), part_gamma, part_beta, part_col, T, W, ln_rows_per_wave(T),                \
+                       static_cast<const E*>(nullptr), static_cast<const E*>(nullptr), static_cast<E*>(nullptr), 0)
 #define NPCD_LN_BWD_W(E)                     \
     do {                                     \
         if (W <= 256) NPCD_LAUNCH_LN_BWD(E, 1);      \
@@ -787,7 +843,8 @@
     NPCD_HIP_CHECK(lds_attr.ensure(reinterpret_cast<const void*>(ln_bwd_kernel<__bf16, 8, float, true>), 3 * 4 * 2048 * 4));
 #define NPCD_LAUNCH_LN_BWD3(NCH)                                                                                                        \
     hipLaunchKernelGGL((ln_bwd_kernel<__bf16, NCH, float, true>), dim3(nblk), dim3(256), lds, st, dy, x, mean, rstd, gamma, dres, dx, \
-                       static_cast<__bf16*>(dx3), part_gamma, part_beta, part_col, T, W, ln_rows_per_wave(T))
+                       static_cast<__bf16*>(dx3), part_gamma, part_beta, part_col, T, W, ln_rows_per_wave(T),                              \
+                       static_cast<const __bf16*>(nullptr), static_cast<const __bf16*>(nullptr), static_cast<__bf16*>(nullptr), 0)
     if (W <= 256) NPCD_LAUNCH_LN_BWD3(1);
     else if (W <= 512) NPCD_LAUNCH_LN_BWD3(2);
     else if (W <= 1024) NPCD_LAUNCH_LN_BWD3(4);
@@ -801,6 +858,106 @@
                            float* dx, void* dxb, float* part_gamma, float* part_beta, float* part_col, int T, int W, void* stream) {
     return npcd_ln_bwd_dt(dy, x, mean, rstd, gamma, dres, dx, dxb, part_gamma, part_beta, part_col, T, W, NPCD_BF16, stream);
 }
+
+static inline bool seq_rows(int B, int N, int* T) {
+    if (B <= 0 || N <= 0 || (int64_t)B * ((int64_t)N + 1) > 0x7fffffff) return false;
+    *T = B * (N + 1);
+    return true;
+}
+static inline bool al8(const void* p) { return (reinterpret_cast<uintptr_t>(p) & 7) == 0; }
+
+#define NPCD_LN_BY_WIDTH(LAUNCH, E)      \
+    do {                                 \
+        if (W <= 256) LAUNCH(E, 1);      \
+        else if (W <= 512) LAUNCH(E, 2); \
+        else if (W <= 1024) LAUNCH(E, 4);\
+        else LAUNCH(E, 8);               \
+    } while (0)
+
+template <int MODE>
+static int ln_fwd_mode(const float* x_in, const void* rows16, const void* temb, const float* gamma, const float* beta, float* x_out, void* y,
+                       float* y32, float* mean, float* rstd, int T, int n1, int W, float eps, int dtype, void* stream) {
+#define NPCD_LAUNCH_LN_FWD_MODE(E, NCH)                                                                                                 \
+    hipLaunchKernelGGL((add_ln_fwd_kernel<E, NCH, MODE>), dim3(ln_fwd_blocks(T)), dim3(256), 0, static_cast<hipStream_t>(stream), x_in, \
+                       static_cast<const E*>(rows16), gamma, beta, x_out, static_cast<E*>(y), mean, rstd, T, W, eps,                     \
+                       static_cast<const E*>(temb), y32, n1)
+    if (dtype == NPCD_BF16) NPCD_LN_BY_WIDTH(NPCD_LAUNCH_LN_FWD_MODE, __bf16);
+    else NPCD_LN_BY_WIDTH(NPCD_LAUNCH_LN_FWD_MODE, _Float16);
+#undef NPCD_LAUNCH_LN_FWD_MODE
+    NPCD_HIP_CHECK(hipGetLastError());
+    return NPCD_OK;
+}
+
+extern "C" int npcd_embed_ln_fwd(const void* tokens, const void* temb, const float* gamma, const float* beta, float* x0, float* mean,
+                                 float* rstd, int B, int N, int W, float eps, int dtype, void* stream) {
+    int T = 0;
+    if (!tokens || !temb || !gamma || !beta || !x0 || !mean || !rstd || W <= 0 || !seq_rows(B, N, &T)) return NPCD_ERR_ARG;
+    if (W % 4 != 0 || W > 256 * kMaxChunks || !dt16(dtype)) return NPCD_ERR_UNSUPPORTED;
+    if (!al16(gamma) || !al16(beta) || !al16(x0) || !al8(tokens) || !al8(temb)) return NPCD_ERR_ARG;
+    return ln_fwd_mode<LN_EMBED>(nullptr, tokens, temb, gamma, beta, nullptr, nullptr, x0, mean, rstd, T, N + 1, W, eps, dtype, stream);
+}
+
+extern "C" int npcd_readout_ln_fwd(const float* x_in, const void* delta, const float* gamma, const float* beta, float* x_out, void* y_tok,
+                                   float* mean, float* rstd, int B, int N, int W, float eps, int dtype, void* stream) {
+    int T = 0;
+    if (!x_in || !delta || !gamma || !beta || !x_out || !y_tok || !mean || !rstd || W <= 0 || !seq_rows(B, N, &T)) return NPCD_ERR_ARG;
+    if (W % 4 != 0 || W > 256 * kMaxChunks || !dt16(dtype)) return NPCD_ERR_UNSUPPORTED;
+    if (!al16(x_in) || !al16(gamma) || !al16(beta) || !al16(x_out) || !al8(y_tok) || !al8(delta)) return NPCD_ERR_ARG;
+    return ln_fwd_mode<LN_READOUT>(x_in, delta, nullptr, gamma, beta, x_out, y_tok, nullptr, mean, rstd, T, N + 1, W, eps, dtype, stream);
+}
+
+template <class E, class D, int MODE>
+static int ln_bwd_mode(const D* dy, const float* x, const float* mean, const float* rstd, const float* gamma, float* dx, E* dxb,
+                       float* part_gamma, float* part_beta, float* part_col, int T, int n1, int W, const E* x16, const E* t16, E* dt16,
+                       void* stream) {
+    const int nblk = npcd_ln_bwd_blocks(T);
+    const size_t lds = (size_t)3 * 4 * W * sizeof(float);
+    hipStream_t st = static_cast<hipStream_t>(stream);
+    static DynLds lds_attr;
+    NPCD_HIP_CHECK(lds_attr.ensure(reinterpret_cast<const void*>(ln_bwd_kernel<E, 8, D, false, MODE>), 3 * 4 * 2048 * 4));
+#define NPCD_LAUNCH_LN_BWD_MODE(E_, NCH)                                                                                               \
+    hipLaunchKernelGGL((ln_bwd_kernel<E_, NCH, D, false, MODE>), dim3(nblk), dim3(256), lds, st, dy, x, mean, rstd, gamma,              \
+                       static_cast<const float*>(nullptr), dx, dxb, part_gamma, part_beta, part_col, T, W, ln_rows_per_wave(T), x16, t16, \
+                       dt16, n1)
+    NPCD_LN_BY_WIDTH(NPCD_LAUNCH_LN_BWD_MODE, E);
+#undef NPCD_LAUNCH_LN_BWD_MODE
+    NPCD_HIP_CHECK(hipGetLastError());
+    return NPCD_OK;
+}
+
+extern "C" int npcd_embed_ln_bwd(const float* dy, const void* tokens, const void* temb, const float* mean, const float* rstd,
+                                 const float* gamma, void* dtok, void* dtemb, float* part_gamma, float* part_beta, float* part_col, int B,
+                                 int N, int W, int dtype, void* stream) {
+    int T = 0;
+    if (!dy || !tokens || !temb || !mean || !rstd || !gamma || !dtok || !dtemb || !part_gamma || !part_beta || !part_col || W <= 0 ||
+        !seq_rows(B, N, &T))
+        return NPCD_ERR_ARG;
+    if (W % 4 != 0 || W > 256 * kMaxChunks || !dt16(dtype)) return NPCD_ERR_UNSUPPORTED;
+    if (!al16(dy) || !al16(gamma) || !al8(tokens) || !al8(temb) || !al8(dtok) || !al8(dtemb)) return NPCD_ERR_ARG;
+    if (dtype == NPCD_BF16)
+        return ln_bwd_mode<__bf16, float, LN_EMBED>(dy, nullptr, mean, rstd, gamma, nullptr, static_cast<__bf16*>(dtok), part_gamma, part_beta,
+                                                    part_col, T, N + 1, W, static_cast<const __bf16*>(tokens),
+                                                    static_cast<const __bf16*>(temb), static_cast<__bf16*>(dtemb), stream);
+    return ln_bwd_mode<_Float16, float, LN_EMBED>(dy, nullptr, mean, rstd, gamma, nullptr, static_cast<_Float16*>(dtok), part_gamma, part_beta,
+                                                  part_col, T, N + 1, W, static_cast<const _Float16*>(tokens),
+                                                  static_cast<const _Float16*>(temb), static_cast<_Float16*>(dtemb), stream);
+}
+
+extern "C" int npcd_readout_ln_bwd(const void* dy_tok, const float* x, const float* mean, const float* rstd, const float* gamma, float* dx,
+                                   void* dxb, float* part_gamma, float* part_beta, float* part_col, int B, int N, int W, int dtype,
+                                   void* stream) {
+    int T = 0;
+    if (!dy_tok || !x || !mean || !rstd || !gamma || !dx || W <= 0 || !seq_rows(B, N, &T)) return NPCD_ERR_ARG;
+    if (W % 4 != 0 || W > 256 * kMaxChunks || !dt16(dtype)) return NPCD_ERR_UNSUPPORTED;
+    if (!al16(x) || !al16(gamma) || !al16(dx) || !al8(dy_tok) || (dxb && !al8(dxb))) return NPCD_ERR_ARG;
+    if (dtype == NPCD_BF16)
+        return ln_bwd_mode<__bf16, __bf16, LN_READOUT>(static_cast<const __bf16*>(dy_tok), x, mean, rstd, gamma, dx, static_cast<__bf16*>(dxb),
+                                                       part_gamma, part_beta, part_col, T, N + 1, W, nullptr, nullptr, nullptr, stream);
+    return ln_bwd_mode<_Float16, _Float16, LN_READOUT>(static_cast<const _Float16*>(dy_tok), x, mean, rstd, gamma, dx,
+                                                       static_cast<_Float16*>(dxb), part_gamma, part_beta, part_col, T, N + 1, W, nullptr,
+                                                       nullptr, nullptr, stream);
+}
+#undef NPCD_LN_BY_WIDTH
 
 __global__ __launch_bounds__(1024) void colsum_onepass_kernel(FinBatch fb) {
     __shared__ float red[16][64];
diff --git a/neural-point-cloud-diffusion_amd/npcd/hip/__init__.py b/neural-point-cloud-diffusion_amd/npcd/hip/__init__.py
--- a/neural-point-cloud-diffusion_amd/npcd/hip/__init__.py
+++ b/neural-point-cloud-diffusion_amd/npcd/hip/__init__.py
@@ -93,6 +93,10 @@
     "npcd_colsum_dt": (c_int, [_P, _P, c_int, c_int, c_int, _P]),
     "npcd_adamw_ema_dt": (c_int, [_P] * 6 + [c_int, c_int64] + [c_float] * 5 + [c_int, c_float, c_int, _P]),
     "npcd_cast_f32_dt": (c_int, [_P, _P, c_int64, c_int, _P]),
+    "npcd_embed_ln_fwd": (c_int, [_P] * 7 + [c_int, c_int, c_int, c_float, c_int, _P]),
+    "npcd_embed_ln_bwd": (c_int, [_P] * 11 + [c_int, c_int, c_int, c_int, _P]),
+    "npcd_readout_ln_fwd": (c_int, [_P] * 8 + [c_int, c_int, c_int, c_float, c_int, _P]),
+    "npcd_readout_ln_bwd": (c_int, [_P] * 10 + [c_int, c_int, c_int, c_int, _P]),
     "npcd_grad_stats_blocks": (c_int, []),
     "npcd_grad_stats": (c_int, [_P, c_int64, _P, _P, _P]),
     "npcd_scaler_finalize": (c_int, [_P, c_int, _P, c_int, c_int] + [c_float] * 5 + [c_int, _P]),
diff --git a/neural-point-cloud-diffusion_amd/npcd/hip/elementwise.py b/neural-point-cloud-diffusion_amd/npcd/hip/elementwise.py
--- a/neural-point-cloud-diffusion_amd/npcd/hip/elementwise.py
+++ b/neural-point-cloud-diffusion_amd/npcd/hip/elementwise.py
@@ -85,6 +85,70 @@
     _finish(batch, parts[1], nblk, W, dbeta_out)
     if dcol_out is not None:
         _finish(batch, parts[2], nblk, W, dcol_out)
+    return dx, dxb
+
+
+def ln_tokens_supported(W, dtype):
+    return W % 4 == 0 and 0 < W <= 2048 and dtype in (_bf16, _f16)
+
+
+def embed_ln_fwd(tokens, temb, gamma, beta, eps=1e-5):
+    require_gpu(tokens, temb)
+    B, N, W = tokens.shape
+    dev = tokens.device
+    x0 = arena.empty((B, N + 1, W), _f32, dev)
+    mean = arena.empty(B * (N + 1), _f32, dev)
+    rstd = arena.empty(B * (N + 1), _f32, dev)
+    check(_timed("embed_ln_fwd", lambda: lib().npcd_embed_ln_fwd(ptr(tokens), ptr(temb), ptr(gamma), ptr(beta), ptr(x0), ptr(mean), ptr(rstd),
+                                                                 B, N, W, float(eps), dtype_code(tokens), stream_ptr())), "npcd_embed_ln_fwd")
+    return x0, mean, rstd
+
+
+def embed_ln_bwd(dy, tokens, temb, mean, rstd, gamma, dgamma_out, dbeta_out, dbias_out, batch=None):
+    B, N, W = tokens.shape
+    dev = tokens.device
+    L = lib()
+    nblk = L.npcd_ln_bwd_blocks(B * (N + 1))
+    dtok = arena.empty_like(tokens)
+    dtemb = arena.empty_like(temb)
+    parts = arena.empty((3, nblk + L.npcd_colsum_scratch_rows(), W), _f32, dev)
+    check(_timed("embed_ln_bwd", lambda: L.npcd_embed_ln_bwd(ptr(dy), ptr(tokens), ptr(temb), ptr(mean), ptr(rstd), ptr(gamma), ptr(dtok),
+                                                             ptr(dtemb), ptr(parts[0]), ptr(parts[1]), ptr(parts[2]), B, N, W,
+                                                             dtype_code(tokens), stream_ptr())), "npcd_embed_ln_bwd")
+    _finish(batch, parts[0], nblk, W, dgamma_out)
+    _finish(batch, parts[1], nblk, W, dbeta_out)
+    _finish(batch, parts[2], nblk, W, dbias_out)
+    return dtok, dtemb
+
+
+def readout_ln_fwd(x_in, delta, gamma, beta, B, N, eps=1e-5, y_out=None):
+    require_gpu(x_in)
+    T, W = x_in.shape
+    dev = x_in.device
+    x_out = arena.empty_like(x_in)
+    y_tok = arena.empty((B, N, W), delta.dtype, dev) if y_out is None else y_out
+    mean = arena.empty(T, _f32, dev)
+    rstd = arena.empty(T, _f32, dev)
+    check(_timed("readout_ln_fwd", lambda: lib().npcd_readout_ln_fwd(ptr(x_in), ptr(delta), ptr(gamma), ptr(beta), ptr(x_out), ptr(y_tok),
+                                                                     ptr(mean), ptr(rstd), B, N, W, float(eps), dtype_code(delta),
+                                                                     stream_ptr())), "npcd_readout_ln_fwd")
+    return x_out, y_tok, mean, rstd
+
+
+def readout_ln_bwd(dy_tok, x, mean, rstd, gamma, dgamma_out, dbeta_out, dcol_out, batch=None):
+    B, N, W = dy_tok.shape
+    dev = x.device
+    L = lib()
+    nblk = L.npcd_ln_bwd_blocks(B * (N + 1))
+    dx = arena.empty((B * (N + 1), W), _f32, dev)
+    dxb = arena.empty((B * (N + 1), W), dy_tok.dtype, dev)
+    parts = arena.empty((3, nblk + L.npcd_colsum_scratch_rows(), W), _f32, dev)
+    check(_timed("readout_ln_bwd", lambda: L.npcd_readout_ln_bwd(ptr(dy_tok), ptr(x), ptr(mean), ptr(rstd), ptr(gamma), ptr(dx), ptr(dxb),
+                                                                 ptr(parts[0]), ptr(parts[1]), ptr(parts[2]), B, N, W, dtype_code(dy_tok),
+                                                                 stream_ptr())), "npcd_readout_ln_bwd")
+    _finish(batch, parts[0], nblk, W, dgamma_out)
+    _finish(batch, parts[1], nblk, W, dbeta_out)
+    _finish(batch, parts[2], nblk, W, dcol_out)
     return dx, dxb
 
 
diff --git a/neural-point-cloud-diffusion_amd/npcd/models/diffusion/fused.py b/neural-point-cloud-diffusion_amd/npcd/models/diffusion/fused.py
--- a/neural-point-cloud-diffusion_amd/npcd/models/diffusion/fused.py
+++ b/neural-point-cloud-diffusion_amd/npcd/models/diffusion/fused.py
@@ -276,6 +276,13 @@
     def __call__(self, x):
         self.sync_shadow()
         return _BackboneFn.apply(x, self)
+
+    def readout_supported(self, x):
+        return x.dim() == 3 and x.shape[1] >= 2 and ew.ln_tokens_supported(x.shape[2], self.dtype)
+
+    def readout(self, x, gamma, beta, eps):
+        self.sync_shadow()
+        return _BackboneFn.apply(x, self, gamma, beta, eps)
 
 
 class InferenceWeights:
@@ -379,8 +386,10 @@
 
 
 class _BackboneFn(torch.autograd.Function):
+
     @staticmethod
-    def forward(ctx, x, eng):
+    def forward(ctx, x, eng, gamma=None, beta=None, eps=None):
+        ctx.tail = None if gamma is None else (gamma, beta, eps)
         B, n, W = x.shape
         T = B * n
         arena = eng.arena if (eng.arena is not None and x.is_cuda and T <= _STEP_ARENA_MAX_T) else None
@@ -427,8 +436,17 @@
                 delta = _linear(e["mlp_c_proj_bias_16"], g, e["mlp_c_proj_weight_16"])
                 saved.append((x_cur, mean1, rstd1, y1, qkv, a, lse, x2, mean2, rstd2, y2, h, g))
                 xs = x2
-            out = xs + delta
+            if ctx.tail is not None:
+                gamma, beta, eps = ctx.tail
+                with harena.paused():
+                    y_tok = torch.empty((B, n - 1, W), dtype=eng.dtype, device=x.device)
+                x_out, _, mean, rstd = ew.readout_ln_fwd(xs, delta, gamma, beta, B, n - 1, eps=eps, y_out=y_tok)
+                ctx.tail_saved = (x_out, mean, rstd, gamma)
+            else:
+                out = xs + delta
         ctx.eng, ctx.saved, ctx.dims, ctx.scale = eng, saved, (B, n, W, H, d), scale
+        if ctx.tail is not None:
+            return y_tok
         return out.view(B, n, W)
 
     @staticmethod
@@ -450,10 +468,22 @@
         eng, (B, n, W, H, d), scale = ctx.eng, ctx.dims, ctx.scale
         T = B * n
         with torch.autocast("cuda", enabled=False):
-            dx = dout.reshape(T, W).contiguous().float()
-            dxb = dx.to(eng.dtype)
             last = eng.blocks[-1]
-            last["mlp_c_proj_bias_g"].copy_(dx.sum(dim=0))
+            if ctx.tail is not None:
+                x_out, mean, rstd, gamma = ctx.tail_saved
+                ctx.tail_saved = None
+                with harena.paused():
+                    dgamma, dbeta = torch.empty(W, dtype=_f32, device=dout.device), torch.empty(W, dtype=_f32, device=dout.device)
+                tail_sums = ew.ColsumBatch()
+                dx, dxb = ew.readout_ln_bwd(dout.contiguous(), x_out, mean, rstd, gamma, dgamma, dbeta, last["mlp_c_proj_bias_g"],
+                                            batch=tail_sums)
+                tail_sums.flush()
+                del x_out, mean, rstd
+                tail_grads = (dgamma.to(gamma.dtype), dbeta.to(ctx.tail[1].dtype), None)
+            else:
+                dx = dout.reshape(T, W).contiguous().float()
+                dxb = dx.to(eng.dtype)
+                last["mlp_c_proj_bias_g"].copy_(dx.sum(dim=0))
             side, pending = _wgrad_side_ok(T), []
             dgrad_t = ctx.transposed and not _DGRAD_NN and T >= _DGRAD_T_MIN_T
 
@@ -542,6 +572,8 @@
             if side:
                 _wgrad_join(dx.device)
                 ready(eng.blocks[0])
+        if ctx.tail is not None:
+            return (dx.view(B, n, W), None) + tail_grads
         return dx.view(B, n, W), None
 
 
diff --git a/neural-point-cloud-diffusion_amd/npcd/models/diffusion/transformer.py b/neural-point-cloud-diffusion_amd/npcd/models/diffusion/transformer.py
--- a/neural-point-cloud-diffusion_amd/npcd/models/diffusion/transformer.py
+++ b/neural-point-cloud-diffusion_amd/npcd/models/diffusion/transformer.py
@@ -156,6 +156,29 @@
         return dh[:, 0], dh[:, 1:], db
 
 
+class _EmbedLN(torch.autograd.Function):
+
+    @staticmethod
+    def forward(ctx, temb, tokens, bias, gamma, beta, eps):
+        from ...hip import elementwise as ew
+        temb, tokens = temb.contiguous(), tokens.contiguous()
+        x0, mean, rstd = ew.embed_ln_fwd(tokens, temb, gamma, beta, eps=eps)
+        ctx.save_for_backward(temb, tokens, mean, rstd, gamma)
+        ctx.dtypes = (bias.dtype, gamma.dtype, beta.dtype)
+        return x0
+
+    @staticmethod
+    def backward(ctx, dx0):
+        from ...hip import elementwise as ew
+        temb, tokens, mean, rstd, gamma = ctx.saved_tensors
+        W = tokens.shape[-1]
+        dgamma, dbeta, dbias = (torch.empty(W, dtype=torch.float32, device=dx0.device) for _ in range(3))
+        sums = ew.ColsumBatch()
+        dtok, dtemb = ew.embed_ln_bwd(dx0.contiguous(), tokens, temb, mean, rstd, gamma, dgamma, dbeta, dbias, batch=sums)
+        sums.flush()
+        return dtemb, dtok, dbias.to(ctx.dtypes[0]), dgamma.to(ctx.dtypes[1]), dbeta.to(ctx.dtypes[2]), None
+
+
 class _LayerNormToBF16(torch.autograd.Function):
 
     @staticmethod
@@ -197,20 +220,33 @@
     def forward(self, coords: torch.Tensor, feats: torch.Tensor, t: torch.Tensor) -> Tuple[torch.Tensor, torch.Tensor]:
         x = torch.cat((coords, feats), dim=1).transpose(1, 2)
         temb = self.time_embed(timestep_embedding(t, self.backbone.width))
-        if (x.is_cuda and torch.is_grad_enabled() and torch.is_autocast_enabled()
-                and torch.get_autocast_dtype("cuda") in (torch.bfloat16, torch.float16) and self.backbone.width % 8 == 0 and not _NO_FAST_GLUE):
+        W = self.backbone.width
+        fast = (x.is_cuda and torch.is_grad_enabled() and torch.is_autocast_enabled()
+                and torch.get_autocast_dtype("cuda") in (torch.bfloat16, torch.float16) and not _NO_FAST_GLUE)
+        ln_rows = fast and W % 4 == 0 and W <= 2048 and x.shape[1] >= 1
+        if ln_rows and self.ln_pre.weight.dtype == self.ln_pre.bias.dtype == torch.float32:
             tokens = F.linear(x, self.input_proj.weight, self.input_proj.bias.detach())
-            h = _TimeTokenCat.apply(temb.to(tokens.dtype), tokens, self.input_proj.bias)
+            h = _EmbedLN.apply(temb.to(tokens.dtype), tokens, self.input_proj.bias, self.ln_pre.weight, self.ln_pre.bias, self.ln_pre.eps)
+        elif fast and W % 8 == 0:
+            tokens = F.linear(x, self.input_proj.weight, self.input_proj.bias.detach())
+            h = self.ln_pre(_TimeTokenCat.apply(temb.to(tokens.dtype), tokens, self.input_proj.bias))
         else:
             tokens = self.input_proj(x)
-            h = torch.cat((temb.unsqueeze(1).to(tokens.dtype), tokens), dim=1)
-        h = self.backbone(self.ln_pre(h))
-        W = h.shape[-1]
-        if (h.is_cuda and h.dtype == torch.float32 and torch.is_grad_enabled() and torch.is_autocast_enabled() and W % 4 == 0 and W <= 2048
-                and torch.get_autocast_dtype("cuda") in (torch.bfloat16, torch.float16) and self.ln_post.weight.dtype == torch.float32
-                and not _NO_FAST_GLUE):
-            h = _LayerNormToBF16.apply(h, self.ln_post.weight, self.ln_post.bias, self.ln_post.eps)
+            h = self.ln_pre(torch.cat((temb.unsqueeze(1).to(tokens.dtype), tokens), dim=1))
+        eng = self.backbone.fused_engine
+        ln_rows = ln_rows and h.dtype == torch.float32 and self.ln_post.weight.dtype == self.ln_post.bias.dtype == torch.float32
+        if (ln_rows and eng is not None and not eng.fp32_class and eng.dtype == torch.get_autocast_dtype("cuda")
+                and eng.readout_supported(h)):
+            h = eng.readout(h, self.ln_post.weight, self.ln_post.bias, self.ln_post.eps)
+            eps = torch.matmul(h, self.output_proj.weight.t()) + self.output_proj.bias.to(h.dtype)
+            eps = eps.transpose(1, 2)
+            return eps[:, :self.coords_dim], eps[:, self.coords_dim:]
         else:
-            h = self.ln_post(h)
-        eps = self.output_proj(h[:, 1:]).transpose(1, 2)
+            h = self.backbone(h)
+            if ln_rows and h.is_cuda:
+                h = _LayerNormToBF16.apply(h, self.ln_post.weight, self.ln_post.bias, self.ln_post.eps)
+            else:
+                h = self.ln_post(h)
+            h = h[:, 1:]
+        eps = self.output_proj(h).transpose(1, 2)
         return eps[:, :self.coords_dim], eps[:, self.coords_dim:]
```

Result: no change. 12.90 steps/s (median of 6 runs) (+0.7%).
